# ArturKKK/graphcast-lite

Hardware: AMD Instinct MI355X
Metric: training samples/sec (6h windows) + achieved HBM GB/s on mesh GCNConv (higher is better)
Workload: dtype f32

## Files before the change

graphcast-lite_amd/csrc/aggregate.hip:

```cpp
#include <algorithm>

#include "common.h"
#include "halo.h"

namespace {

template <int LPR, bool VL, bool VS, int EW, int ITER>
__global__ __launch_bounds__(256) void agg_kernel(const int32_t* __restrict__ rowptr, const int32_t* __restrict__ col,
                                                  const float* __restrict__ w, const int32_t* __restrict__ ecol,
                                                  const float* __restrict__ ew, const float* __restrict__ H,
                                                  int64_t ldh, int64_t bsh, const float* __restrict__ bias,
                                                  float* __restrict__ Y, int64_t ldy, int64_t bsy, int32_t n,
                                                  int32_t B, int32_t F, int32_t nRB, int32_t xcd_map,
                                                  int32_t nt_store, const int32_t* __restrict__ order16) {
  constexpr int RPW = 64 / LPR;
  constexpr int EL = LPR < gcl::kEll ? LPR : gcl::kEll;
  static_assert(EW <= EL, "ELL width exceeds the lanes of a row group");
  const int bid = blockIdx.x;
  int b, rb;
  if (xcd_map) {
    const int xcd = bid & (gcl::kNumXCD - 1);
    const int slot = bid >> 3;
    b = xcd + gcl::kNumXCD * (slot / nRB);
    rb = slot % nRB;
  } else {
    b = bid / nRB;
    rb = bid % nRB;
  }
  if (b >= B) return;
  if (order16) {
    constexpr int RPB = RPW * 4 * ITER, K = 16 / RPB;
    rb = order16[rb / (K > 0 ? K : 1)] * (K > 0 ? K : 1) + rb % (K > 0 ? K : 1);
  }
  const int lane = threadIdx.x & 63;
  const int wave = threadIdx.x >> 6;
  const int sub = lane / LPR;
  const int l = lane % LPR;
  const int gbase = sub * LPR;
  const int c0 = l * 4;
  const bool cactive = c0 < F;
  const int cc = cactive ? c0 : 0;
  const float* __restrict__ Hb = H + (int64_t)b * bsh;
  float* __restrict__ Yb = Y + (int64_t)b * bsy;

  float bz0 = 0.f, bz1 = 0.f, bz2 = 0.f, bz3 = 0.f;
  if (bias && cactive) {
    bz0 = bias[c0];
    if (VS || c0 + 1 < F) bz1 = bias[c0 + 1];
    if (VS || c0 + 2 < F) bz2 = bias[c0 + 2];
    if (VS || c0 + 3 < F) bz3 = bias[c0 + 3];
  }

  auto ld4 = [&](int j, float& x0, float& x1, float& x2, float& x3) {
    const float* p = Hb + (int64_t)j * ldh + cc;
    if (VL) {
      const float4 v = *reinterpret_cast<const float4*>(p);
      x0 = v.x; x1 = v.y; x2 = v.z; x3 = v.w;
    } else {
      x0 = p[0];
      x1 = (cc + 1 < F) ? p[1] : 0.f;
      x2 = (cc + 2 < F) ? p[2] : 0.f;
      x3 = (cc + 3 < F) ? p[3] : 0.f;
    }
  };

  const int row_first = (rb * 4 + wave) * (RPW * ITER) + sub;
  auto meta = [&](int row, int& start, int& end, int& cj, float& wj) {
    const int rc = row < n ? row : n - 1;
    start = rowptr[rc];
    end = rowptr[rc + 1];
    cj = ecol[(int64_t)rc * gcl::kEll + (l & (EL - 1))];
    wj = ew[(int64_t)rc * gcl::kEll + (l & (EL - 1))];
  };
  int start, end, cj;
  float wj;
  meta(row_first, start, end, cj, wj);

#pragma unroll 1
  for (int it = 0; it < ITER; ++it) {
    const int row = row_first + it * RPW;
    int nstart = 0, nend = 0, ncj = 0;
    float nwj = 0.f;
    if (it + 1 < ITER) meta(row + RPW, nstart, nend, ncj, nwj);

    const int deg_all = end - start;
    const bool heavy = deg_all > gcl::kHeavy;
    const int deg = heavy ? 0 : deg_all;
    if (heavy) end = start;
    float a0 = 0.f, a1 = 0.f, a2 = 0.f, a3 = 0.f;
    {
      int jj[EW];
      float ww[EW], v0[EW], v1[EW], v2[EW], v3[EW];
#pragma unroll
      for (int k = 0; k < EW; ++k) {
        jj[k] = __shfl(cj, gbase + k, 64);
        ww[k] = __shfl(wj, gbase + k, 64);
      }
#pragma unroll
      for (int k = 0; k < EW; ++k) ld4(jj[k], v0[k], v1[k], v2[k], v3[k]);
#pragma unroll
      for (int k = 0; k < EW; ++k) {
        const bool in = k < deg;
        a0 += in ? ww[k] * v0[k] : 0.f;
        a1 += in ? ww[k] * v1[k] : 0.f;
        a2 += in ? ww[k] * v2[k] : 0.f;
        a3 += in ? ww[k] * v3[k] : 0.f;
      }
    }
    if (__any(deg > EW)) {
      for (int base = start + EW; base < end; base += LPR) {
        const int mine = base + l;
        int oj = 0;
        float ow = 0.f;
        if (mine < end) {
          oj = col[mine];
          ow = w[mine];
        }
        const int cnt = min(LPR, end - base);
        for (int k = 0; k < cnt; k += 4) {
          const int j0 = __shfl(oj, gbase + k, 64);
          const int j1 = __shfl(oj, gbase + ((k + 1) & (LPR - 1)), 64);
          const int j2 = __shfl(oj, gbase + ((k + 2) & (LPR - 1)), 64);
          const int j3 = __shfl(oj, gbase + ((k + 3) & (LPR - 1)), 64);
          const float w0 = __shfl(ow, gbase + k, 64);
          const float w1 = __shfl(ow, gbase + ((k + 1) & (LPR - 1)), 64);
          const float w2 = __shfl(ow, gbase + ((k + 2) & (LPR - 1)), 64);
          const float w3 = __shfl(ow, gbase + ((k + 3) & (LPR - 1)), 64);
          float p0 = 0, p1 = 0, p2 = 0, p3 = 0, q0 = 0, q1 = 0, q2 = 0, q3 = 0;
          float r0 = 0, r1 = 0, r2 = 0, r3 = 0, s0 = 0, s1 = 0, s2 = 0, s3 = 0;
          ld4(j0, p0, p1, p2, p3);
          if (k + 1 < cnt) ld4(j1, q0, q1, q2, q3);
          if (k + 2 < cnt) ld4(j2, r0, r1, r2, r3);
          if (k + 3 < cnt) ld4(j3, s0, s1, s2, s3);
          a0 += w0 * p0; a1 += w0 * p1; a2 += w0 * p2; a3 += w0 * p3;
          if (k + 1 < cnt) { a0 += w1 * q0; a1 += w1 * q1; a2 += w1 * q2; a3 += w1 * q3; }
          if (k + 2 < cnt) { a0 += w2 * r0; a1 += w2 * r1; a2 += w2 * r2; a3 += w2 * r3; }
          if (k + 3 < cnt) { a0 += w3 * s0; a1 += w3 * s1; a2 += w3 * s2; a3 += w3 * s3; }
        }
      }
    }
    if (row < n && cactive && !heavy) {
      a0 += bz0; a1 += bz1; a2 += bz2; a3 += bz3;
      float* __restrict__ yp = Yb + (int64_t)row * ldy + c0;
      if (VS) {
        if (nt_store) {
          typedef float v4f __attribute__((ext_vector_type(4)));
          v4f v = {a0, a1, a2, a3};
          __builtin_nontemporal_store(v, reinterpret_cast<v4f*>(yp));
        } else {
          *reinterpret_cast<float4*>(yp) = make_float4(a0, a1, a2, a3);
        }
      } else {
        yp[0] = a0;
        if (c0 + 1 < F) yp[1] = a1;
        if (c0 + 2 < F) yp[2] = a2;
        if (c0 + 3 < F) yp[3] = a3;
      }
    }
    start = nstart; end = nend; cj = ncj; wj = nwj;
  }
}

template <int LPR, bool VL, bool VS>
__global__ __launch_bounds__(256) void agg_heavy_kernel(const int32_t* __restrict__ rows_heavy,
                                                        const int32_t* __restrict__ rowptr,
                                                        const int32_t* __restrict__ col, const float* __restrict__ w,
                                                        const float* __restrict__ H, int64_t ldh, int64_t bsh,
                                                        const float* __restrict__ bias, float* __restrict__ Y,
                                                        int64_t ldy, int64_t bsy, int32_t F) {
  constexpr int NG = 256 / LPR;
  __shared__ float red[NG][LPR * 4 + 1];
  const int row = rows_heavy[blockIdx.x];
  const int b = blockIdx.y;
  const int g = threadIdx.x / LPR, l = threadIdx.x % LPR;
  const int c0 = l * 4;
  const bool cactive = c0 < F;
  const int cc = cactive ? c0 : 0;
  const float* __restrict__ Hb = H + (int64_t)b * bsh;
  const int start = rowptr[row], end = rowptr[row + 1];
  float a0 = 0.f, a1 = 0.f, a2 = 0.f, a3 = 0.f;
  auto ld4 = [&](int j, float& x0, float& x1, float& x2, float& x3) {
    const float* p = Hb + (int64_t)j * ldh + cc;
    if (VL) {
      const float4 v = *reinterpret_cast<const float4*>(p);
      x0 = v.x; x1 = v.y; x2 = v.z; x3 = v.w;
    } else {
      x0 = p[0];
      x1 = (cc + 1 < F) ? p[1] : 0.f;
      x2 = (cc + 2 < F) ? p[2] : 0.f;
      x3 = (cc + 3 < F) ? p[3] : 0.f;
    }
  };
  for (int e = start + g; e < end; e += 4 * NG) {
    const int e1 = e + NG, e2 = e + 2 * NG, e3 = e + 3 * NG;
    const int j0 = col[e], j1 = col[e1 < end ? e1 : e], j2 = col[e2 < end ? e2 : e], j3 = col[e3 < end ? e3 : e];
    const float w0 = w[e], w1 = e1 < end ? w[e1] : 0.f, w2 = e2 < end ? w[e2] : 0.f, w3 = e3 < end ? w[e3] : 0.f;
    float p0, p1, p2, p3, q0, q1, q2, q3, r0, r1, r2, r3, s0, s1, s2, s3;
    ld4(j0, p0, p1, p2, p3);
    ld4(j1, q0, q1, q2, q3);
    ld4(j2, r0, r1, r2, r3);
    ld4(j3, s0, s1, s2, s3);
    a0 += w0 * p0; a1 += w0 * p1; a2 += w0 * p2; a3 += w0 * p3;
    if (e1 < end) { a0 += w1 * q0; a1 += w1 * q1; a2 += w1 * q2; a3 += w1 * q3; }
    if (e2 < end) { a0 += w2 * r0; a1 += w2 * r1; a2 += w2 * r2; a3 += w2 * r3; }
    if (e3 < end) { a0 += w3 * s0; a1 += w3 * s1; a2 += w3 * s2; a3 += w3 * s3; }
  }
  red[g][c0] = a0; red[g][c0 + 1] = a1; red[g][c0 + 2] = a2; red[g][c0 + 3] = a3;
  __syncthreads();
  if (g == 0 && cactive) {
    float t0 = 0.f, t1 = 0.f, t2 = 0.f, t3 = 0.f;
#pragma unroll
    for (int q = 0; q < NG; ++q) { t0 += red[q][c0]; t1 += red[q][c0 + 1]; t2 += red[q][c0 + 2]; t3 += red[q][c0 + 3]; }
    if (bias) {
      t0 += bias[c0];
      if (c0 + 1 < F) t1 += bias[c0 + 1];
      if (c0 + 2 < F) t2 += bias[c0 + 2];
      if (c0 + 3 < F) t3 += bias[c0 + 3];
    }
    float* yp = Y + (int64_t)b * bsy + (int64_t)row * ldy + c0;
    if (VS) {
      *reinterpret_cast<float4*>(yp) = make_float4(t0, t1, t2, t3);
    } else {
      yp[0] = t0;
      if (c0 + 1 < F) yp[1] = t1;
      if (c0 + 2 < F) yp[2] = t2;
      if (c0 + 3 < F) yp[3] = t3;
    }
  }
}

using gcl::halo::mul_then_add;
using gcl::halo::row_bcast;
typedef gcl::halo::gptr_t gcl_gptr_t;
typedef gcl::halo::lptr_t gcl_lptr_t;

#ifdef GCL_STAMPS
__device__ unsigned long long agg_stamps[8 * 4096];
#define GCL_AGG_STAMP(i)                                   \
  {                                                        \
    const unsigned long long t_ = __builtin_amdgcn_s_memtime(); \
    st_acc[i] += t_ - st_last;                             \
    st_last = t_;                                          \
  }
#else
#define GCL_AGG_STAMP(i)
#endif

template <int LPR, int T, int MAXPW>
__global__ __launch_bounds__(256) void agg_halo_loop_kernel(const int32_t* __restrict__ list, const int32_t* __restrict__ cnt,
                                                            const int2* __restrict__ rec, const int32_t* __restrict__ rowptr,
                                                            const int32_t* __restrict__ opos, const float* __restrict__ w,
                                                            int32_t smax, const float* __restrict__ H, int64_t ldh,
                                                            int64_t bsh, const float* __restrict__ bias,
                                                            float* __restrict__ Y, int64_t ldy, int64_t bsy, int32_t n,
                                                            int32_t B, int32_t F, int32_t ntiles, int32_t nt_store) {
  extern __shared__ float4 img[];
  constexpr int RPW = 64 / LPR;
  constexpr int NW = 4;
  constexpr int NIT = T / NW / RPW;
  constexpr int SH = LPR == 16 ? 8 : LPR == 32 ? 9 : 10;
  typedef float v4f __attribute__((ext_vector_type(4)));
  typedef __attribute__((address_space(3))) const v4f* lds4_t;
  const int xcd = blockIdx.x & (gcl::kNumXCD - 1);
  const int J = gridDim.x >> 3, j = blockIdx.x >> 3;
  const int nsamp = (B - xcd + gcl::kNumXCD - 1) / gcl::kNumXCD;
  const int items = nsamp * ntiles;
  const int base = items / J, extra = items - base * J;
  int m = j * base + min(j, extra);
  const int mend = m + base + (j < extra ? 1 : 0);
  if (m >= mend) return;
  const int lane = threadIdx.x & 63;
  const int wave = __builtin_amdgcn_readfirstlane(threadIdx.x >> 6);
  const int sub = lane / LPR;
  const int l = lane % LPR;
  const int c0 = l * 4;
  const bool cactive = c0 < F;
  const unsigned cb = (unsigned)(cactive ? c0 : 0) * 4u;
  const unsigned ldb = (unsigned)ldh * 4u;
  const int hstride = smax - T;
  const unsigned lb = (unsigned)(size_t)((gcl_lptr_t)img) + (unsigned)l * 16u;
  const int zrow = smax << SH;

  if (threadIdx.x < LPR) img[smax * LPR + threadIdx.x] = make_float4(0.f, 0.f, 0.f, 0.f);
  float bz0 = 0.f, bz1 = 0.f, bz2 = 0.f, bz3 = 0.f;
  if (bias && cactive) {
    const float4 bv = *reinterpret_cast<const float4*>(bias + c0);
    bz0 = bv.x; bz1 = bv.y; bz2 = bv.z; bz3 = bv.w;
  }

  auto fetch_list = [&](int tile, int (&jj)[MAXPW], int& nhalo) {
    nhalo = cnt[tile] / RPW;
    const int32_t* __restrict__ tl = list + (int64_t)tile * hstride;
#pragma unroll
    for (int q = 0; q < MAXPW; ++q) {
      const int e0 = min((wave + NW * q) * RPW, hstride - RPW);
      int j = tl[e0];
#pragma unroll
      for (int r = 1; r < RPW; ++r) {
        const int jr = tl[e0 + r];
        j = sub == r ? jr : j;
      }
      jj[q] = j;
    }
  };
  int jj[MAXPW], nhalo = 0, tile = -1;
  int2 rc[NIT];
#ifdef GCL_STAMPS
  unsigned long long st_acc[8] = {0, 0, 0, 0, 0, 0, 0, 0}, st_last = __builtin_amdgcn_s_memtime();
#endif

  while (true) {
    const int tnew = m / nsamp;
    const int s = m - tnew * nsamp;
    const int b = xcd + gcl::kNumXCD * s;
    const bool newtile = tnew != tile;
    if (newtile) {
      tile = tnew;
      fetch_list(tile, jj, nhalo);
    }
    GCL_AGG_STAMP(0)
    const char* Hc = reinterpret_cast<const char*>(H + (int64_t)b * bsh);
    float* __restrict__ Yb = Y + (int64_t)b * bsy;
    const int row0 = tile * T + wave * (T / NW) + sub;
#pragma unroll
    for (int it = 0; it < NIT; ++it) {
      const int row = row0 + it * RPW;
      const char* src = Hc + (__umul24(row < n ? row : n - 1, ldb) + cb);
      __builtin_amdgcn_global_load_lds((gcl_gptr_t)src, (gcl_lptr_t)(img + (wave * (T / NW) + it * RPW) * LPR), 16, 0, 0);
    }
#pragma unroll
    for (int q = 0; q < MAXPW; ++q) {
      const int p = wave + NW * q;
      if (p < nhalo) {
        const char* src = Hc + (__umul24(jj[q], ldb) + cb);
        __builtin_amdgcn_global_load_lds((gcl_gptr_t)src, (gcl_lptr_t)(img + (T + p * RPW) * LPR), 16, 0, 0);
      }
    }
    if (newtile) {
#pragma unroll
      for (int it = 0; it < NIT; ++it) {
        const int row = row0 + it * RPW;
        rc[it] = rec[(int64_t)(row < n ? row : n - 1) * gcl::kHaloRec + (l & (gcl::kHaloRec - 1))];
      }
    }
    GCL_AGG_STAMP(1)
    __syncthreads();
    GCL_AGG_STAMP(2)

#pragma unroll
    for (int it = 0; it < NIT; ++it) {
      const int row = row0 + it * RPW;
      const int rx = rc[it].x, rw = rc[it].y;
      const int rxb = (rx & gcl::kHaloPosMask) << SH;
      float a0 = 0.f, a1 = 0.f, a2 = 0.f, a3 = 0.f;
#define GCL_HALO_MULADD(K)                                          \
  {                                                                 \
    const unsigned ad = (unsigned)row_bcast<K>(rxb) + lb;           \
    const float wk = __int_as_float(row_bcast<K>(rw));              \
    const v4f v = *(lds4_t)ad;                                      \
    a0 = mul_then_add(wk, v.x, a0);                                 \
    a1 = mul_then_add(wk, v.y, a1);                                 \
    a2 = mul_then_add(wk, v.z, a2);                                 \
    a3 = mul_then_add(wk, v.w, a3);                                 \
  }
#define GCL_HALO_FMA(K)                                             \
  {                                                                 \
    const unsigned ad = (unsigned)row_bcast<K>(rxb) + lb;           \
    const float wk = __int_as_float(row_bcast<K>(rw));              \
    const v4f v = *(lds4_t)ad;                                      \
    a0 = __fmaf_rn(wk, v.x, a0);                                    \
    a1 = __fmaf_rn(wk, v.y, a1);                                    \
    a2 = __fmaf_rn(wk, v.z, a2);                                    \
    a3 = __fmaf_rn(wk, v.w, a3);                                    \
  }
      GCL_HALO_MULADD(0) GCL_HALO_MULADD(1) GCL_HALO_MULADD(2) GCL_HALO_MULADD(3)
      GCL_HALO_MULADD(4) GCL_HALO_MULADD(5) GCL_HALO_MULADD(6) GCL_HALO_MULADD(7)
      const int last = row_bcast<15>(rx);
      if (__any(row_bcast<8>(rxb) != zrow)) {
        GCL_HALO_FMA(8) GCL_HALO_FMA(9) GCL_HALO_FMA(10) GCL_HALO_FMA(11)
        GCL_HALO_FMA(12) GCL_HALO_FMA(13) GCL_HALO_FMA(14) GCL_HALO_FMA(15)
        if (__any((last & gcl::kHaloMore) != 0)) {
          const int rcl = row < n ? row : n - 1;
          const int end = (last & gcl::kHaloMore) ? rowptr[rcl + 1] : 0;
          for (int e = rowptr[rcl] + gcl::kHaloRec; e < end; ++e) {
            const float wk = w[e];
            const v4f v = *(lds4_t)(((unsigned)opos[e] << SH) + lb);
            a0 = __fmaf_rn(wk, v.x, a0);
            a1 = __fmaf_rn(wk, v.y, a1);
            a2 = __fmaf_rn(wk, v.z, a2);
            a3 = __fmaf_rn(wk, v.w, a3);
          }
        }
      }
#undef GCL_HALO_MULADD
#undef GCL_HALO_FMA
      if (row < n && cactive && !(last & gcl::kHaloSkip)) {
        a0 += bz0; a1 += bz1; a2 += bz2; a3 += bz3;
        float* __restrict__ yp = Yb + (int64_t)row * ldy + c0;
        v4f v = {a0, a1, a2, a3};
        if (nt_store) __builtin_nontemporal_store(v, reinterpret_cast<v4f*>(yp));
        else *reinterpret_cast<v4f*>(yp) = v;
      }
    }
    GCL_AGG_STAMP(3)
#ifdef GCL_STAMPS
    st_acc[5] += 1;
#endif
    if (++m >= mend) break;
    __syncthreads();
    GCL_AGG_STAMP(4)
  }
#ifdef GCL_STAMPS
  if (lane == 0 && (blockIdx.x * NW + wave) < 4096)
    for (int i = 0; i < 8; ++i) agg_stamps[(blockIdx.x * NW + wave) * 8 + i] = st_acc[i];
#endif
}

#ifdef GCL_STAMPS
extern "C" int gcl_debug_read_agg_stamps(unsigned long long* host_out, int count) {
  GCL_CHECK_HIP(hipDeviceSynchronize());
  GCL_CHECK_HIP(hipMemcpyFromSymbol(host_out, HIP_SYMBOL(agg_stamps), sizeof(unsigned long long) * count));
  return GCL_OK;
}
#endif

struct AggArgs {
  const int32_t *rowptr, *col, *ecol, *heavy;
  const float *w, *ew;
  int ell_width, n_heavy;
  const gcl_halo* halo;
  const int32_t* order16 = nullptr;
  int32_t n_order16 = 0;
};

template <int LPR>
int launch_agg_halo(const AggArgs& ga, const float* h, int64_t ldh, int64_t bsh, const float* bias, float* y,
                    int64_t ldy, int64_t bsy, int32_t n, int32_t B, int32_t F, hipStream_t st) {
  const int enabled = gcl::env_int("GCL_AGG_HALO", 1);
  static const int force_t = gcl::env_int("GCL_AGG_HALO_T", 0);
  static const int bpc_env = gcl::env_int("GCL_AGG_HALO_BPC", 0);
  static const int nt = gcl::env_int("GCL_AGG_NT", 1);
  if (!enabled || ga.ell_width != 8) return -1;
  if ((int64_t)n * ldh * 4 >= (int64_t)1 << 31 || ldh * 4 >= (int64_t)1 << 24 || n >= 1 << 24) return -1;
  constexpr int RPW = 64 / LPR;
  const gcl_halo* hl = nullptr;
  for (int t = 0; t < 2; ++t) {
    const gcl_halo& c = ga.halo[t];
    if (c.T == 0 || (force_t && c.T != force_t)) continue;
    const int64_t bytes = (int64_t)(c.smax + 1) * LPR * 16;
    if (bytes > 80 * 1024 || gcl::cdiv((c.smax - c.T) / RPW, 4) > 32) continue;
    hl = &c;
    break;
  }
  if (!hl) return -1;
  const int64_t lds = (int64_t)(hl->smax + 1) * LPR * 16;
  const int per_cu = (int)std::min<int64_t>(8, gcl::kLdsBytes / lds);
  const int J = 32 * (bpc_env > 0 ? bpc_env : per_cu);
  const int mpw = (int)gcl::cdiv((hl->smax - hl->T) / RPW, 4);
  dim3 grid((unsigned)(gcl::kNumXCD * J)), block(256);
  auto go = [&](auto kern) -> int {
    GCL_ENSURE_DYN_LDS(kern, (size_t)lds);
    hipLaunchKernelGGL(kern, grid, block, (size_t)lds, st, hl->list, hl->cnt, reinterpret_cast<const int2*>(hl->rec),
                       ga.rowptr, hl->opos, ga.w, hl->smax, h, ldh, bsh, bias, y, ldy, bsy, n, B, F, hl->ntiles, nt);
    return GCL_OK;
  };
  int rc;
  if (hl->T == 64)
    rc = mpw <= 4 ? go(&agg_halo_loop_kernel<LPR, 64, 4>) : mpw <= 8 ? go(&agg_halo_loop_kernel<LPR, 64, 8>)
       : mpw <= 16 ? go(&agg_halo_loop_kernel<LPR, 64, 16>) : go(&agg_halo_loop_kernel<LPR, 64, 32>);
  else
    rc = mpw <= 4 ? go(&agg_halo_loop_kernel<LPR, 32, 4>) : mpw <= 8 ? go(&agg_halo_loop_kernel<LPR, 32, 8>)
       : mpw <= 16 ? go(&agg_halo_loop_kernel<LPR, 32, 16>) : go(&agg_halo_loop_kernel<LPR, 32, 32>);
  if (rc) return rc;
  GCL_CHECK_LAUNCH();
  return GCL_OK;
}

template <int LPR>
int launch_agg_heavy(const AggArgs& ga, const float* h, int64_t ldh, int64_t bsh, const float* bias, float* y,
                     int64_t ldy, int64_t bsy, int32_t B, int32_t F, bool vl, bool vs, hipStream_t st) {
  dim3 hgrid((unsigned)ga.n_heavy, (unsigned)B), block(256);
#define GCL_AGGH(VL_, VS_)                                                                                       \
  hipLaunchKernelGGL((agg_heavy_kernel<LPR, VL_, VS_>), hgrid, block, 0, st, ga.heavy, ga.rowptr, ga.col, ga.w, h, \
                     ldh, bsh, bias, y, ldy, bsy, F)
  if (vl && vs) GCL_AGGH(true, true);
  else if (vl) GCL_AGGH(true, false);
  else if (vs) GCL_AGGH(false, true);
  else GCL_AGGH(false, false);
#undef GCL_AGGH
  GCL_CHECK_LAUNCH();
  return GCL_OK;
}

template <int LPR>
int launch_agg(const AggArgs& ga, const float* h, int64_t ldh, int64_t bsh, const float* bias, float* y, int64_t ldy,
               int64_t bsy, int32_t n, int32_t B, int32_t F, hipStream_t st) {
  constexpr int RPW = 64 / LPR;
  constexpr int EL = LPR < gcl::kEll ? LPR : gcl::kEll;
  const bool vl = (ldh % 4 == 0) && (bsh % 4 == 0) && gcl::aligned16(h) && ldh >= ((F + 3) / 4) * 4;
  const bool vs = (ldy % 4 == 0) && (bsy % 4 == 0) && gcl::aligned16(y) && (F % 4 == 0);
  if constexpr (LPR >= 16) {
    if (vl && vs && (!bias || gcl::aligned16(bias))) {
      const int hr = launch_agg_halo<LPR>(ga, h, ldh, bsh, bias, y, ldy, bsy, n, B, F, st);
      if (hr >= 0) {
        if (hr != GCL_OK || ga.n_heavy == 0) return hr;
        return launch_agg_heavy<LPR>(ga, h, ldh, bsh, bias, y, ldy, bsy, B, F, true, true, st);
      }
    }
  }
  static const int iter_env = gcl::env_int("GCL_AGG_ITER", 0);
  static const int ew_env = gcl::env_int("GCL_AGG_EW", 0);
  static const int nt = gcl::env_int("GCL_AGG_NT", 1);
  int ewidth = ew_env > 0 ? ew_env : ga.ell_width;
  if (ewidth > EL) ewidth = EL;
  ewidth = ewidth >= 8 ? 8 : ewidth >= 4 ? 4 : ewidth >= 2 ? 2 : 1;
  const int iter = (iter_env == 1 || iter_env == 2 || iter_env == 4 || iter_env == 8) ? iter_env
                                                                                       : (ewidth >= 4 ? 1 : 2);
  int32_t nRB = (int32_t)gcl::cdiv(n, RPW * 4 * iter);
  if (ga.order16 && RPW * 4 * iter <= 16) nRB = ga.n_order16 * (16 / (RPW * 4 * iter));
  const int xcd_map = B >= gcl::kNumXCD ? 1 : 0;
  const int64_t nb = xcd_map ? (int64_t)gcl::kNumXCD * gcl::cdiv(B, gcl::kNumXCD) * nRB : (int64_t)B * nRB;
  GCL_CHECK_ARG(nb < (int64_t)INT32_MAX, "aggregate: grid too large");
  dim3 grid((unsigned)nb), block(256);
  const int32_t* order16 = (RPW * 4 * iter <= 16) ? ga.order16 : nullptr;
#define GCL_AGG4(VL_, VS_, EW_, IT_)                                                                             \
  hipLaunchKernelGGL((agg_kernel<LPR, VL_, VS_, EW_, IT_>), grid, block, 0, st, ga.rowptr, ga.col, ga.w, ga.ecol, \
                     ga.ew, h, ldh, bsh, bias, y, ldy, bsy, n, B, F, nRB, xcd_map, nt, order16)
#define GCL_AGG3(VL_, VS_, EW_)              \
  do {                                       \
    if (iter == 8) GCL_AGG4(VL_, VS_, EW_, 8); \
    else if (iter == 4) GCL_AGG4(VL_, VS_, EW_, 4); \
    else if (iter == 2) GCL_AGG4(VL_, VS_, EW_, 2); \
    else GCL_AGG4(VL_, VS_, EW_, 1);         \
  } while (0)
#define GCL_AGG2(VL_, VS_)                                        \
  do {                                                            \
    if constexpr (EL >= 8) { if (ewidth == 8) { GCL_AGG3(VL_, VS_, 8); break; } } \
    if (ewidth >= 4) GCL_AGG3(VL_, VS_, 4);                       \
    else if (ewidth == 2) GCL_AGG3(VL_, VS_, 2);                  \
    else GCL_AGG3(VL_, VS_, 1);                                   \
  } while (0)
  if (vl && vs) GCL_AGG2(true, true);
  else if (vl) GCL_AGG2(true, false);
  else if (vs) GCL_AGG2(false, true);
  else GCL_AGG2(false, false);
#undef GCL_AGG2
#undef GCL_AGG3
#undef GCL_AGG4
  GCL_CHECK_LAUNCH();
  if (ga.n_heavy > 0) return launch_agg_heavy<LPR>(ga, h, ldh, bsh, bias, y, ldy, bsy, B, F, vl, vs, st);
  return GCL_OK;
}

}

extern "C" int gcl_aggregate(const gcl_graph_t* g, int32_t transpose, const float* h, int64_t ldh, int64_t bsh,
                             const float* bias, float* y, int64_t ldy, int64_t bsy, int32_t B, int32_t F,
                             gcl_stream_t stream) {
  GCL_CHECK_ARG(g && h && y, "aggregate: null argument");
  GCL_CHECK_ARG(B > 0 && F > 0 && F <= 256, "aggregate: unsupported B=%d F=%d (F must be in 1..256)", B, F);
  GCL_CHECK_ARG(ldh >= F && ldy >= F, "aggregate: leading dimension smaller than F");
  GCL_CHECK_ARG(g->kind != GCL_GRAPH_GAT, "aggregate: GAT graphs carry no edge weights; use gcl_gat_fwd");
  GCL_CHECK_ARG(h != y, "aggregate: in-place aggregation is not supported");
  AggArgs ga;
  ga.rowptr = transpose ? g->trowptr : g->rowptr;
  ga.col = transpose ? g->tcol : g->col;
  ga.w = transpose ? g->tw : g->w;
  ga.ecol = transpose ? g->tecol : g->ecol;
  ga.ew = transpose ? g->tew : g->ew;
  ga.ell_width = transpose ? g->tell_width : g->ell_width;
  ga.order16 = g->order16[transpose ? 1 : 0];
  ga.n_order16 = g->n_order16;
  ga.heavy = transpose ? g->theavy : g->heavy;
  ga.n_heavy = transpose ? g->n_theavy : g->n_heavy;
  ga.halo = g->halo[transpose ? 1 : 0];
  GCL_CHECK_ARG(B <= 65535 || ga.n_heavy == 0, "aggregate: batch too large for the heavy-row launch");
  hipStream_t st = (hipStream_t)stream;
  const int lanes = (F + 3) / 4;
  if (lanes <= 4) return launch_agg<4>(ga, h, ldh, bsh, bias, y, ldy, bsy, g->n, B, F, st);
  if (lanes <= 8) return launch_agg<8>(ga, h, ldh, bsh, bias, y, ldy, bsy, g->n, B, F, st);
  if (lanes <= 16) return launch_agg<16>(ga, h, ldh, bsh, bias, y, ldy, bsy, g->n, B, F, st);
  if (lanes <= 32) return launch_agg<32>(ga, h, ldh, bsh, bias, y, ldy, bsy, g->n, B, F, st);
  return launch_agg<64>(ga, h, ldh, bsh, bias, y, ldy, bsy, g->n, B, F, st);
}
```

graphcast-lite_amd/csrc/gcn_layer.hip:

```cpp
#include "common.h"
#include "halo.h"
#include "mfma_io.h"
#include "x3.h"

namespace {

using namespace gcl::mfma_io;
using gcl::x3::bf16x8;
using gcl::x3::Pk3;
using gcl::x3::split2;
constexpr int kWRowB = 144;

template <int ACT>
__device__ __forceinline__ float act_t(float x, float a) {
  if (ACT == gcl::kActPrelu) return x > 0.f ? x : a * x;
  if (ACT == gcl::kActSilu) return gcl::silu_f(x);
  return x;
}

struct Sched {
  int xcd_map, nRT, s, rt, ds, drt, xg;
  int64_t left;
  __device__ __forceinline__ void init(int B_, int nRT_, int nwaves) {
    nRT = nRT_;
// ... 487 lines not shown
    for (int u = 0; u < 8; ++u) {
      const int k = s * 16 + h * 8 + u;
      v[u] = (j < N && k < K) ? W[(int64_t)j * K + k] : 0.f;
    }
    const Pk3 p0 = split2(v[0], v[1]), p1 = split2(v[2], v[3]), p2 = split2(v[4], v[5]), p3 = split2(v[6], v[7]);
    typedef unsigned u32x4_t __attribute__((ext_vector_type(4)));
    wf.f[s][0] = __builtin_bit_cast(bf16x8, u32x4_t{p0.h, p1.h, p2.h, p3.h});
    wf.f[s][1] = __builtin_bit_cast(bf16x8, u32x4_t{p0.m, p1.m, p2.m, p3.m});
    wf.f[s][2] = __builtin_bit_cast(bf16x8, u32x4_t{p0.l, p1.l, p2.l, p3.l});
  }
  return wf;
}

struct NoBetween {
  __device__ __forceinline__ void operator()(int) const {}
};
template <class F = NoBetween>
__device__ __forceinline__ void mfma_half_x3(f32x16& acc, const float* __restrict__ At, int KP, const WFrag& wf, int nks,
                                             F between = F()) {
  const int lane = threadIdx.x & 63, r = lane & 31, h = lane >> 5;
  const float* ap = At + r * KP + 8 * h;
  bf16x8 ah[4], am[4], al[4];
#pragma unroll
  for (int s = 0; s < 4; ++s) {
    if (s < nks) {
      const float2 f0 = *reinterpret_cast<const float2*>(ap + 16 * s), f1 = *reinterpret_cast<const float2*>(ap + 16 * s + 2);
      const float2 f2 = *reinterpret_cast<const float2*>(ap + 16 * s + 4), f3 = *reinterpret_cast<const float2*>(ap + 16 * s + 6);
      const Pk3 p0 = split2(f0.x, f0.y), p1 = split2(f1.x, f1.y), p2 = split2(f2.x, f2.y), p3 = split2(f3.x, f3.y);
      typedef unsigned u32x4_t __attribute__((ext_vector_type(4)));
      ah[s] = __builtin_bit_cast(bf16x8, u32x4_t{p0.h, p1.h, p2.h, p3.h});
      am[s] = __builtin_bit_cast(bf16x8, u32x4_t{p0.m, p1.m, p2.m, p3.m});
      al[s] = __builtin_bit_cast(bf16x8, u32x4_t{p0.l, p1.l, p2.l, p3.l});
    }
    between(s);
  }
#pragma unroll
  for (int s = 0; s < 4; ++s)
    if (s < nks) {
      acc = __builtin_amdgcn_mfma_f32_32x32x16_bf16(al[s], wf.f[s][0], acc, 0, 0, 0);
      acc = __builtin_amdgcn_mfma_f32_32x32x16_bf16(ah[s], wf.f[s][2], acc, 0, 0, 0);
      acc = __builtin_amdgcn_mfma_f32_32x32x16_bf16(am[s], wf.f[s][1], acc, 0, 0, 0);
    }
#pragma unroll
  for (int s = 0; s < 4; ++s)
    if (s < nks) {
      acc = __builtin_amdgcn_mfma_f32_32x32x16_bf16(am[s], wf.f[s][0], acc, 0, 0, 0);
      acc = __builtin_amdgcn_mfma_f32_32x32x16_bf16(ah[s], wf.f[s][1], acc, 0, 0, 0);
    }
#pragma unroll
  for (int s = 0; s < 4; ++s)
    if (s < nks) acc = __builtin_amdgcn_mfma_f32_32x32x16_bf16(ah[s], wf.f[s][0], acc, 0, 0, 0);
}

template <int ACT, int MAXPW, int STAUX = 0, bool DIRECT = false, bool INTER = false, bool TAB = false>
__global__ __launch_bounds__(256, 3) void gcn_halo_fwd_kernel(
    const int32_t* __restrict__ list, const int32_t* __restrict__ cnt, const int2* __restrict__ rec,
    const int32_t* __restrict__ rowptr, const int32_t* __restrict__ opos, const float* __restrict__ w, int32_t smax,
    const float* __restrict__ X, int64_t ldx, int64_t bsx, const float* __restrict__ slope_p, const float* __restrict__ W,
    const float* __restrict__ bias, float* __restrict__ Y, int64_t ldy, int64_t bsy, int32_t n, int32_t B, int32_t K,
    int32_t N, int32_t Nst, int32_t ntiles, const int32_t* __restrict__ tab = nullptr) {
  using gcl::halo::glds16;
  using gcl::halo::row_bcast;
  extern __shared__ __align__(16) float smem[];
  constexpr int T = 64, LPR = 16, RPW = 4, NIT = 4, SH = 8;
  typedef float v4f __attribute__((ext_vector_type(4)));
  typedef __attribute__((address_space(3))) const v4f* lds4_t;
  const int KP = K + 2;
  const int AtF = 32 * KP > 2048 ? 32 * KP : 2048;
  float* At = smem;
  float* imgf = At + 2 * AtF;
  float4* img = reinterpret_cast<float4*>(imgf);
  const int lane = threadIdx.x & 63;
  const int wave = __builtin_amdgcn_readfirstlane(threadIdx.x >> 6);
  const int sub = lane >> 4, l = lane & 15, c0 = l * 4;
  const bool cactive = c0 < K;
  const unsigned cb = (unsigned)(cactive ? c0 : 0) * 4u, ldb = (unsigned)ldx * 4u;
  const int hstride = smax - T;
  const unsigned lds_img = (unsigned)(size_t)((gcl::halo::lptr_t)img);
  const unsigned lb = lds_img + (unsigned)l * 16u;
  const int zrow = smax << SH;
  const int pair = wave >> 1, half = wave & 1;
  const WFrag wf = load_wfrag(W, half * 32, N, K);
  if (threadIdx.x < LPR) img[smax * LPR + threadIdx.x] = make_float4(0.f, 0.f, 0.f, 0.f);
  const float slope = (ACT == gcl::kActPrelu) ? *slope_p : 1.f;
  float4 bq = make_float4(0.f, 0.f, 0.f, 0.f);
  if (bias) {
    const int oc = half * 32 + (lane & 7) * 4;
    bq.x = oc < N ? bias[oc] : 0.f; bq.y = oc + 1 < N ? bias[oc + 1] : 0.f;
    bq.z = oc + 2 < N ? bias[oc + 2] : 0.f; bq.w = oc + 3 < N ? bias[oc + 3] : 0.f;
  }
  float bcol = 0.f;
  if (bias && half * 32 + (lane & 31) < N) bcol = bias[half * 32 + (lane & 31)];
  asm volatile("" : "+v"(bq.x), "+v"(bq.y), "+v"(bq.z), "+v"(bq.w), "+v"(bcol));
  __syncthreads();

  const int xcd = blockIdx.x & (gcl::kNumXCD - 1);
  const int J = gridDim.x >> 3, j = blockIdx.x >> 3;
  const int nsamp = (B - xcd + gcl::kNumXCD - 1) / gcl::kNumXCD;
  const int items = nsamp * ntiles;
  const int base = items / J, extra = items - base * J;
  int m = j * base + min(j, extra);
  const int mend = m + base + (j < extra ? 1 : 0);
  if (m >= mend) return;

  int jj[MAXPW], nhalo = 0, tile = -1;
  int own[TAB ? NIT : 1];
  int2 rc[NIT];
  auto new_tile = [&](int t) {
    tile = t;
    nhalo = cnt[t] / RPW;
    const int32_t* __restrict__ tl = list + (int64_t)t * hstride;
#pragma unroll
    for (int q = 0; q < MAXPW; ++q) {
      const int e0 = min((wave + 4 * q) * RPW, hstride - RPW);
      int jv = tl[e0];
#pragma unroll
      for (int r = 1; r < RPW; ++r) {
        const int jr = tl[e0 + r];
        jv = sub == r ? jr : jv;
      }
      jj[q] = TAB ? tab[jv] : jv;
    }
#pragma unroll
    for (int it = 0; it < NIT; ++it) {
      const int row = t * T + wave * 16 + sub + it * RPW;
      rc[it] = rec[(int64_t)(row < n ? row : n - 1) * gcl::kHaloRec + l];
      if (TAB) own[it] = tab[row < n ? row : n - 1];
    }
  };
  auto src_off = [&](int src, unsigned sboff) -> unsigned {
    if (!TAB) return __umul24(src, ldb) + cb;
    return (src >= 0 ? sboff + __umul24(src, ldb) : __umul24(~src, ldb)) + cb;
  };
  auto stage = [&](int mm) {
    const int s = mm - tile * nsamp;
    const char* Xc = reinterpret_cast<const char*>(X + (TAB ? 0 : (int64_t)(xcd + gcl::kNumXCD * s) * bsx));
    const unsigned sboff = TAB ? (unsigned)(xcd + gcl::kNumXCD * s) * (unsigned)bsx * 4u : 0u;
#pragma unroll
    for (int it = 0; it < NIT; ++it) {
      const int row = tile * T + wave * 16 + sub + it * RPW;
      glds16(Xc, src_off(TAB ? own[TAB ? it : 0] : (row < n ? row : n - 1), sboff), lds_img + (unsigned)((wave * 16 + it * RPW) << SH));
    }
#pragma unroll
    for (int q = 0; q < MAXPW; ++q) {
      const int p = wave + 4 * q;
      if (p < nhalo) glds16(Xc, src_off(jj[q], sboff), lds_img + (unsigned)((T + p * RPW) << SH));
    }
  };
  const char* Xn = nullptr;
  unsigned sbn = 0;
  auto stage_pair = [&](int s2) {
#pragma unroll
    for (int u = 0; u < 2; ++u) {
      const int pc = s2 * 2 + u;
      if (pc < NIT) {
        const int row = tile * T + wave * 16 + sub + pc * RPW;
        glds16(Xn, src_off(TAB ? own[TAB ? pc : 0] : (row < n ? row : n - 1), sbn), lds_img + (unsigned)((wave * 16 + pc * RPW) << SH));
      } else if (pc - NIT < MAXPW) {
        const int q = pc - NIT, p = wave + 4 * q;
        if (p < nhalo) glds16(Xn, src_off(jj[q < MAXPW ? q : 0], sbn), lds_img + (unsigned)((T + p * RPW) << SH));
      }
    }
  };
  new_tile(m / nsamp);
#pragma unroll
  for (int it = 0; it < NIT; ++it) asm volatile("" : "+v"(rc[it].x), "+v"(rc[it].y));
  if (TAB) {
#pragma unroll
    for (int it = 0; it < NIT; ++it) asm volatile("" : "+v"(own[TAB ? it : 0]));
  }
  stage(m);
#ifdef GCL_STAMPS
  unsigned long long stamp_acc[8] = {0, 0, 0, 0, 0, 0, 0, 0}, stamp_last = __builtin_amdgcn_s_memtime();
#endif

  while (true) {
    const int s = m - tile * nsamp;
    const int b = xcd + gcl::kNumXCD * s;
    const int trow = tile * T;
    asm volatile("s_waitcnt vmcnt(0)" ::: "memory");
    if (ACT != gcl::kActNone) {
      typedef __attribute__((address_space(3))) v4f* lds4w_t;
      auto act_piece = [&](unsigned ad) {
        v4f v = *(lds4_t)ad;
        if (ACT == gcl::kActPrelu) {
          v.x = v.x > 0.f ? v.x : slope * v.x; v.y = v.y > 0.f ? v.y : slope * v.y;
          v.z = v.z > 0.f ? v.z : slope * v.z; v.w = v.w > 0.f ? v.w : slope * v.w;
        } else {
          v.x = gcl::silu_f(v.x); v.y = gcl::silu_f(v.y); v.z = gcl::silu_f(v.z); v.w = gcl::silu_f(v.w);
        }
        *(lds4w_t)ad = v;
      };
      const unsigned la = lds_img + (unsigned)lane * 16u;
#pragma unroll
      for (int it = 0; it < NIT; ++it) act_piece(la + (unsigned)((wave * 16 + it * RPW) << SH));
#pragma unroll
      for (int q = 0; q < MAXPW; ++q) {
        const int p = wave + 4 * q;
        if (p < nhalo) act_piece(la + (unsigned)((T + p * RPW) << SH));
      }
      asm volatile("s_waitcnt lgkmcnt(0)" ::: "memory");
    }
    __builtin_amdgcn_s_barrier();
    GCL_STAMP(0);
    float* Ap = At + pair * AtF;
#pragma unroll
    for (int it = 0; it < NIT; ++it) {
      const int row = trow + wave * 16 + it * RPW + sub;
      const int rx = rc[it].x, rw = rc[it].y;
      const int rxb = (rx & gcl::kHaloPosMask) << SH;
      f32x2 a01 = {0.f, 0.f}, a23 = {0.f, 0.f};
#define GCL_FUSED_SLOT(Kk)                                              \
  {                                                                     \
    const unsigned ad = (unsigned)row_bcast<Kk>(rxb) + lb;              \
    const float wk = __int_as_float(row_bcast<Kk>(rw));                 \
    const v4f v = *(lds4_t)ad;                                          \
    row_fma<gcl::kActNone>(a01, a23, make_float4(v.x, v.y, v.z, v.w), wk, 1.f); \
  }
      GCL_FUSED_SLOT(0) GCL_FUSED_SLOT(1) GCL_FUSED_SLOT(2) GCL_FUSED_SLOT(3)
      GCL_FUSED_SLOT(4) GCL_FUSED_SLOT(5) GCL_FUSED_SLOT(6) GCL_FUSED_SLOT(7)
      const int last = row_bcast<15>(rx);
      if (__any(row_bcast<8>(rxb) != zrow)) {
        GCL_FUSED_SLOT(8) GCL_FUSED_SLOT(9) GCL_FUSED_SLOT(10) GCL_FUSED_SLOT(11)
        GCL_FUSED_SLOT(12) GCL_FUSED_SLOT(13) GCL_FUSED_SLOT(14) GCL_FUSED_SLOT(15)
        if (__any((last & gcl::kHaloMore) != 0)) {
          const int rcl = row < n ? row : n - 1;
          const int end = (last & gcl::kHaloMore) ? rowptr[rcl + 1] : 0;
          for (int e = rowptr[rcl] + gcl::kHaloRec; e < end; ++e) {
            const v4f v = *(lds4_t)(((unsigned)opos[e] << SH) + lb);
            row_fma<gcl::kActNone>(a01, a23, make_float4(v.x, v.y, v.z, v.w), w[e], 1.f);
          }
        }
      }
#undef GCL_FUSED_SLOT
      if (cactive) {
        float2* d = reinterpret_cast<float2*>(Ap + (half * 16 + it * RPW + sub) * KP + c0);
        d[0] = make_float2(a01.x, a01.y);
        d[1] = make_float2(a23.x, a23.y);
      }
    }
    GCL_STAMP(1);
    asm volatile("s_waitcnt lgkmcnt(0)" ::: "memory");
    __builtin_amdgcn_s_barrier();
    GCL_STAMP(2);
    const bool more = m + 1 < mend;
    if (more) {
      const int tn = (m + 1) / nsamp;
      if (tn != tile) new_tile(tn);
      if (!INTER) stage(m + 1);
      else if (TAB) Xn = reinterpret_cast<const char*>(X), sbn = (unsigned)(xcd + gcl::kNumXCD * (m + 1 - tile * nsamp)) * (unsigned)bsx * 4u;
      else Xn = reinterpret_cast<const char*>(X + (int64_t)(xcd + gcl::kNumXCD * (m + 1 - tile * nsamp)) * bsx);
    }
    GCL_STAMP(3);
    f32x16 acc;
#pragma unroll
    for (int r = 0; r < 16; ++r) acc[r] = 0.f;
    if (INTER) {
      static_assert(!INTER || NIT + MAXPW <= 8, "the interleaved issue places two pieces behind each of four k-steps");
      mfma_half_x3(acc, Ap, KP, wf, K >> 4, [&](int s2) {
        if (more) stage_pair(s2);
      });
    } else
    mfma_half_x3(acc, Ap, KP, wf, K >> 4);
#ifdef GCL_STAMPS
    asm volatile("" ::"v"(acc[0]));
#endif
    GCL_STAMP(4);
    if (DIRECT) {
      const int r0 = trow + pair * 32;
      const int nr = n - r0 < 32 ? n - r0 : 32;
      const int col = half * 32 + (lane & 31);
      float* Yb = Y + (int64_t)b * bsy + (int64_t)r0 * ldy;
      const __amdgpu_buffer_rsrc_t ry = make_rsrc(Yb, nr > 0 ? ((int64_t)(nr - 1) * ldy + Nst) * 4 : 0);
      const unsigned cofs = col < Nst ? (unsigned)col * 4u : kOOB;
      const unsigned ldyb = (unsigned)ldy * 4u;
#pragma unroll
      for (int r = 0; r < 16; ++r) {
        const unsigned off = (unsigned)d_row(r, lane) * ldyb + cofs;
        __builtin_amdgcn_raw_buffer_store_b32(__builtin_bit_cast(unsigned, acc[r] + bcol), ry, off, 0, STAUX);
      }
      GCL_STAMP(6);
    } else {
    asm volatile("s_waitcnt lgkmcnt(0)" ::: "memory");
    __builtin_amdgcn_s_barrier();
    GCL_STAMP(5);
    {
      f32x16 accv[1] = {acc};
      const int r0 = trow + pair * 32;
      const int nr = n - r0 < 32 ? n - r0 : 32;
      int nst = Nst - half * 32;
      nst = nst < 0 ? 0 : (nst > 32 ? 32 : nst);
      store_tile<1, STAUX>(accv, Ap + half * (32 * 32), Y + (int64_t)b * bsy + (int64_t)r0 * ldy + half * 32, ldy, nr, nst, bq);
    }
    GCL_STAMP(6);
    }
#ifdef GCL_STAMPS
    stamp_acc[7] += 1;
#endif
    if (!more) break;
    ++m;
  }
#ifdef GCL_STAMPS
  if (lane == 0 && blockIdx.x < 4096 / 4)
    for (int i = 0; i < 8; ++i) gl_stamps[(blockIdx.x * 4 + wave) * 8 + i] = stamp_acc[i];
#endif
}

}

#ifdef GCL_STAMPS
extern "C" int gcl_debug_read_stamps(unsigned long long* host_out, int count) {
  GCL_CHECK_HIP(hipDeviceSynchronize());
  GCL_CHECK_HIP(hipMemcpyFromSymbol(host_out, HIP_SYMBOL(gl_stamps), sizeof(unsigned long long) * count));
  return GCL_OK;
}
#endif

static int halo_layer_launch(const gcl_graph_t* g, const float* x, int64_t ldx, int64_t bsx, const int32_t* tab,
                             int64_t x_rows, int32_t act, const float* slope, const float* W, const float* bias, float* y,
                             int64_t ldy, int64_t bsy, int32_t B, int32_t Fin, int32_t Fout, int32_t Fout_store,
                             int32_t rows_out, hipStream_t st, bool* launched) {
  *launched = false;
  const int32_t n = g->n;
  const int halo_on = gcl::env_int("GCL_GCN_HALO", 1);
  const int x3_on = gcl::env_int("GCL_X3", 1) && gcl::env_int("GCL_X3_GCN", 1);
  const gcl_halo& hl = g->halo[0][0];
  const int hp4 = hl.T == 64 ? (int)gcl::cdiv((hl.smax - 64) / 4, 4) : 99;
  const int KPh = Fin + 2;
  const size_t ldsh = (size_t)2 * (32 * KPh > 2048 ? 32 * KPh : 2048) * 4 + (size_t)(hl.smax + 1) * 256;
  const bool offs_ok = tab ? (x_rows * ldx * 4 < ((int64_t)1 << 32) && (int64_t)B * bsx * 4 < ((int64_t)1 << 32) && x_rows < (1 << 24))
                           : ((int64_t)n * ldx * 4 < ((int64_t)1 << 31));
  if (!(halo_on && x3_on && g->kind == GCL_GRAPH_GCN && g->n_heavy == 0 && hl.T == 64 && hp4 <= 8 && Fin % 16 == 0 && Fin > 32 && rows_out == n &&
        g->e >= 6 * (int64_t)n && ldsh <= 80 * 1024 && offs_ok && n < (1 << 24) && ldx * 4 < (1 << 24) &&
        (int64_t)n * ldy * 4 < ((int64_t)1 << 31)))
    return GCL_OK;
  if (tab && hp4 > 4) return GCL_OK;
  static const int bpc_env = gcl::env_int("GCL_GCN_HALO_BPC", 0);
  const int per_cu = (int)(gcl::kLdsBytes / ldsh);
  const int Jx = 32 * (bpc_env > 0 ? bpc_env : per_cu);
  dim3 grid((unsigned)(gcl::kNumXCD * Jx));
  auto go = [&](auto kern) -> int {
    GCL_ENSURE_DYN_LDS(kern, ldsh);
    hipLaunchKernelGGL(kern, grid, dim3(256), ldsh, st, hl.list, hl.cnt, reinterpret_cast<const int2*>(hl.rec), g->rowptr,
                       hl.opos, g->w, hl.smax, x, ldx, bsx, slope, W, bias, y, ldy, bsy, n, B, Fin, Fout, Fout_store,
                       hl.ntiles, tab);
    return GCL_OK;
  };
  int rc;
  const int form_env = gcl::env_int("GCL_GCN_HALO_FORM", 1);
  if (tab)
    rc = act == GCL_ACT_PRELU  ? go(&gcn_halo_fwd_kernel<gcl::kActPrelu, 4, 2, true, true, true>)
         : act == GCL_ACT_SILU ? go(&gcn_halo_fwd_kernel<gcl::kActSilu, 4, 2, true, true, true>)
                               : go(&gcn_halo_fwd_kernel<gcl::kActNone, 4, 2, true, true, true>);
  else if (hp4 <= 4 && form_env)
    rc = act == GCL_ACT_PRELU  ? go(&gcn_halo_fwd_kernel<gcl::kActPrelu, 4, 2, true, true>)
         : act == GCL_ACT_SILU ? go(&gcn_halo_fwd_kernel<gcl::kActSilu, 4, 2, true, true>)
                               : go(&gcn_halo_fwd_kernel<gcl::kActNone, 4, 2, true, true>);
  else if (hp4 <= 4)
    rc = act == GCL_ACT_PRELU  ? go(&gcn_halo_fwd_kernel<gcl::kActPrelu, 4>)
         : act == GCL_ACT_SILU ? go(&gcn_halo_fwd_kernel<gcl::kActSilu, 4>)
                               : go(&gcn_halo_fwd_kernel<gcl::kActNone, 4>);
  else
    rc = act == GCL_ACT_PRELU  ? go(&gcn_halo_fwd_kernel<gcl::kActPrelu, 8, 2, true>)
         : act == GCL_ACT_SILU ? go(&gcn_halo_fwd_kernel<gcl::kActSilu, 8, 2, true>)
                               : go(&gcn_halo_fwd_kernel<gcl::kActNone, 8, 2, true>);
  if (rc) return rc;
  GCL_CHECK_LAUNCH();
  *launched = true;
  return GCL_OK;
}

extern "C" int gcl_gcn_layer_fwd(const gcl_graph_t* g, const float* x, int64_t ldx, int64_t bsx, int32_t act,
                                 const float* slope, const float* W, const float* bias, float* y, int64_t ldy,
                                 int64_t bsy, int32_t B, int32_t Fin, int32_t Fout, int32_t Fout_store,
                                 gcl_stream_t stream) {
  return gcl_gcn_layer_fwd_rows(g, x, ldx, bsx, act, slope, W, bias, y, ldy, bsy, B, Fin, Fout, Fout_store,
                                g ? g->n : 0, stream);
}

extern "C" int gcl_gcn_layer_fwd_rows(const gcl_graph_t* g, const float* x, int64_t ldx, int64_t bsx, int32_t act,
                                      const float* slope, const float* W, const float* bias, float* y, int64_t ldy,
                                      int64_t bsy, int32_t B, int32_t Fin, int32_t Fout, int32_t Fout_store,
                                      int32_t rows_out, gcl_stream_t stream) {
  GCL_CHECK_ARG(g && x && W && y, "gcn_layer_fwd: null argument");
  GCL_CHECK_ARG(g->kind == GCL_GRAPH_GCN || g->kind == GCL_GRAPH_MEAN, "gcn_layer_fwd: graph carries no edge weights");
  GCL_CHECK_ARG(B > 0 && Fin >= 4 && Fin <= 64 && Fin % 4 == 0 && Fout >= 1 && Fout <= 64,
                "gcn_layer_fwd: unsupported Fin=%d Fout=%d (Fin %% 4 == 0, both <= 64)", Fin, Fout);
  GCL_CHECK_ARG(Fout_store >= Fout && Fout_store % 4 == 0 && Fout_store <= 64 && ldy >= Fout_store,
                "gcn_layer_fwd: Fout_store=%d must be a multiple of 4 in [Fout, min(64, ldy)]", Fout_store);
  GCL_CHECK_ARG(ldx >= Fin && ldx % 4 == 0 && bsx % 4 == 0 && gcl::aligned16(x), "gcn_layer_fwd: x rows must be 16-B aligned");
  GCL_CHECK_ARG(ldy % 4 == 0 && bsy % 4 == 0 && gcl::aligned16(y), "gcn_layer_fwd: y rows must be 16-B aligned");
  GCL_CHECK_ARG(g->n_heavy == 0, "gcn_layer_fwd: the graph has rows with more than %d in-edges", gcl::kHeavy);
  GCL_CHECK_ARG(act == GCL_ACT_NONE || act == GCL_ACT_SILU || (act == GCL_ACT_PRELU && slope),
                "gcn_layer_fwd: bad activation %d", act);
  GCL_CHECK_ARG(x != y, "gcn_layer_fwd: in-place is not supported");
  const int32_t n = g->n;
  GCL_CHECK_ARG(rows_out >= 1 && rows_out <= n, "gcn_layer_fwd: rows_out=%d outside [1, n=%d]", rows_out, n);
  hipStream_t st = (hipStream_t)stream;
  {
    bool launched = false;
    const int rc = halo_layer_launch(g, x, ldx, bsx, nullptr, 0, act, slope, W, bias, y, ldy, bsy, B, Fin, Fout, Fout_store,
                                     rows_out, st, &launched);
    if (rc || launched) return rc;
  }
  const int32_t nRT = (int32_t)gcl::cdiv(rows_out, 32);
  const int NS = Fout_store > 32 ? 2 : 1;
  constexpr int NW12 = 12, NW8 = 8;
  const int KP = Fin + 2;
  const int x3_env = gcl::env_int("GCL_X3", 1) && gcl::env_int("GCL_X3_GCN", 1);
  const size_t wave1_b = (size_t)wave_region_f(32 * (KP > NS * 32 ? KP : NS * 32)) * sizeof(float);
  const bool x3 = x3_env != 0 && (Fin % 16 == 0);
  const int NWr = x3 ? NW8 : NW12;
  const size_t lds = (x3 ? (size_t)3 * NS * 32 * kWRowB : (size_t)NS * 32 * KP * sizeof(float)) + NWr * wave1_b;
  GCL_CHECK_ARG((int64_t)n * ldx * 4 < (int64_t)1 << 31 && n < (1 << 24) && ldx * 4 < (1 << 24),
                "gcn_layer_fwd: one sample of x must stay below 2 GiB (n, row bytes < 2^24)");
  const int64_t tiles = (int64_t)B * nRT;
  int64_t grid = gcl::kNumCU;
  if (tiles < grid * NWr) grid = gcl::cdiv(tiles, NWr);
  if (B >= gcl::kNumXCD) grid = gcl::cdiv(grid, gcl::kNumXCD) * gcl::kNumXCD;
  const int ewidth = g->ell_cover;
#define GCL_GF4(NS_, ACT_, EW_)                \
  do {                                         \
    if (x3) GCL_GF5(NS_, ACT_, EW_, true);     \
    else GCL_GF5(NS_, ACT_, EW_, false);       \
  } while (0)
#define GCL_GF5(NS_, ACT_, EW_, X3_)                                                                                 \
  do {                                                                                                              \
    constexpr int NW = X3_ ? NW8 : NW12;                                                                            \
    auto kern = gcn_fwd_kernel<NS_, ACT_, EW_, NW, false, X3_>;                                                              \
    GCL_ENSURE_DYN_LDS(kern, gcl::kLdsBytes);                                                                       \
    hipLaunchKernelGGL(kern, dim3((unsigned)grid), dim3(NW * 64), lds, st, g->rowptr, g->col, g->w, g->ecol, g->ew, x, \
                       ldx, bsx, slope, W, bias, y, ldy, bsy, n, B, Fin, Fout, Fout_store, nRT, rows_out);                     \
  } while (0)
#define GCL_GF3(NS_, ACT_)                  \
  do {                                      \
    switch (ewidth) {                       \
      case 8: GCL_GF4(NS_, ACT_, 8); break; \
      case 4: GCL_GF4(NS_, ACT_, 4); break; \
      default: GCL_GF4(NS_, ACT_, 2); break; \
    }                                       \
  } while (0)
#define GCL_GF2(NS_)                                         \
  do {                                                       \
    if (act == GCL_ACT_PRELU) GCL_GF3(NS_, gcl::kActPrelu);  \
    else if (act == GCL_ACT_SILU) GCL_GF3(NS_, gcl::kActSilu); \
    else GCL_GF3(NS_, gcl::kActNone);                        \
  } while (0)
  if (g->kind == GCL_GRAPH_MEAN) {
    GCL_CHECK_ARG(act == GCL_ACT_NONE, "gcn_layer_fwd: mean-aggregation graphs take no activation");
    constexpr int NW = NW12;
    const size_t lds = (size_t)NS * 32 * KP * sizeof(float) + NW * wave1_b;
    int64_t grid = gcl::kNumCU;
    if (tiles < grid * NW) grid = gcl::cdiv(tiles, NW);
    if (B >= gcl::kNumXCD) grid = gcl::cdiv(grid, gcl::kNumXCD) * gcl::kNumXCD;
    if (NS == 2) {
      auto kern = gcn_fwd_kernel<2, gcl::kActNone, 8, NW, true, false>;
      GCL_ENSURE_DYN_LDS(kern, gcl::kLdsBytes);
      hipLaunchKernelGGL(kern, dim3((unsigned)grid), dim3(NW * 64), lds, st, g->rowptr, g->col, g->w, g->ecol, g->ew, x, ldx,
                         bsx, slope, W, bias, y, ldy, bsy, n, B, Fin, Fout, Fout_store, nRT, rows_out);
    } else {
      auto kern = gcn_fwd_kernel<1, gcl::kActNone, 8, NW, true, false>;
      GCL_ENSURE_DYN_LDS(kern, gcl::kLdsBytes);
      hipLaunchKernelGGL(kern, dim3((unsigned)grid), dim3(NW * 64), lds, st, g->rowptr, g->col, g->w, g->ecol, g->ew, x, ldx,
                         bsx, slope, W, bias, y, ldy, bsy, n, B, Fin, Fout, Fout_store, nRT, rows_out);
    }
  } else if (NS == 2) GCL_GF2(2);
  else GCL_GF2(1);
#undef GCL_GF2
#undef GCL_GF3
#undef GCL_GF4
#undef GCL_GF5
  GCL_CHECK_LAUNCH();
  return GCL_OK;
}

extern "C" int gcl_gcn_layer_fwd_tab(const gcl_graph_t* g, const float* x, int64_t ldx, int64_t bsx, int64_t x_rows,
                                     const int32_t* tab, int32_t act, const float* slope, const float* W,
                                     const float* bias, float* y, int64_t ldy, int64_t bsy, int32_t B, int32_t Fin,
                                     int32_t Fout, int32_t Fout_store, gcl_stream_t stream) {
  GCL_CHECK_ARG(g && x && W && y && tab, "gcn_layer_fwd_tab: null argument");
  GCL_CHECK_ARG(g->kind == GCL_GRAPH_GCN, "gcn_layer_fwd_tab: graph carries no GCN edge weights");
  GCL_CHECK_ARG(B > 0 && Fin >= 4 && Fin <= 64 && Fin % 4 == 0 && Fout >= 1 && Fout <= 64,
                "gcn_layer_fwd_tab: unsupported Fin=%d Fout=%d (Fin %% 4 == 0, both <= 64)", Fin, Fout);
  GCL_CHECK_ARG(Fout_store >= Fout && Fout_store % 4 == 0 && Fout_store <= 64 && ldy >= Fout_store,
                "gcn_layer_fwd_tab: Fout_store=%d must be a multiple of 4 in [Fout, min(64, ldy)]", Fout_store);
  GCL_CHECK_ARG(ldx >= Fin && ldx % 4 == 0 && bsx % 4 == 0 && gcl::aligned16(x) && x_rows >= 1,
                "gcn_layer_fwd_tab: x rows must be 16-B aligned");
  GCL_CHECK_ARG(ldy % 4 == 0 && bsy % 4 == 0 && gcl::aligned16(y), "gcn_layer_fwd_tab: y rows must be 16-B aligned");
  GCL_CHECK_ARG(act == GCL_ACT_NONE || act == GCL_ACT_SILU || (act == GCL_ACT_PRELU && slope),
                "gcn_layer_fwd_tab: bad activation %d", act);
  bool launched = false;
  const int rc = halo_layer_launch(g, x, ldx, bsx, tab, x_rows, act, slope, W, bias, y, ldy, bsy, B, Fin, Fout, Fout_store,
                                   g->n, (hipStream_t)stream, &launched);
  if (rc) return rc;
  if (!launched && g->n_heavy) {
    gcl::set_error("gcn_layer_fwd_tab: the graph has %d heavy rows (more than %d in-edges), which the source-tile form "
                   "does not compute", g->n_heavy, gcl::kHeavy);
    return GCL_EUNSUPPORTED;
  }
  if (!launched) {
    gcl::set_error("gcn_layer_fwd_tab: this graph / shape has no source-tile form (Fin=%d Fout=%d)", Fin, Fout);
    return GCL_EUNSUPPORTED;
  }
  return GCL_OK;
}

extern "C" int gcl_gcn_layer_fwd_tab_ok(const gcl_graph_t* g, int64_t ldx, int64_t bsx, int64_t x_rows, int32_t B,
                                        int32_t Fin, int32_t Fout) {
  if (!g || g->kind != GCL_GRAPH_GCN || g->n_heavy) return 0;
  const int x3_on = gcl::env_int("GCL_X3", 1) && gcl::env_int("GCL_X3_GCN", 1);
  const gcl_halo& hl = g->halo[0][0];
  if (!gcl::env_int("GCL_GCN_HALO", 1) || !x3_on || hl.T != 64) return 0;
  const int hp4 = (int)gcl::cdiv((hl.smax - 64) / 4, 4);
  const size_t ldsh = (size_t)2 * (32 * (Fin + 2) > 2048 ? 32 * (Fin + 2) : 2048) * 4 + (size_t)(hl.smax + 1) * 256;
  return hp4 <= 4 && Fin % 16 == 0 && Fin > 32 && Fin <= 64 && Fout >= 1 && Fout <= 64 && g->e >= 6 * (int64_t)g->n &&
                 ldsh <= 80 * 1024 && x_rows * ldx * 4 < ((int64_t)1 << 32) && (int64_t)B * bsx * 4 < ((int64_t)1 << 32) &&
                 x_rows < (1 << 24) && g->n < (1 << 24) && ldx * 4 < (1 << 24)
             ? 1
             : 0;
}
```

graphcast-lite_amd/csrc/norm.hip:

```cpp
#include "common.h"

namespace {

template <int LPR>
__device__ __forceinline__ float group_sum(float v) {
#pragma unroll
  for (int off = LPR / 2; off > 0; off >>= 1) v += __shfl_xor(v, off, 64);
  return v;
}

__device__ __forceinline__ void load4(const float* p, int c0, int F, bool vec, float& a, float& b, float& c, float& d) {
  if (vec) {
#ifndef GCL_NORM_LD_PLAIN
    typedef float lv4f __attribute__((ext_vector_type(4)));
    const lv4f v = __builtin_nontemporal_load(reinterpret_cast<const lv4f*>(p));
#else
    const float4 v = *reinterpret_cast<const float4*>(p);
#endif
    a = v.x; b = v.y; c = v.z; d = v.w;
  } else {
    a = (c0 < F) ? p[0] : 0.f;
    b = (c0 + 1 < F) ? p[1] : 0.f;
    c = (c0 + 2 < F) ? p[2] : 0.f;
    d = (c0 + 3 < F) ? p[3] : 0.f;
  }
}
template <bool V>
__device__ __forceinline__ void load4_row(const float* p, int c0, int F, bool vec, float& a, float& b, float& c, float& d) {
  load4(p, c0, F, vec, a, b, c, d);
  if (!V && vec) {
    b = (c0 + 1 < F) ? b : 0.f;
    c = (c0 + 2 < F) ? c : 0.f;
    d = (c0 + 3 < F) ? d : 0.f;
  }
}
__device__ __forceinline__ void store4(float* p, int c0, int F, bool vec, float a, float b, float c, float d) {
  if (vec) {
    *reinterpret_cast<float4*>(p) = make_float4(a, b, c, d);
  } else {
    if (c0 < F) p[0] = a;
    if (c0 + 1 < F) p[1] = b;
    if (c0 + 2 < F) p[2] = c;
    if (c0 + 3 < F) p[3] = d;
  }
}

template <int LPR, bool V, bool MAP = false>
__global__ __launch_bounds__(256) void ln_fwd_kernel(const float* __restrict__ X, int64_t ldx,
                                                     const float* __restrict__ gamma, const float* __restrict__ beta,
                                                     float eps, float* __restrict__ Y, int64_t ldy,
                                                     float* __restrict__ stats, int64_t rows, int32_t F, int32_t vx,
                                                     int32_t vy, const int32_t* __restrict__ pos = nullptr,
                                                     int64_t bsy = 0, int32_t n_per = 1) {
  if (V) vx = vy = 1;
  constexpr int RPB = (64 / LPR) * 4;
  const int lane = threadIdx.x & 63, wave = threadIdx.x >> 6;
  const int sub = lane / LPR, l = lane % LPR, c0 = l * 4;
  const float invF = 1.f / (float)F;
  float g0 = 0, g1 = 0, g2 = 0, g3 = 0, b0 = 0, b1 = 0, b2 = 0, b3 = 0;
  if (c0 < F) {
    load4(gamma + c0, c0, F, false, g0, g1, g2, g3);
    load4(beta + c0, c0, F, false, b0, b1, b2, b3);
  }
  for (int64_t row = (int64_t)blockIdx.x * RPB + wave * (64 / LPR) + sub; row < rows; row += (int64_t)gridDim.x * RPB) {
    float x0 = 0, x1 = 0, x2 = 0, x3 = 0;
    if (c0 < F) load4_row<V>(X + row * ldx + c0, c0, F, vx, x0, x1, x2, x3);
    const float mean = group_sum<LPR>(x0 + x1 + x2 + x3) * invF;
    const float d0 = (c0 < F) ? x0 - mean : 0.f, d1 = (c0 + 1 < F) ? x1 - mean : 0.f;
    const float d2 = (c0 + 2 < F) ? x2 - mean : 0.f, d3 = (c0 + 3 < F) ? x3 - mean : 0.f;
    float sq;
    {
#pragma clang fp contract(off)
      const float q0 = d0 * d0, q1 = d1 * d1, q2 = d2 * d2, q3 = d3 * d3;
      sq = (q0 + q1) + (q2 + q3);
    }
    const float var = group_sum<LPR>(sq) * invF;
    const float rstd = 1.0f / sqrtf(var + eps);
    if (MAP) {
      const int64_t bq = row / n_per;
      const int pj = pos[(int)(row - bq * n_per)];
      if (c0 < F && pj >= 0)
        store4(Y + bq * bsy + (int64_t)pj * ldy + c0, c0, F, vy, d0 * rstd * g0 + b0, d1 * rstd * g1 + b1,
               d2 * rstd * g2 + b2, d3 * rstd * g3 + b3);
    } else if (c0 < F)
      store4(Y + row * ldy + c0, c0, F, vy, d0 * rstd * g0 + b0, d1 * rstd * g1 + b1, d2 * rstd * g2 + b2,
             d3 * rstd * g3 + b3);
    if (l == 0 && stats) {
      stats[2 * row] = mean;
      stats[2 * row + 1] = rstd;
    }
  }
}

template <int LPR, bool V, bool CS, bool MAP>
__global__ __launch_bounds__(256) void ln_bwd_kernel(const float* __restrict__ dY, int64_t lddy,
                                                     const float* __restrict__ X, int64_t ldx,
                                                     const float* __restrict__ gamma, const float* __restrict__ stats,
                                                     float* __restrict__ dX, int64_t lddx, float* __restrict__ part,
                                                     int64_t rows, int32_t F, int32_t FP, int32_t vdy, int32_t vx,
                                                     int32_t vdx, const int32_t* __restrict__ pos, int64_t bsdy,
                                                     int32_t n_per) {
  if (V) vdy = vx = vdx = 1;
  constexpr int RPW = 64 / LPR;
  constexpr int RPB = RPW * 4;
  constexpr int NV = CS ? 3 : 2;
  __shared__ float red[RPB][LPR * 4 * NV + 1];
  const int lane = threadIdx.x & 63, wave = threadIdx.x >> 6;
  const int sub = lane / LPR, l = lane % LPR, c0 = l * 4;
  const float invF = 1.f / (float)F;
  float g0 = 0, g1 = 0, g2 = 0, g3 = 0;
  if (c0 < F) load4(gamma + c0, c0, F, false, g0, g1, g2, g3);
  float dg0 = 0, dg1 = 0, dg2 = 0, dg3 = 0, db0 = 0, db1 = 0, db2 = 0, db3 = 0;
  float cs0 = 0, cs1 = 0, cs2 = 0, cs3 = 0;
  const int64_t row_first = (int64_t)blockIdx.x * RPB + wave * RPW + sub, row_step = (int64_t)gridDim.x * RPB;
  int64_t mb = 0, msb = 0;
  int mi = 0, msi = 0;
  if (MAP) {
    mb = row_first / n_per;
    mi = (int)(row_first - mb * n_per);
    msb = row_step / n_per;
    msi = (int)(row_step - msb * n_per);
  }
  for (int64_t row = row_first; row < rows; row += row_step) {
    float x0 = 0, x1 = 0, x2 = 0, x3 = 0, y0 = 0, y1 = 0, y2 = 0, y3 = 0;
    if (c0 < F) {
      load4_row<V>(X + row * ldx + c0, c0, F, vx, x0, x1, x2, x3);
      if (MAP) {
        const int pj = pos[mi];
        if (pj >= 0) load4_row<V>(dY + mb * bsdy + (int64_t)pj * lddy + c0, c0, F, vdy, y0, y1, y2, y3);
      } else {
        load4_row<V>(dY + row * lddy + c0, c0, F, vdy, y0, y1, y2, y3);
      }
    }
    if (MAP) {
      mi += msi;
      mb += msb;
      if (mi >= n_per) { mi -= n_per; ++mb; }
    }
    const float mean = stats[2 * row], rstd = stats[2 * row + 1];
    const float h0 = (c0 < F) ? (x0 - mean) * rstd : 0.f, h1 = (c0 + 1 < F) ? (x1 - mean) * rstd : 0.f;
    const float h2 = (c0 + 2 < F) ? (x2 - mean) * rstd : 0.f, h3 = (c0 + 3 < F) ? (x3 - mean) * rstd : 0.f;
    const float q0 = y0 * g0, q1 = y1 * g1, q2 = y2 * g2, q3 = y3 * g3;
    const float m1 = group_sum<LPR>(q0 + q1 + q2 + q3) * invF;
    const float m2 = group_sum<LPR>(q0 * h0 + q1 * h1 + q2 * h2 + q3 * h3) * invF;
    const float o0 = rstd * (q0 - m1 - h0 * m2), o1 = rstd * (q1 - m1 - h1 * m2), o2 = rstd * (q2 - m1 - h2 * m2),
                o3 = rstd * (q3 - m1 - h3 * m2);
    if (c0 < F) store4(dX + row * lddx + c0, c0, F, vdx, o0, o1, o2, o3);
    if (CS) {
      cs0 += (c0 < F) ? o0 : 0.f; cs1 += (c0 + 1 < F) ? o1 : 0.f; cs2 += (c0 + 2 < F) ? o2 : 0.f; cs3 += (c0 + 3 < F) ? o3 : 0.f;
    }
    dg0 += y0 * h0; dg1 += y1 * h1; dg2 += y2 * h2; dg3 += y3 * h3;
    db0 += y0; db1 += y1; db2 += y2; db3 += y3;
  }
  const int g = wave * RPW + sub;
  float* r = red[g];
  r[c0] = dg0; r[c0 + 1] = dg1; r[c0 + 2] = dg2; r[c0 + 3] = dg3;
  r[LPR * 4 + c0] = db0; r[LPR * 4 + c0 + 1] = db1; r[LPR * 4 + c0 + 2] = db2; r[LPR * 4 + c0 + 3] = db3;
  if (CS) {
    r[2 * LPR * 4 + c0] = cs0; r[2 * LPR * 4 + c0 + 1] = cs1; r[2 * LPR * 4 + c0 + 2] = cs2; r[2 * LPR * 4 + c0 + 3] = cs3;
  }
  __syncthreads();
  for (int idx = threadIdx.x; idx < NV * LPR * 4; idx += 256) {
    float s = 0.f;
#pragma unroll
    for (int q = 0; q < RPB; ++q) s += red[q][idx];
    const int which = idx / (LPR * 4), c = idx % (LPR * 4);
    if (c < F) part[(size_t)blockIdx.x * NV * FP + which * FP + c] = s;
  }
}

template <int LPR, bool V>
__global__ __launch_bounds__(256) void colsum_kernel(const float* __restrict__ X, int64_t ldx,
                                                     float* __restrict__ part, int64_t rows, int32_t F, int32_t FP,
                                                     int32_t vx) {
  if (V) vx = 1;
  constexpr int RPW = 64 / LPR;
  constexpr int RPB = RPW * 4;
  __shared__ float red[RPB][LPR * 4 + 1];
  const int lane = threadIdx.x & 63, wave = threadIdx.x >> 6;
  const int sub = lane / LPR, l = lane % LPR, c0 = l * 4;
  float s0 = 0, s1 = 0, s2 = 0, s3 = 0;
  if (c0 < F) {
    const int64_t step = (int64_t)gridDim.x * RPB;
    int64_t row = (int64_t)blockIdx.x * RPB + wave * RPW + sub;
    for (; row + 3 * step < rows; row += 4 * step) {
      float a0, a1, a2, a3, b0, b1, b2, b3, c1_, c2_, c3_, c4_, d0, d1, d2, d3;
      load4(X + row * ldx + c0, c0, F, vx, a0, a1, a2, a3);
// ... 40 lines not shown
    case 16: CALL(16); break;       \
    case 32: CALL(32); break;       \
    default: CALL(64); break;       \
  }

extern "C" int gcl_layernorm_fwd(const float* x, int64_t ldx, const float* gamma, const float* beta, float eps,
                                 float* y, int64_t ldy, float* stats, int64_t rows, int32_t F, gcl_stream_t stream) {
  GCL_CHECK_ARG(x && gamma && beta && y, "layernorm_fwd: null argument");
  GCL_CHECK_ARG(F >= 1 && F <= 256 && ldx >= F && ldy >= F, "layernorm_fwd: bad shape F=%d", F);
  if (rows == 0) return GCL_OK;
  const int lpr = lpr_for(F);
  const int rpb = (64 / lpr) * 4;
  int64_t nb = gcl::cdiv(rows, rpb);
  if (nb > 8192) nb = 8192;
  const int vx = vec_ok(x, ldx, F), vy = vec_store_ok(y, ldy, F);
#define CALL(L)                                                                                                  \
  if (vx && vy)                                                                                                  \
    hipLaunchKernelGGL((ln_fwd_kernel<L, true>), dim3((unsigned)nb), dim3(256), 0, (hipStream_t)stream, x, ldx,  \
                       gamma, beta, eps, y, ldy, stats, rows, F, vx, vy, (const int32_t*)nullptr, (int64_t)0, 1); \
  else                                                                                                           \
    hipLaunchKernelGGL((ln_fwd_kernel<L, false>), dim3((unsigned)nb), dim3(256), 0, (hipStream_t)stream, x, ldx, \
                       gamma, beta, eps, y, ldy, stats, rows, F, vx, vy, (const int32_t*)nullptr, (int64_t)0, 1)
  GCL_DISPATCH_LPR(lpr, CALL)
#undef CALL
  GCL_CHECK_LAUNCH();
  return GCL_OK;
}

extern "C" int gcl_layernorm_fwd_map(const float* x, int64_t ldx, const float* gamma, const float* beta, float eps,
                                     float* y, int64_t ldy, int64_t bsy, const int32_t* pos, int32_t n_per, float* stats,
                                     int64_t rows, int32_t F, gcl_stream_t stream) {
  GCL_CHECK_ARG(x && gamma && beta && y && pos && stats, "layernorm_fwd_map: null argument");
  GCL_CHECK_ARG(F >= 1 && F <= 256 && ldx >= F && ldy >= F, "layernorm_fwd_map: bad shape F=%d", F);
  GCL_CHECK_ARG(n_per > 0 && rows % n_per == 0, "layernorm_fwd_map: rows must be B * n_per");
  if (rows == 0) return GCL_OK;
  const int lpr = lpr_for(F);
  const int rpb = (64 / lpr) * 4;
  int64_t nb = gcl::cdiv(rows, rpb);
  if (nb > 8192) nb = 8192;
  const int vx = vec_ok(x, ldx, F), vy = vec_store_ok(y, ldy, F) && (bsy % 4 == 0);
#define CALL(L)                                                                                                        \
  if (vx && vy)                                                                                                        \
    hipLaunchKernelGGL((ln_fwd_kernel<L, true, true>), dim3((unsigned)nb), dim3(256), 0, (hipStream_t)stream, x, ldx,  \
                       gamma, beta, eps, y, ldy, stats, rows, F, vx, vy, pos, bsy, n_per);                             \
  else                                                                                                                 \
    hipLaunchKernelGGL((ln_fwd_kernel<L, false, true>), dim3((unsigned)nb), dim3(256), 0, (hipStream_t)stream, x, ldx, \
                       gamma, beta, eps, y, ldy, stats, rows, F, vx, vy, pos, bsy, n_per)
  GCL_DISPATCH_LPR(lpr, CALL)
#undef CALL
  GCL_CHECK_LAUNCH();
  return GCL_OK;
}

extern "C" size_t gcl_layernorm_bwd_ws_bytes(int64_t rows, int32_t F) {
  (void)rows;
  const size_t FP = (size_t)((F + 3) / 4) * 4;
  return (size_t)kNormBlocks * 3 * FP * sizeof(float);
}

extern "C" int gcl_layernorm_bwd_cs(const float* dy, int64_t lddy, const float* x, int64_t ldx, const float* gamma,
                                    const float* stats, float* dx, int64_t lddx, float* dgamma, float* dbeta,
                                    float* colsum_dx, int32_t accumulate, int64_t rows, int32_t F, void* ws,
                                    size_t ws_bytes, gcl_stream_t stream) {
  return gcl_layernorm_bwd_map(dy, lddy, 0, nullptr, 0, x, ldx, gamma, stats, dx, lddx, dgamma, dbeta, colsum_dx, accumulate,
                               rows, F, ws, ws_bytes, stream);
}

extern "C" int gcl_layernorm_bwd_map(const float* dy, int64_t lddy, int64_t bsdy, const int32_t* pos, int32_t n_per,
                                     const float* x, int64_t ldx, const float* gamma, const float* stats, float* dx,
                                     int64_t lddx, float* dgamma, float* dbeta, float* colsum_dx, int32_t accumulate,
                                     int64_t rows, int32_t F, void* ws, size_t ws_bytes, gcl_stream_t stream) {
  GCL_CHECK_ARG(dy && x && gamma && stats && dx && dgamma && dbeta, "layernorm_bwd: null argument");
  GCL_CHECK_ARG(!pos || (n_per > 0 && rows % n_per == 0), "layernorm_bwd: mapped dy needs rows = B * n_per");
  GCL_CHECK_ARG(F >= 1 && F <= 256 && ldx >= F && lddy >= F && lddx >= F, "layernorm_bwd: bad shape F=%d", F);
  GCL_CHECK_ARG(ws && ws_bytes >= gcl_layernorm_bwd_ws_bytes(rows, F), "layernorm_bwd: workspace too small");
  if (rows == 0) return GCL_OK;
  hipStream_t st = (hipStream_t)stream;
  const int lpr = lpr_for(F);
  const int rpb = (64 / lpr) * 4;
  const int FP = ((F + 3) / 4) * 4;
  int64_t nb = gcl::cdiv(rows, rpb);
  if (nb > kNormBlocks) nb = kNormBlocks;
  float* part = (float*)ws;
  const int vdy = vec_ok(dy, lddy, F) && (bsdy % 4 == 0), vx = vec_ok(x, ldx, F), vdx = vec_store_ok(dx, lddx, F);
  const int acc_p = (accumulate & GCL_ACC_DW) ? 1 : 0, acc_cs = (accumulate & GCL_ACC_COLSUM) ? 1 : 0;
#define CALL4(L, V_, CS_, MAP_)                                                                                       \
  hipLaunchKernelGGL((ln_bwd_kernel<L, V_, CS_, MAP_>), dim3((unsigned)nb), dim3(256), 0, st, dy, lddy, x, ldx, gamma, \
                     stats, dx, lddx, part, rows, F, FP, vdy, vx, vdx, pos, bsdy, n_per)
#define CALL3(L, V_, CS_)            \
  do {                               \
    if (pos) CALL4(L, V_, CS_, true); \
    else CALL4(L, V_, CS_, false);   \
  } while (0)
#define CALL(L)                                     \
  if (vdy && vx && vdx) {                           \
    if (colsum_dx) CALL3(L, true, true);            \
    else CALL3(L, true, false);                     \
  } else {                                          \
    if (colsum_dx) CALL3(L, false, true);           \
    else CALL3(L, false, false);                    \
  }
  GCL_DISPATCH_LPR(lpr, CALL)
#undef CALL
#undef CALL3
#undef CALL4
  GCL_CHECK_LAUNCH();
  if (!colsum_dx) return gcl::launch_reduce_parts2(part, (int)nb, 2 * FP, FP, FP, dgamma, dbeta, F, acc_p, st);
  return gcl::launch_reduce_parts3(part, (int)nb, 3 * FP, FP, dgamma, acc_p, dbeta, acc_p, colsum_dx, acc_cs, F, st);
}

extern "C" int gcl_layernorm_bwd(const float* dy, int64_t lddy, const float* x, int64_t ldx, const float* gamma,
                                 const float* stats, float* dx, int64_t lddx, float* dgamma, float* dbeta,
                                 int32_t accumulate, int64_t rows, int32_t F, void* ws, size_t ws_bytes,
                                 gcl_stream_t stream) {
  return gcl_layernorm_bwd_cs(dy, lddy, x, ldx, gamma, stats, dx, lddx, dgamma, dbeta, nullptr,
                              accumulate ? GCL_ACC_DW : 0, rows, F, ws, ws_bytes, stream);
}

extern "C" size_t gcl_colsum_ws_bytes(int64_t rows, int32_t F) {
  (void)rows;
  return (size_t)kNormBlocks * (size_t)(((F + 3) / 4) * 4) * sizeof(float);
}

extern "C" int gcl_colsum(const float* x, int64_t ldx, int64_t rows, int32_t F, float* out, int32_t accumulate,
                          void* ws, size_t ws_bytes, gcl_stream_t stream) {
  GCL_CHECK_ARG(x && out, "colsum: null argument");
  GCL_CHECK_ARG(F >= 1 && F <= 256 && ldx >= F, "colsum: bad shape F=%d", F);
  GCL_CHECK_ARG(ws && ws_bytes >= gcl_colsum_ws_bytes(rows, F), "colsum: workspace too small");
  hipStream_t st = (hipStream_t)stream;
  const int lpr = lpr_for(F);
  const int rpb = (64 / lpr) * 4;
  const int FP = ((F + 3) / 4) * 4;
  int64_t nb = gcl::cdiv(rows > 0 ? rows : 1, rpb);
  if (nb > kNormBlocks) nb = kNormBlocks;
  float* part = (float*)ws;
  const int vx = vec_ok(x, ldx, F);
#define CALL(L)                                                                                                     \
  if (vx) hipLaunchKernelGGL((colsum_kernel<L, true>), dim3((unsigned)nb), dim3(256), 0, st, x, ldx, part, rows, F, FP, vx); \
  else hipLaunchKernelGGL((colsum_kernel<L, false>), dim3((unsigned)nb), dim3(256), 0, st, x, ldx, part, rows, F, FP, vx)
  GCL_DISPATCH_LPR(lpr, CALL)
#undef CALL
  GCL_CHECK_LAUNCH();
  return gcl::launch_reduce_parts(part, (int)nb, FP, FP, out, F, 1, F, accumulate, st);
}
```

graphcast-lite_amd/functional.py:

```python
from typing import List, Optional

import os

import torch

from . import hip


def _grad_slot(p: Optional[torch.Tensor], needs: bool):
    if p is None or not needs:
        return None, False, True
    if p.grad is not None:
        return p.grad, True, True
    return torch.zeros_like(p), False, False


class _Grads:

    def __init__(self, params: List[Optional[torch.Tensor]], needs: List[bool]):
        self.dst, self.acc, self.ret_none = [], [], []
        for p, nd in zip(params, needs):
            d, a, r = _grad_slot(p, nd)
            self.dst.append(d)
            self.acc.append(a)
# ... 23 lines not shown
            W, b = params[3 * k], params[3 * k + 1]
            z = hip.linear_fwd(cur, W.detach(), b.detach(), slope)
            zs.append(z)
            cur = z
            slope = params[3 * k + 2].detach() if k < L - 1 else None
        stats = None
        out = cur
        if has_ln:
            out, stats = hip.layernorm_fwd(cur, params[-2].detach(), params[-1].detach(), eps)
        ctx.owner, ctx.has_ln, ctx.L = owner, has_ln, L
        ctx.x2, ctx.zs, ctx.stats = x2, zs, stats
        ctx.params = params
        return out.view(shape[:-1] + (out.shape[-1],))

    @staticmethod
    def backward(ctx, dy):
        params, L = ctx.params, ctx.L
        needs = list(ctx.needs_input_grad[4:])
        G = _Grads(list(params), needs)
        dy2 = hip.rows2d(dy)
        zs = ctx.zs
        if ctx.has_ln:
            gi, bi = len(params) - 2, len(params) - 1
            dgam = G.dst[gi] if G.dst[gi] is not None else torch.zeros_like(params[gi])
            dbet = G.dst[bi] if G.dst[bi] is not None else torch.zeros_like(params[bi])
            dz = hip.layernorm_bwd(dy2, zs[-1], params[gi].detach(), ctx.stats, dgam, dbet, G.acc[gi] and G.acc[bi])
        else:
            dz = dy2
        dx = None
        for k in range(L - 1, -1, -1):
            W = params[3 * k].detach()
            inp = ctx.x2 if k == 0 else zs[k - 1]
            slope = None if k == 0 else params[3 * k - 1].detach()
            wi, bi = 3 * k, 3 * k + 1
            dW = G.dst[wi] if G.dst[wi] is not None else torch.zeros_like(params[wi])
            db = G.dst[bi]
            if k > 0:
                dz = hip.linear_bwd_all(dz, W, inp, slope, G.dst[3 * k - 1], dW, db, None, G.acc[wi], acc_db=G.acc[bi])
            elif ctx.needs_input_grad[0]:
                dx = hip.linear_bwd_all(dz, W, inp, None, None, dW, db, None, G.acc[wi], acc_db=G.acc[bi],
                                        act=hip.ACT_NONE)
            elif db is not None and G.acc[bi] != G.acc[wi]:
                hip.linear_bwd_dw(dz, inp, None, dW, None, G.acc[wi])
                hip.colsum(dz, db, G.acc[bi])
            else:
                hip.linear_bwd_dw(dz, inp, None, dW, db, G.acc[wi])
        if dx is not None:
            dx = dx.view(dy.shape[:-1] + (dx.shape[-1],))
        return (dx, None, None, None) + G.out()


_LN_COLSUM = os.environ.get("GCL_NO_LN_COLSUM", "0") in ("0", "")
_ROWS_OUT = os.environ.get("GCL_NO_ROWS_OUT", "0") in ("0", "")


def _lat_first_layer_bwd(lat, enc3, dz3, W, dW, acc_dw: bool, want_dx: bool, Pc=None, enc_shape=None):
    _, _, inv_a, inv_fold = lat.maps
    B, ne, D = enc_shape if enc3 is None else enc3.shape
    G, Md, r = lat.G, lat.Md, lat.r
    nc = Md + r
    Fo = dz3.shape[-1]
    dz3 = dz3 if dz3.is_contiguous() else dz3.contiguous()
    dzc = torch.empty(B, nc, Fo, dtype=torch.float32, device=dz3.device)
    if Md > 0:
        hip.gather2_rows(dz3, inv_a[G: G + Md], None, None, Md, B, out=dzc[:, :Md])
    if r > 1:
        hip.gather2_rows(dz3, inv_fold, None, None, B * r, B, sum_batch=True, out=dzc[:, Md:], deal=r)
    elif r == 1:
        tmp = hip.gather2_rows(dz3, inv_fold, None, None, B * r, B, sum_batch=True)
        hip.copy_rows(tmp.view(B, r, Fo), dzc[:, Md:])
    if Pc is None:
        Pc = hip.copy_rows(enc3[:, G:, :], torch.empty(B, nc, D, dtype=torch.float32, device=dz3.device))
    land = lat.landing
    shared = land is not None and land.buf is not None
    if not want_dx:
        hip.linear_bwd_dw(dzc.view(B * nc, Fo), Pc.view(B * nc, D), None, dW, None, acc_dw)
        dxc = None
    else:
        dxc = hip.linear_bwd_all(dzc.view(B * nc, Fo), W, Pc.view(B * nc, D), None, None, dW, None, None, acc_dw,
                                 act=hip.ACT_NONE).view(B, nc, D)
    if shared:
        if dxc is not None:
            hip.copy_rows(dxc, land.buf[:, G:])
        land.buf, land.mesh_pending, land.handed_over = None, False, False
        return None
    if dxc is None:
        return None
    out = torch.zeros(B, ne, D, dtype=torch.float32, device=dz3.device)
    hip.copy_rows(dxc, out[:, G:])
    return out


class LatSource:

    def __init__(self, tab, maps, M: int, G: int, Md: int, r: int, landing=None):
        self.tab, self.maps, self.M, self.G, self.Md, self.r, self.landing = tab, maps, M, G, Md, r, landing
        self._compact = {}

    def compact_tab(self, ne: int):
        t = self._compact.get(ne)
        if t is None:
            tab = self.tab.to(torch.int64)
            f = -tab - 1
            bq = torch.div(f, ne, rounding_mode="floor")
            flat_c = bq * (self.Md + self.r) + (f - bq * ne - self.G)
            t = torch.where(tab >= 0, tab - self.G, -flat_c - 1).to(torch.int32).contiguous()
            self._compact[ne] = t
        return t


class GCNStackFn(torch.autograd.Function):
    @staticmethod
    def forward(ctx, x, owner, graph, L: int, has_ln: bool, eps: float, out_rows: int, *params):
        squeeze = x.dim() == 2
        x3 = _flat3(x.detach())
        B, n, _ = x3.shape
        lat = getattr(owner, "_lat_src", None)
        if lat is not None:
            owner._lat_src = None
            n = lat.M
            if not x3.is_contiguous():
                x3 = x3.contiguous()
            if lat.landing is not None:
                lat.landing.mesh_pending = True
        ctx.lat = lat
        slope_p = params[2 * L]
        akind = getattr(owner, "act_kind", hip.ACT_PRELU)
        slope_t = slope_p.detach() if slope_p is not None else getattr(owner, "const_slope", None)
        ps = []
        cur = x3
        pad_last = None
        for k in range(L):
            W, b = params[2 * k].detach(), params[2 * k + 1].detach()
            Fout = W.shape[0]
            ldh = (Fout + 3) // 4 * 4
            act_k, slope_k = (akind, slope_t) if k > 0 else (hip.ACT_NONE, None)
            if k == 0 and lat is not None:
                p = hip.gcn_layer_fwd_tab(graph, x3, lat.tab, act_k, slope_k, W, b)
                if ldh != Fout:
                    p = p.contiguous()
                ps.append(p)
                cur = p
                continue
            if hip.gcn_layer_fusable(graph, cur, W.shape[1], Fout):
                last_rows = int(out_rows) if (k == L - 1 and out_rows and out_rows < n and not has_ln and _ROWS_OUT) else None
                p = hip.gcn_layer_fwd(graph, cur, act_k, slope_k, W, b, rows_out=last_rows)
                if k == L - 1 and ldh != Fout and not has_ln:
                    pad_last = (ldh, Fout, None)
                elif ldh != Fout:
                    p = p.contiguous()
                ps.append(p)
                cur = p
                continue
            if k == L - 1 and ldh != Fout and not has_ln:
                Wp = torch.nn.functional.pad(W, (0, 0, 0, ldh - Fout))
                bp = torch.nn.functional.pad(b, (0, ldh - Fout))
                h = hip.linear_fwd(cur.reshape(B * n, -1), Wp, None, slope_k, act=act_k)
                p = hip.aggregate(graph, h.view(B, n, ldh), bp)
                ps.append(p)
                cur = p[..., :Fout]
                pad_last = (ldh, Fout, Wp)
                continue
            h = hip.linear_fwd(cur.reshape(B * n, -1) if not cur.is_contiguous() else cur.view(B * n, -1), W, None, slope_k,
                               ld_out=ldh, act=act_k)
            h3 = torch.as_strided(h, (B, n, Fout), (n * ldh, ldh, 1))
            p = hip.aggregate(graph, h3, b)
            ps.append(p)
            cur = p
        ctx.akind, ctx.slope_t, ctx.pad_last = akind, slope_t, pad_last
        out, stats = cur, None
        ctx.land = getattr(owner, "_grad_src", None)
        if ctx.land is not None:
            owner._grad_src = None
            if has_ln and not (out_rows and out_rows < n) and not squeeze:
                ctx.land.proc_ready = True
            else:
                ctx.land = None
        if has_ln:
            land = ctx.land
            if land is not None and land.dec_buf is not None and cur.is_contiguous() and land.dec_buf.shape[2] == cur.shape[2]:
                stats = hip.layernorm_fwd_map(cur.view(B * n, -1), params[-2].detach(), params[-1].detach(), eps,
                                              land.dec_buf, land.dec_map)
                land.dec_filled = True
                out = cur.new_zeros(()).expand(B, n, cur.shape[2])
            else:
                o2, stats = hip.layernorm_fwd(cur.view(B * n, -1), params[-2].detach(), params[-1].detach(), eps)
                out = o2.view(B, n, -1)
        ctx.owner, ctx.graph, ctx.L, ctx.has_ln = owner, graph, L, has_ln
        ctx.x3, ctx.ps, ctx.stats, ctx.params, ctx.squeeze = x3, ps, stats, params, squeeze
        ctx.n_rows, ctx.out_rows = n, (int(out_rows) if out_rows and out_rows < n else 0)
        if ctx.out_rows:
            out = out[:, :ctx.out_rows, :]
        return out[0] if squeeze else out

    @staticmethod
    def backward(ctx, dy):
        params, L, graph = ctx.params, ctx.L, ctx.graph
        needs = list(ctx.needs_input_grad[7:])
        G = _Grads(list(params), needs)
        land = ctx.land
        dy_map = None
        if land is not None and land.proc_src is not None:
            if all(st == 0 for st in dy.stride()):
                dy_map = (land.proc_src, land.proc_map)
                dy3 = dy
            else:
                src, pmap = land.proc_src, land.proc_map
                dy3 = _flat3(dy) + hip.gather2_rows(src, pmap, None, None, dy.shape[-2], src.shape[0])
            land.proc_src = land.proc_map = None
            land.proc_ready = False
        else:
            dy3 = _flat3(dy)
        B, n = dy3.shape[0], ctx.n_rows
        ps = ctx.ps
        pad = ctx.pad_last
        dy_rows = dy3
        if ctx.out_rows and (ctx.has_ln or pad is None):
            dy3 = hip.pad_rows(dy3, n, dy3.shape[2])
        bi_last = 2 * L - 1
        cs_done = False
        if ctx.has_ln:
            gi, bi = len(params) - 2, len(params) - 1
            dgam = G.dst[gi] if G.dst[gi] is not None else torch.zeros_like(params[gi])
            dbet = G.dst[bi] if G.dst[bi] is not None else torch.zeros_like(params[bi])
            cs = G.dst[bi_last] if (pad is None and _LN_COLSUM) else None
            dp = hip.layernorm_bwd(None if dy_map is not None else dy3.view(B * n, -1), ps[-1].view(B * n, -1),
                                   params[gi].detach(), ctx.stats, dgam, dbet, G.acc[gi] and G.acc[bi], colsum_dx=cs,
                                   acc_colsum=bool(cs is not None and G.acc[bi_last]), dy_map=dy_map).view(B, n, -1)
            cs_done = cs is not None
        else:
            dp = dy3
        si = 2 * L
        dsl = G.dst[si] if params[si] is not None else None
        slope_t, akind = ctx.slope_t, ctx.akind
        dx = None
        Fo = params[2 * (L - 1)].shape[0]
        Fp = Fo
        if pad is not None:
            Fp = pad[0]
            dp = hip.pad_rows(dy_rows if not ctx.has_ln else dp, n, Fp)
        if G.dst[bi_last] is not None and not cs_done:
            src = dy_rows if not ctx.has_ln else dp[..., :Fo]
            hip.colsum(src.reshape(-1, Fo), G.dst[bi_last], G.acc[bi_last])
        for k in range(L - 1, -1, -1):
            W = params[2 * k].detach()
            wi = 2 * k
            inp = (ctx.x3 if k == 0 else ps[k - 1]).view(-1, (ctx.x3 if k == 0 else ps[k - 1]).shape[-1])
            dh2 = hip.aggregate(graph, dp, None, transpose=True).view(B * n, -1)
            if k == L - 1 and Fp != Fo:
                dh2 = dh2[:, :Fo]
            dW = G.dst[wi] if G.dst[wi] is not None else torch.zeros_like(params[wi])
            if k > 0:
                dp = hip.linear_bwd_all(dh2, W, inp, slope_t, dsl, dW, None, G.dst[2 * k - 1], G.acc[wi],
                                        acc_colsum=G.acc[2 * k - 1], act=akind).view(B, n, -1)
            elif ctx.lat is not None:
                dx = _lat_first_layer_bwd(ctx.lat, ctx.x3, dh2.reshape(B, n, -1), W, dW, G.acc[wi], ctx.needs_input_grad[0])
            elif ctx.needs_input_grad[0]:
                dx = hip.linear_bwd_all(dh2, W, inp, None, None, dW, None, None, G.acc[wi],
                                        act=hip.ACT_NONE).view(B, n, -1)
            else:
                hip.linear_bwd_dw(dh2, inp, None, dW, None, G.acc[wi])
        if dx is not None and ctx.squeeze:
            dx = dx[0]
        return (dx, None, None, None, None, None, None) + G.out()


class GATLayerFn(torch.autograd.Function):

    @staticmethod
    def forward(ctx, x, owner, graph, H: int, want_alpha: bool, slope, W, att_src, att_dst, bias):
        squeeze = x.dim() == 2
        x3 = _flat3(x.detach())
        B, n, _ = x3.shape
        Cc = W.shape[0] // H
        sl = slope.detach() if slope is not None else None
        act = getattr(owner, "_in_act", None)
        lat = getattr(owner, "_lat_src", None)
        ctx.lat = ctx.tab = None
        if lat is not None:
            owner._lat_src = None
            assert sl is None, "a LatSource feeds the first layer of a stack (no input activation)"
            if not x3.is_contiguous():
                x3 = x3.contiguous()
            ne, D = x3.shape[1], x3.shape[2]
            nc = lat.Md + lat.r
            Pc = hip.copy_rows(x3[:, lat.G:, :], torch.empty(B, nc, D, dtype=torch.float32, device=x3.device))
            h = hip.linear_fwd(Pc.view(B * nc, D), W.detach(), None, None, act=act).view(B, nc, H * Cc)
            ctx.lat, ctx.tab, ctx.enc_shape = lat, lat.compact_tab(ne), x3.shape
            x3 = Pc
            if lat.landing is not None:
                lat.landing.mesh_pending = True
        else:
            h = hip.linear_fwd(x3.view(B * n, -1), W.detach(), None, sl, act=act).view(B, n, H * Cc)
        ctx.act = act
        y, a_s, a_d, alpha = hip.gat_fwd(graph, h, att_src.detach().reshape(-1), att_dst.detach().reshape(-1),
                                         bias.detach(), H, Cc, tab=ctx.tab)
        alpha_edges = hip.gat_alpha_edge_order(graph, alpha[0], H) if want_alpha else torch.empty(0, device=x3.device)
        ctx.owner, ctx.graph, ctx.H, ctx.Cc, ctx.squeeze = owner, graph, H, Cc, squeeze
        ctx.x3, ctx.h, ctx.a_s, ctx.a_d, ctx.alpha = x3, h, a_s, a_d, alpha
        ctx.params = (slope, W, att_src, att_dst, bias)
        ctx.mark_non_differentiable(alpha_edges)
# ... 189 lines not shown
    @staticmethod
    def forward(ctx, a, b, maps, nd: int, B: int, landing=None):
        map_a, map_b, inv_a, inv_b = maps
        a3 = a.detach()
        if not a3.is_contiguous():
            a3 = a3.contiguous()
        ctx.maps, ctx.B, ctx.landing = maps, B, landing
        ctx.sa, ctx.sb = a3.shape, (b.shape if b is not None else None)
        if landing is not None and landing.dec_filled:
            landing.dec_filled = False
            buf, landing.dec_buf = landing.dec_buf, None
            hip.copy_rows(a3[:, : landing.head, :], buf[:, : landing.head, :])
            return buf
        if landing is not None:
            landing.dec_buf = None
        b3 = b.detach() if b is not None else None
        if b3 is not None and not b3.is_contiguous():
            b3 = b3.contiguous()
        return hip.gather2_rows(a3, map_a, b3, map_b, nd, B)

    @staticmethod
    def backward(ctx, g):
        map_a, map_b, inv_a, inv_b = ctx.maps
        g = g.contiguous()
        da = db = None
        if ctx.needs_input_grad[0]:
            bc = ctx.sa[0] == 1 and ctx.B > 1
            land = ctx.landing
            if land is not None and land.mesh_pending and not bc:
                land.buf = torch.empty(ctx.sa, dtype=torch.float32, device=g.device)
                hip.gather2_rows(g, inv_a, None, None, land.head, ctx.B, out=land.buf[:, : land.head])
                da = land.buf
                land.handed_over = True
            else:
                da = hip.gather2_rows(g, inv_a, None, None, ctx.sa[1], ctx.B, sum_batch=bc)
        if ctx.sb is not None and ctx.needs_input_grad[1]:
            bc = ctx.sb[0] == 1 and ctx.B > 1
            land = ctx.landing
            if land is not None and land.proc_ready and not bc:
                land.proc_src, land.proc_map = g, inv_b
                db = g.new_zeros(()).expand(ctx.sb)
            else:
                db = hip.gather2_rows(g, inv_b, None, None, ctx.sb[1], ctx.B, sum_batch=bc)
        return da, db, None, None, None, None


class GradLanding:

    def __init__(self, head: int):
        self.head, self.buf, self.mesh_pending = head, None, False
        self.handed_over = False
        self.proc_ready, self.proc_src, self.proc_map = False, None, None
        self.dec_buf, self.dec_map, self.dec_filled = None, None, False


class MeshLatFn(torch.autograd.Function):

    @staticmethod
    def forward(ctx, enc, maps, M: int, gmd: int, r: int, landing=None):
        map_a, map_b, inv_a, inv_fold = maps
        e3 = enc.detach()
        if not e3.is_contiguous():
            e3 = e3.contiguous()
        B, ne, D = e3.shape
        ctx.maps, ctx.shape, ctx.gmd, ctx.r, ctx.landing = maps, (B, ne, D), gmd, r, landing
        if landing is not None:
            landing.mesh_pending = True
        return hip.gather2_rows(e3, map_a, e3.view(1, B * ne, D), map_b, M, B)

    @staticmethod
    def backward(ctx, g):
        _, _, inv_a, inv_fold = ctx.maps
        B, ne, D = ctx.shape
        g = g.contiguous()
        land = ctx.landing
        shared = land is not None and land.buf is not None
        out = land.buf if shared else torch.empty(B, ne, D, dtype=torch.float32, device=g.device)
        h = land.head if shared else 0
        hip.gather2_rows(g, inv_a[h:], None, None, ctx.gmd - h, B, out=out[:, h: ctx.gmd])
        if ctx.r > 1:
            hip.gather2_rows(g, inv_fold, None, None, B * ctx.r, B, sum_batch=True, out=out[:, ctx.gmd:], deal=ctx.r)
        elif ctx.r == 1:
            tmp = hip.gather2_rows(g, inv_fold, None, None, B * ctx.r, B, sum_batch=True)
            hip.copy_rows(tmp.view(B, ctx.r, D), out[:, ctx.gmd:])
        if shared:
            land.buf, land.mesh_pending, land.handed_over = None, False, False
            return None, None, None, None, None, None
        return out, None, None, None, None, None


class EdgeLayout:

    def __init__(self, edge_index: torch.Tensor, n: int, device):
        ei = edge_index.detach().to("cpu", torch.int64)
        snd, rcv = ei[0], ei[1]
        if ei.numel() and (int(ei.min()) < 0 or int(ei.max()) >= n):
            raise ValueError("edge_index refers to nodes outside [0, n)")
        order = torch.sort(rcv, stable=True).indices
        self.order = order.to(device)
        snd_s, rcv_s = snd[order], rcv[order]
        cnt = torch.bincount(rcv_s, minlength=n)
        rowptr = torch.zeros(n + 1, dtype=torch.int64)
        rowptr[1:] = torch.cumsum(cnt, 0)
        torder = torch.sort(snd_s, stable=True).indices
        tcnt = torch.bincount(snd_s, minlength=n)
        trowptr = torch.zeros(n + 1, dtype=torch.int64)
# ... 123 lines not shown
```

graphcast-lite_amd/hip.py:

```python
import ctypes as C
import os
from typing import Optional

import torch

_HERE = os.path.dirname(os.path.abspath(__file__))
LIB_PATH = os.environ.get("GCL_LIB") or os.path.join(_HERE, "libgcl_hip.so")

GRAPH_GCN, GRAPH_GAT, GRAPH_MEAN = 0, 1, 2

_lib = None

_i32, _i64, _f32, _vp, _sz = C.c_int32, C.c_int64, C.c_float, C.c_void_p, C.c_size_t

_SIGNATURES = {
    "gcl_version": (C.c_int, []),
    "gcl_last_error": (C.c_char_p, []),
    "gcl_graph_count_edges": (C.c_int, [_vp, _i64, _i32, _i32, C.POINTER(_i64)]),
    "gcl_graph_build_host": (C.c_int, [_vp, _i64, _i32, _i32] + [_vp] * 8),
    "gcl_graph_create": (C.c_int, [_vp, _i64, _i32, _i32, C.POINTER(_vp)]),
    "gcl_graph_destroy": (None, [_vp]),
    "gcl_graph_num_nodes": (_i32, [_vp]),
    "gcl_graph_num_edges": (_i64, [_vp]),
    "gcl_graph_max_in_degree": (_i32, [_vp]),
    "gcl_graph_export_edges": (C.c_int, [_vp, _vp]),
    "gcl_graph_eperm_device": (_vp, [_vp]),
    "gcl_graph_halo_info": (C.c_int, [_vp, _i32, _i32, _vp]),
    "gcl_linear_fwd": (C.c_int, [_vp, _i64, _vp, _vp, _vp, _vp, _i64, _i64, _i32, _i32, _vp]),
    "gcl_linear_bwd_dx": (C.c_int, [_vp, _i64, _vp, _vp, _i64, _vp, _vp, _vp, _i64, _i64, _i32, _i32, _vp, _sz, _vp]),
    "gcl_linear_bwd_dw": (C.c_int, [_vp, _i64, _vp, _i64, _vp, _vp, _vp, _i64, _i32, _i32, _i32, _vp, _sz, _vp]),
    "gcl_linear_bwd_ws_bytes": (_sz, [_i64, _i32, _i32]),
    "gcl_linear_bwd_all": (C.c_int, [_vp, _i64, _vp, _vp, _i64, _vp, _vp, _vp, _i64, _vp, _vp, _vp, _i64, _i32, _i32,
                                     _i32, _vp, _sz, _vp]),
    "gcl_linear_bwd_all_deferred": (C.c_int, [_vp, _i64, _vp, _vp, _i64, _vp, _vp, _vp, _i64, _vp, _vp, _vp, _i64, _i32,
                                              _i32, _i32, _vp, _sz, _vp, _vp]),
    "gcl_reduce_jobs": (C.c_int, [_vp, _i32, _vp]),
    "gcl_linear_bwd_all_ws_bytes": (_sz, [_i64, _i32, _i32]),
    "gcl_aggregate": (C.c_int, [_vp, _i32, _vp, _i64, _i64, _vp, _vp, _i64, _i64, _i32, _i32, _vp]),
    "gcl_gat_fwd": (C.c_int, [_vp, _vp, _i64, _i64, _vp, _vp, _vp, _vp, _vp, _vp, _vp, _i64, _i64, _i32, _i32, _i32, _vp]),
    "gcl_gat_bwd": (C.c_int, [_vp, _vp, _i64, _i64, _vp, _i64, _i64, _vp, _vp, _vp, _vp, _vp, _vp, _i64, _i64,
                              _vp, _vp, _vp, _i32, _i32, _i32, _i32, _vp, _sz, _vp]),
    "gcl_gat_bwd_ws_bytes": (_sz, [_i64, _i32, _i32, _i32, _i32]),
    "gcl_gat_fwd_tab": (C.c_int, [_vp, _vp, _i64, _i64, _vp, _vp, _vp, _vp, _vp, _vp, _vp, _vp, _i64, _i64, _i32, _i32, _i32, _vp]),
    "gcl_gat_bwd_tab": (C.c_int, [_vp, _vp, _i64, _i64, _vp, _i64, _i64, _vp, _vp, _vp, _vp, _vp, _vp, _vp, _i64, _i64,
                                  _vp, _vp, _vp, _i32, _i32, _i32, _i32, _vp, _sz, _vp]),
    "gcl_gat_tab_ok": (C.c_int, [_vp, _i64, _i32, _i32]),
    "gcl_gat_alpha_to_edge_order": (C.c_int, [_vp, _vp, _vp, _i32, _vp]),
    "gcl_gat_prune": (C.c_int, [_vp, _vp, _f32, _vp, C.POINTER(_i64), _vp, _sz, _vp]),
    "gcl_gat_prune_ws_bytes": (_sz, [_i64]),
    "gcl_layernorm_fwd": (C.c_int, [_vp, _i64, _vp, _vp, _f32, _vp, _i64, _vp, _i64, _i32, _vp]),
    "gcl_layernorm_bwd": (C.c_int, [_vp, _i64, _vp, _i64, _vp, _vp, _vp, _i64, _vp, _vp, _i32, _i64, _i32, _vp, _sz, _vp]),
    "gcl_layernorm_bwd_cs": (C.c_int, [_vp, _i64, _vp, _i64, _vp, _vp, _vp, _i64, _vp, _vp, _vp, _i32, _i64, _i32, _vp, _sz, _vp]),
    "gcl_layernorm_bwd_map": (C.c_int, [_vp, _i64, _i64, _vp, _i32, _vp, _i64, _vp, _vp, _vp, _i64, _vp, _vp, _vp, _i32, _i64,
                                        _i32, _vp, _sz, _vp]),
    "gcl_layernorm_bwd_ws_bytes": (_sz, [_i64, _i32]),
    "gcl_graphnorm_fwd": (C.c_int, [_vp, _i64, _i64, _vp, _vp, _f32, _vp, _i64, _i64, _vp, _i32, _i32, _i32, _vp, _sz, _vp]),
    "gcl_graphnorm_bwd": (C.c_int, [_vp, _i64, _i64, _vp, _i64, _i64, _vp, _vp, _f32, _vp, _i64, _i64, _vp, _vp,
                                    _i32, _i32, _i32, _i32, _vp, _sz, _vp]),
    "gcl_graphnorm_ws_bytes": (_sz, [_i32, _i32, _i32]),
    "gcl_colsum": (C.c_int, [_vp, _i64, _i64, _i32, _vp, _i32, _vp, _sz, _vp]),
    "gcl_colsum_ws_bytes": (_sz, [_i64, _i32]),
    "gcl_assemble_input": (C.c_int, [_vp, _vp, _vp, _vp, _i64, _i32, _i32, _i32, _i32, _i32, _vp]),
    "gcl_assemble_input_tail": (C.c_int, [_vp, _vp, _vp, _vp, _i32, _vp, _i64, _i32, _i32, _i32, _i32, _i32, _vp]),
    "gcl_wmse_fwd_bwd": (C.c_int, [_vp, _i64, _i64, _vp, _i64, _i64, _vp, _i64, _i64, _vp, _vp, _f32, _f32, _vp,
                                   _vp, _vp, _vp, _i32, _i32, _i32, _vp, _sz, _vp]),
    "gcl_ar_step_bwd": (C.c_int, [_vp, _vp, _vp, _vp, _i32, _i32, _vp, _vp, _i32, _i32, _i32, _i32, _vp]),
    "gcl_pad_rows": (C.c_int, [_vp, _i64, _i64, _i32, _i32, _vp, _i64, _i64, _i32, _i32, _i32, _vp]),
    "gcl_zero": (C.c_int, [_vp, _sz, _vp]),
    "gcl_wmse_ws_bytes": (_sz, [_i32, _i32, _i32]),
    "gcl_adam_step": (C.c_int, [_vp, _vp, _vp, _vp, _i64, _f32, _f32, _f32, _f32, _f32, _i32, _f32, _vp]),
    "gcl_adam_step_dev": (C.c_int, [_vp, _vp, _vp, _vp, _i64, _f32, _f32, _f32, _f32, _f32, _vp, _vp, _f32, _vp]),
    "gcl_adam_step_groups": (C.c_int, [_vp, _vp, _vp, _vp, _i64, _vp, _i32, _vp, _vp, _vp, _vp, _f32, _f32, _f32, _f32,
                                       _f32, _vp]),
    "gcl_copy_rows": (C.c_int, [_vp, _i64, _i64, _vp, _i64, _i64, _i32, _i32, _i32, _vp]),
    "gcl_dense_fwd": (C.c_int, [_vp, _i64, _i32, _vp, _vp, _i64, _vp, _vp, _i64, _vp, _i64, _i64, _i32, _i32, _vp]),
    "gcl_dense_bwd_dx": (C.c_int, [_vp, _i64, _vp, _i64, _vp, _i64, _i32, _vp, _vp, _vp, _i64, _vp, _i64, _i64, _i32, _i32,
                                   _vp, C.c_size_t, _vp]),
    "gcl_dense_bwd_dw": (C.c_int, [_vp, _i64, _vp, _i64, _i32, _vp, _vp, _i64, _vp, _i64, _i32, _i32, _i32, _vp,
                                   C.c_size_t, _vp]),
    "gcl_gcn_layer_fwd": (C.c_int, [_vp, _vp, _i64, _i64, _i32, _vp, _vp, _vp, _vp, _i64, _i64, _i32, _i32, _i32, _i32, _vp]),
    "gcl_gcn_layer_fwd_rows": (C.c_int, [_vp, _vp, _i64, _i64, _i32, _vp, _vp, _vp, _vp, _i64, _i64, _i32, _i32, _i32, _i32, _i32, _vp]),
    "gcl_layernorm_fwd_map": (C.c_int, [_vp, _i64, _vp, _vp, _f32, _vp, _i64, _i64, _vp, _i32, _vp, _i64, _i32, _vp]),
    "gcl_gcn_layer_fwd_tab": (C.c_int, [_vp, _vp, _i64, _i64, _i64, _vp, _i32, _vp, _vp, _vp, _vp, _i64, _i64, _i32, _i32, _i32, _i32, _vp]),
    "gcl_gcn_layer_fwd_tab_ok": (C.c_int, [_vp, _i64, _i64, _i64, _i32, _i32, _i32]),
    "gcl_segment_reduce": (C.c_int, [_vp, _i64, _i64, _vp, _vp, _i32, _vp, _i64, _i64, _i32, _i32, _i32, _vp]),
    "gcl_edge_combine": (C.c_int, [_vp, _vp, _vp, _i64, _i64, _vp, _vp, _vp, _i64, _i64, _vp, _vp, _i32, _i64, _i32, _vp]),
    "gcl_act_fwd": (C.c_int, [_vp, _vp, _i64, _i32, _vp, _vp]),
    "gcl_act_bwd": (C.c_int, [_vp, _vp, _vp, _i64, _i32, _vp, _vp, _vp, C.c_size_t, _vp]),
    "gcl_act_bwd_ws_bytes": (C.c_size_t, []),
    "gcl_window_pack": (C.c_int, [_vp, _i64, _i32, _i32, _i32, _vp, _vp, _vp, _i32, _i32, _i32, _vp, _vp, _i32, _vp]),
    "gcl_ar_advance": (C.c_int, [_vp, _vp, _i64, _i64, _vp, _i64, _i64, _vp, _vp, _vp, _i64, _i64, _i32, _i32, _i32, _i32,
                                 _i32, _i32, _vp]),
    "gcl_gather2_rows": (C.c_int, [_vp, _i64, _i64, _vp, _vp, _i64, _i64, _vp, _vp, _i64, _i64, _i32, _i32, _i32, _i32, _vp]),
    "gcl_roi_gather_rows": (C.c_int, [_vp, _i32, _i32] + [_vp, _i64, _i64, _i32] * 3 + [_vp, _i64, _i64, _i32, _i32, _vp]),
    "gcl_roi_compose": (C.c_int, [_vp, _i64, _i64, _vp, _i64, _i64, _vp, _vp, _i64, _i64, _i32, _i32, _i32, _vp]),
    "gcl_segment_wsum": (C.c_int, [_vp, _i64, _i64, _i32, _i32, _vp, _vp, _vp, _vp, _i64, _i64, _vp, _i64, _i64, _i32,
                                   _i32, _i32, _i32, _vp]),
    "gcl_cross_update_fwd": (C.c_int, [_vp, _i64, _i64, _vp, _i64, _i64, _vp, _vp, _vp, _f32, _vp, _vp, _vp, _i32, _i32,
                                       _i32, _vp]),
    "gcl_nudge": (C.c_int, [_vp, _i64, _i64, _vp, _i64, _i64, _vp, _f32, _f32, _i32, _vp, _i64, _i64, _i32, _i32, _i32,
                            _vp]),
    "gcl_oi_max_stations": (C.c_int, []),
    "gcl_oi_station_cov": (C.c_int, [_vp, _vp, _i32, C.c_double, C.c_double, C.c_double, _vp, _vp]),
    "gcl_oi_factor": (C.c_int, [_vp, _i32, _vp]),
    "gcl_oi_solve": (C.c_int, [_vp, _i32, _vp, _vp, _vp, _i32, _vp]),
    "gcl_oi_innovation": (C.c_int, [_vp, _i64, _i64, _vp, _i64, _i64, _vp, _vp, _vp, _i32, _i32, _i32, _vp, _vp]),
    "gcl_oi_analysis": (C.c_int, [_vp, _i64, _i64, _vp, _i64, _i64, _vp, _i32, _vp, _vp, _vp, _vp, _i32, _vp, _vp, _vp,
                                  _vp, _i32, _f32, _f32, _f32, _f32, _i32, _vp]),
    "gcl_verify_colstats_ws_bytes": (_sz, [_i32, _i32, _i32, _i32]),
    "gcl_verify_colstats": (C.c_int, [_vp, _i64, _i64, _i32, _i32] + [_vp, _i64, _i64, _vp] * 4
                            + [_vp, _i32, _i32, _vp, _vp, _sz, _vp]),
    "gcl_verify_accumulate": (C.c_int, [_vp, _vp, _i32, _vp, _vp, _vp]),
    "gcl_regrid_blend": (C.c_int, [_vp, _i32, _i64, _i64, _i32, _vp, _vp, _i32, _i32, _vp, _i64, _i64, _vp, _vp, _i64,
                                   _i64, _vp, _i64, _i64, _i32, _vp]),
    "gcl_taper_blend": (C.c_int, [_vp, _vp, _i64, _i64, _vp, _i64, _i64, _vp, _i64, _i64, _i32, _i32, _i32, _vp]),
    "gcl_mos_forest_eval": (C.c_int, [_vp, _vp, _i32, C.c_double, _vp, _i32, _vp, _vp]),
    "gcl_mos_forest_predict": (C.c_int, [_vp, _vp, _i32, C.c_double, _vp, _i32, _i64, _i64, _i64, _i32] + [_i32] * 5
                               + [_vp, _vp, _i32, _i32, _vp, _vp, _vp, _vp, _i32, _vp]),
    "gcl_mos_idw_apply": (C.c_int, [_vp, _i32, _i64, _i64, _i64, _vp, _i64, _i64, _i64, _i32, _i32, _i32, _i32, _vp,
                                    _vp, _vp, _i32, _vp, _i32, C.c_double, C.c_double, _vp, _i32, _vp]),
    "gcl_mos_table_apply": (C.c_int, [_vp, _i32, _i64, _i64, _i64, _vp, _i64, _i64, _i64, _i32, _i32, _i32, _i32, _vp,
                                      _i32, _i32, _vp]),
    "gcl_multires_window_pack": (C.c_int, [_vp, _i64, _i32, _i32, _i32, _vp, _i64, _i32, _i32, _i32, _vp, _i32, _i32, _vp,
                                           _vp, _vp, _i64, _i64, _vp, _vp, _i32, _i32, _i32, _i32, _i32, _vp, _vp, _i32,
                                           _vp]),
    "gcl_pipeline_roi_phys": (C.c_int, [_vp, _i64, _vp, _i64, _vp, _i32, _i32, _i32, _vp, _vp, _i32, _i32, C.c_double,
                                        _i32, _vp, _vp, _vp]),
    "gcl_pipeline_lapse": (C.c_int, [_vp, _vp, _i32, _i32, _i32, _i32, _i32, C.c_double, _i32, _vp]),
    "gcl_pipeline_station_obs": (C.c_int, [_vp, _i64, _vp, _i32, _i32, _i32, _vp, _vp]),
    "gcl_pipeline_sqerr": (C.c_int, [_vp, _i64, _i64, _i32, _vp, _i64, _vp, _i32, _i32, _i32, _i32, _i32, _vp, _vp, _vp]),
}


def exported_symbols():
# ... 283 lines not shown
    a = _act_of(act, in_slope)
    if a == ACT_SILU:
        if db is not None and bool(acc_db) != bool(acc_dW):
            dense_bwd_dw(dy, x, dW, None, acc_dW, a, None)
            colsum(dy, db, acc_db)
        else:
            dense_bwd_dw(dy, x, dW, db, acc_dW, a, None)
        dx = dense_bwd_dx(dy, W, x, a, None, None)
        if colsum_dx is not None:
            colsum(dx, colsum_dx, acc_colsum)
        return dx
    rows, Fout = dy.shape
    Fin = W.shape[1]
    dx = torch.empty(rows, Fin, dtype=torch.float32, device=dy.device)
    nb = lib().gcl_linear_bwd_all_ws_bytes(rows, Fin, Fout)
    acc = (ACC_DW if acc_dW else 0) | (ACC_DB if acc_db else 0) | (ACC_COLSUM if acc_colsum else 0)
    d = _deferred
    if d.active:
        dests = {t.data_ptr() for t in (dW, db, colsum_dx) if t is not None}
        if dests & d.dests:
            defer_flush(close=False)
        ws = d.ws(nb, dy.device)
        job = ReduceJob()
        _check(lib().gcl_linear_bwd_all_deferred(
            _p(dy), _ld(dy), _p(W), _p(x), _ld(x), _p(in_slope), _p(d_in_slope), _p(dx), Fin, _p(dW), _p(db),
            _p(colsum_dx), rows, Fin, Fout, acc, ws.data_ptr(), ws.numel(), _stream(), C.byref(job)))
        if job.nparts > 0:
            d.jobs.append(job)
            d.dests |= dests
            d.keep.append((dW, db, colsum_dx, d_in_slope, ws))
        else:
            d.used -= 1
        return dx
    ws = workspace(nb, dy.device)
    _check(lib().gcl_linear_bwd_all(
        _p(dy), _ld(dy), _p(W), _p(x), _ld(x), _p(in_slope), _p(d_in_slope), _p(dx), Fin, _p(dW), _p(db),
        _p(colsum_dx), rows, Fin, Fout, acc, ws.data_ptr(), ws.numel(), _stream()))
    return dx


def aggregate(graph: Graph, h3, bias, transpose=False, out=None):
    B, n, F = h3.shape
    assert n == graph.n, f"graph has {graph.n} nodes, features have {n} rows"
    assert h3.stride(2) == 1
    if out is None:
        out = torch.empty(B, n, F, dtype=torch.float32, device=h3.device)
    tok = _probe_begin("aggregate", graph=graph, transpose=bool(transpose), B=B, F=F)
    _check(lib().gcl_aggregate(graph.handle, 1 if transpose else 0, _p(h3), h3.stride(1), h3.stride(0), _p(bias),
                               _p(out), out.stride(1), out.stride(0), B, F, _stream()))
    _probe_end(tok)
    return out


def layernorm_fwd(x, gamma, beta, eps=1e-5):
    rows, F = x.shape
    y = torch.empty(rows, F, dtype=torch.float32, device=x.device)
    stats = torch.empty(rows, 2, dtype=torch.float32, device=x.device)
    _check(lib().gcl_layernorm_fwd(_p(x), _ld(x), _p(gamma), _p(beta), float(eps), _p(y), F, _p(stats), rows, F, _stream()))
    return y, stats


def layernorm_fwd_map(x, gamma, beta, eps, out3, pos):
    rows, F = x.shape
    n_per = pos.numel()
    assert out3.stride(2) == 1 and rows % n_per == 0 and out3.shape[0] == rows // n_per
    stats = torch.empty(rows, 2, dtype=torch.float32, device=x.device)
    _check(lib().gcl_layernorm_fwd_map(_p(x), _ld(x), _p(gamma), _p(beta), float(eps), _p(out3), out3.stride(1), out3.stride(0),
                                       _pi(pos), n_per, _p(stats), rows, F, _stream()))
    return stats


def layernorm_bwd(dy, x, gamma, stats, dgamma, dbeta, accumulate: bool, colsum_dx=None, acc_colsum: bool = False,
                  dy_map=None):
    rows, F = x.shape
    dx = torch.empty(rows, F, dtype=torch.float32, device=x.device)
    nb = lib().gcl_layernorm_bwd_ws_bytes(rows, F)
    ws = workspace(nb, x.device)
    acc = (ACC_DW if accumulate else 0) | (ACC_COLSUM if acc_colsum else 0)
    if dy_map is not None:
        src3, pos = dy_map
        assert src3.stride(2) == 1 and src3.shape[2] >= F and rows % pos.numel() == 0 and src3.shape[0] == rows // pos.numel()
        _check(lib().gcl_layernorm_bwd_map(_p(src3), src3.stride(1), src3.stride(0), _pi(pos), pos.numel(), _p(x), _ld(x),
                                           _p(gamma), _p(stats), _p(dx), F, _p(dgamma), _p(dbeta), _p(colsum_dx), acc, rows, F,
                                           ws.data_ptr(), ws.numel(), _stream()))
        return dx
    _check(lib().gcl_layernorm_bwd_cs(_p(dy), _ld(dy), _p(x), _ld(x), _p(gamma), _p(stats), _p(dx), F, _p(dgamma),
                                      _p(dbeta), _p(colsum_dx), acc, rows, F, ws.data_ptr(), ws.numel(), _stream()))
    return dx


def graphnorm_fwd(x3, gamma, beta, eps=1e-5):
    B, n, F = x3.shape
    y = torch.empty(B, n, F, dtype=torch.float32, device=x3.device)
    stats = torch.empty(B, 2, dtype=torch.float32, device=x3.device)
    nb = lib().gcl_graphnorm_ws_bytes(B, n, F)
    ws = workspace(nb, x3.device)
    _check(lib().gcl_graphnorm_fwd(_p(x3), x3.stride(1), x3.stride(0), _p(gamma), _p(beta), float(eps), _p(y), F, n * F,
                                   _p(stats), B, n, F, ws.data_ptr(), ws.numel(), _stream()))
    return y, stats


def graphnorm_bwd(dy3, x3, gamma, stats, dgamma, dbeta, accumulate: bool, eps=1e-5):
    B, n, F = x3.shape
    dx = torch.empty(B, n, F, dtype=torch.float32, device=x3.device)
    nb = lib().gcl_graphnorm_ws_bytes(B, n, F)
    ws = workspace(nb, x3.device)
    _check(lib().gcl_graphnorm_bwd(_p(dy3), dy3.stride(1), dy3.stride(0), _p(x3), x3.stride(1), x3.stride(0), _p(gamma),
                                   _p(stats), float(eps), _p(dx), F, n * F, _p(dgamma), _p(dbeta),
                                   1 if accumulate else 0, B, n, F, ws.data_ptr(), ws.numel(), _stream()))
    return dx


def colsum(x, out, accumulate: bool):
    rows, F = x.shape
    nb = lib().gcl_colsum_ws_bytes(rows, F)
    ws = workspace(nb, x.device)
    _check(lib().gcl_colsum(_p(x), _ld(x), rows, F, _p(out), 1 if accumulate else 0, ws.data_ptr(), ws.numel(), _stream()))
    return out


def gat_tab_ok(graph: Graph, H: int, Cc: int) -> bool:
    return bool(lib().gcl_gat_tab_ok(graph.handle, H * Cc, int(H), int(Cc)))


def gat_fwd(graph: Graph, h3, att_src, att_dst, bias, H, Cc, need_alpha=True, tab=None):
    B, n, HC = h3.shape
    if tab is not None:
        n = graph.n
        assert h3.is_contiguous()
    dev = h3.device
    a_s = torch.empty(B, n, H, dtype=torch.float32, device=dev)
    a_d = torch.empty(B, n, H, dtype=torch.float32, device=dev)
    alpha = torch.empty(B, graph.e, H, dtype=torch.float32, device=dev) if need_alpha else None
    y = torch.empty(B, n, Cc, dtype=torch.float32, device=dev)
    tok = _probe_begin("gat_fwd", graph=graph, B=B, H=H, C=Cc, alpha=need_alpha)
    if tab is not None:
        _check(lib().gcl_gat_fwd_tab(graph.handle, _p(h3), h3.stride(1), h3.stride(0), _pi(tab), _p(att_src), _p(att_dst),
                                     _p(bias), _p(a_s), _p(a_d), _p(alpha), _p(y), Cc, n * Cc, B, H, Cc, _stream()))
# ... 250 lines not shown
        out3 = torch.empty(B, E, D, dtype=torch.float32, device=(A3 if ref is None else ref).device)
    _check(lib().gcl_edge_combine(
        _p(base3), _p(extra3), _p(A3), A3.stride(1) if A3 is not None else 0, A3.stride(0) if A3 is not None else 0,
        _pi(ia), _p(sa), _p(C3), C3.stride(1) if C3 is not None else 0, C3.stride(0) if C3 is not None else 0, _pi(ic),
        _p(out3), B, E, D, _stream()))
    return out3


def act_fwd(x, act, slope=None):
    y = torch.empty_like(x)
    assert x.is_contiguous()
    _check(lib().gcl_act_fwd(_p(x), _p(y), x.numel(), int(act), _p(slope), _stream()))
    return y


def act_bwd(x, dy, act, slope=None, d_slope=None):
    assert x.is_contiguous() and dy.is_contiguous()
    dx = torch.empty_like(x)
    ws = workspace(lib().gcl_act_bwd_ws_bytes(), x.device)
    _check(lib().gcl_act_bwd(_p(x), _p(dy), _p(dx), x.numel(), int(act), _p(slope), _p(d_slope), ws.data_ptr(), ws.numel(),
                             _stream()))
    return dx


def window_pack(series, t0, mean, std, C: int, obs: int, pred: int, out=None):
    assert series.is_cuda and series.dtype == torch.float16 and series.is_contiguous()
    assert t0.is_cuda and t0.dtype == torch.int64 and t0.is_contiguous()
    if series.dim() == 3:
        T, n_lon, Ct = series.shape
        n_lat = 1
    else:
        T, n_lon, n_lat, Ct = series.shape
    B, G = t0.numel(), n_lon * n_lat
    if out is not None:
        X, Y = out
        assert X.is_contiguous() and X.shape == (B, G, obs * C) and X.dtype == torch.float32 and X.device == series.device
        assert pred == 0 or (Y.is_contiguous() and Y.shape == (B, G, pred * C) and Y.dtype == torch.float32)
    else:
        X = torch.empty(B, G, obs * C, dtype=torch.float32, device=series.device)
        Y = torch.empty(B, G, pred * C, dtype=torch.float32, device=series.device) if pred > 0 else None
    _check(lib().gcl_window_pack(series.data_ptr(), T, n_lon, n_lat, Ct, t0.data_ptr(), _p(mean), _p(std), C, obs, pred,
                                 _p(X), _p(Y), B, _stream()))
    return X, Y


def gcn_layer_fusable(graph: Graph, x3, Fin: int, Fout: int) -> bool:
    import os
    if os.environ.get("GCL_FUSED_GCN", "1") in ("0",):
        return False
    return (Fin % 4 == 0 and 4 <= Fin <= 64 and 1 <= Fout <= 64 and graph.max_in_degree <= 64 and graph.kind in (GRAPH_GCN, GRAPH_MEAN)
            and x3.stride(2) == 1 and x3.stride(1) % 4 == 0 and x3.stride(0) % 4 == 0 and x3.data_ptr() % 16 == 0)


def gcn_layer_fwd(graph: Graph, x3, act, slope, W, bias, out=None, rows_out=None):
    B, n, Fin = x3.shape
    assert n == graph.n
    Fout = W.shape[0]
    Fst = (Fout + 3) // 4 * 4
    if out is None:
        out = torch.empty(B, n, Fst, dtype=torch.float32, device=x3.device)
    assert out.shape[2] >= Fst or out.stride(1) >= Fst
    tok = _probe_begin("gcn_layer_fwd", graph=graph, B=B, Fin=Fin, Fout=Fout)
    _check(lib().gcl_gcn_layer_fwd_rows(graph.handle, _p(x3), x3.stride(1), x3.stride(0), int(act), _p(slope),
                                        _p(W.contiguous()), _p(bias), _p(out), out.stride(1), out.stride(0), B, Fin, Fout,
                                        Fst, int(rows_out) if rows_out else n, _stream()))
    _probe_end(tok)
    return out[..., :Fout]


def gcn_layer_tab_ok(graph: Graph, x3, Fout: int) -> bool:
    B, nx, Fin = x3.shape
    return bool(lib().gcl_gcn_layer_fwd_tab_ok(graph.handle, x3.stride(1), x3.stride(0), B * nx, B, Fin, int(Fout)))


def gcn_layer_fwd_tab(graph: Graph, x3, tab, act, slope, W, bias):
    B, nx, Fin = x3.shape
    assert x3.is_contiguous() and tab.dtype == torch.int32 and tab.numel() == graph.n
    Fout = W.shape[0]
    Fst = (Fout + 3) // 4 * 4
    out = torch.empty(B, graph.n, Fst, dtype=torch.float32, device=x3.device)
    tok = _probe_begin("gcn_layer_fwd", graph=graph, B=B, Fin=Fin, Fout=Fout)
    _check(lib().gcl_gcn_layer_fwd_tab(graph.handle, _p(x3), x3.stride(1), x3.stride(0), B * nx, _pi(tab), int(act), _p(slope),
                                       _p(W.contiguous()), _p(bias), _p(out), out.stride(1), out.stride(0), B, Fin, Fout, Fst,
                                       _stream()))
    _probe_end(tok)
    return out[..., :Fout]


def _pd(t: torch.Tensor):
    assert t.is_cuda and t.dtype == torch.float64 and t.is_contiguous()
    return t.data_ptr()


def nudge(f3, o3, out3, c0: float, c1: float, form: int, chan_mask=None):
    B, G, Cc = f3.shape
    assert o3.shape == f3.shape and out3.shape == f3.shape
    assert f3.stride(2) == 1 and o3.stride(2) == 1 and out3.stride(2) == 1
    if chan_mask is not None:
        assert chan_mask.is_cuda and chan_mask.dtype == torch.uint8 and chan_mask.numel() == Cc
    _check(lib().gcl_nudge(_p(f3), f3.stride(1), f3.stride(0), _p(o3), o3.stride(1), o3.stride(0),
                           chan_mask.data_ptr() if chan_mask is not None else None, float(c0), float(c1), int(form),
                           _p(out3), out3.stride(1), out3.stride(0), B, G, Cc, _stream()))
    return out3


def oi_max_stations() -> int:
    return int(lib().gcl_oi_max_stations())


def oi_factor(lat, lon, sb2: float, rl2: float, diag: float):
    m = lat.numel()
    M = torch.empty(m, m, dtype=torch.float64, device=lat.device)
    _check(lib().gcl_oi_station_cov(_pd(lat), _pd(lon), m, float(sb2), float(rl2), float(diag), M.data_ptr(), _stream()))
    _check(lib().gcl_oi_factor(M.data_ptr(), m, _stream()))
# ... 163 lines not shown
```

graphcast-lite_amd/models.py:

```python
import contextlib
import math
import os
import sys
from collections import OrderedDict
from typing import Optional, Tuple

import numpy as np
import torch
import torch.nn as nn

from . import hip
from .config import (
    DataConfig,
    GraphBlock,
    GraphBuildingConfig,
    GraphLayerType,
    MLPBlock,
    ModelConfig,
    PipelineConfig,
)
from .create_graphs import (create_decoding_graph, create_encoding_graph, create_processing_graph,
                            create_product_graph)
from .functional import (AssembleFn, EdgeLayout, GATLayerFn, Gather2Fn, GCNStackFn, GradLanding, GraphNormFn, InteractionNetFn,
                         LatSource, LayerNormFn, MeanAggFn, MeshLatFn, MLPFn)
# ... 650 lines not shown

    def _forward_compact(self, X: torch.Tensor, attention_threshold=0.0, **kwargs):
        G, M = self._num_grid_nodes, self._num_mesh_nodes
        squeeze = X.dim() == 2 or (X.dim() == 3 and X.shape[0] == 1)
        X3 = X if X.dim() == 3 else X.unsqueeze(0)
        B = X3.shape[0]
        if self.use_product_graph:
            X3 = self._product_stage(X3)
        c = getattr(self, "_compact", None) or self._compact_setup(X3.device)
        if self._fold_invariant_rows:
            f = c.fold.get(B) or self._fold_setup(c, B, X3.device)
            if self._mlp_on_folded_rows and self.encoder.mlp is not None and f.rd > 0:
                x_m = AssembleFn.apply(X3, self.init_grid_features, f.mstat2, f.x_tail2)
                h_m = self.encoder.mlp(X=x_m)
                x_g = MeshLatFn.apply(h_m, f.maps_e, f.ne, G + f.r, f.rd, None)
                enc_c = self.encoder.graph_layer(X=x_g, edge_index=c.enc_graph)
            else:
                x_c = AssembleFn.apply(X3, self.init_grid_features, f.mstat, f.x_fold if f.r > 0 else None)
                enc_c = self.encoder.forward(X=x_c, edge_index=c.enc_graph)
            land = GradLanding(G) if kwargs.pop("_landing", False) and self._grad_landing else None
            lat_src = self._lat_source(c, f, enc_c, land)
            if lat_src is None:
                mesh_lat = MeshLatFn.apply(enc_c, f.maps, M, G + c.Md, f.r, land)
            maps_dec = f.maps_dec
        else:
            kwargs.pop("_landing", None)
            land = None
            lat_src = None
            maps_dec = c.maps_dec
            x_c = AssembleFn.apply(X3, self.init_grid_features, c.mstat_dep)
            enc_c = self.encoder.forward(X=x_c, edge_index=c.enc_graph)
            inv = self.encoder.forward(X=c.x_inv, edge_index=c.empty_graph) if c.Mi > 0 else None
            mesh_lat = Gather2Fn.apply(enc_c, inv, c.maps_mesh, M, B)
        if self.using_sparse_gat:
            pg = self._processing_graph_tiled() if c.perm is not None else self.processing_graph
            if land is not None and self._ln_into_decoder_input and self._latents_discarded and not squeeze:
                land.dec_buf = torch.empty(B, G + c.U, enc_c.shape[-1], dtype=torch.float32, device=enc_c.device)
                land.dec_map = maps_dec[3]
            processed, new_edge_index = self.processor.forward(
                X=mesh_lat, edge_index=pg, attention_threshold=attention_threshold,
                **({"_grad_src": land} if land is not None else {}), **kwargs)
            self.processing_graph = self._processing_graph_from_tiled(new_edge_index) if c.perm is not None else new_edge_index
        elif self.using_interaction_net:
            processed = self.processor.forward(X=mesh_lat, edge_index=self.processing_graph,
                                               attention_threshold=attention_threshold,
                                               edge_attr=self._processing_edge_features)
        else:
            pg = self._processing_graph_tiled() if c.perm is not None else self.processing_graph
            if (land is not None and self._ln_into_decoder_input and self._latents_discarded
                    and self.processor.graph_layer.layer_type in (GraphLayerType.ConvGCN, GraphLayerType.GATConv)
                    and not squeeze):
                land.dec_buf = torch.empty(B, G + c.U, enc_c.shape[-1], dtype=torch.float32, device=enc_c.device)
                land.dec_map = maps_dec[3]
            if lat_src is not None:
                processed = self.processor.forward(X=enc_c, edge_index=pg, attention_threshold=attention_threshold,
                                                   _lat_src=lat_src, **({"_grad_src": land} if land is not None else {}))
            else:
                processed = self.processor.forward(X=mesh_lat, edge_index=pg, attention_threshold=attention_threshold,
                                                   **({"_grad_src": land} if land is not None else {}))
        dec_in = Gather2Fn.apply(enc_c, processed, maps_dec, G + c.U, B, land)
        gcn_dec = self.decoder.graph_layer.layer_type == GraphLayerType.ConvGCN
        decoded = self.decoder.forward(X=dec_in, edge_index=c.dec_graph, **({"_out_rows": G} if gcn_dec else {}))
        out, grid_lat = (decoded if gcn_dec else decoded[:, :G, :]), enc_c[:, :G, :]
        if c.perm is not None and not self._want_prediction_only:
            pos_dev = getattr(c, "perm_pos_dev", None)
            if pos_dev is None or pos_dev.device != processed.device:
                pos_dev = c.perm_pos_dev = c.perm[1].to(processed.device)
            processed = processed.index_select(1, pos_dev)
        if squeeze:
            return out[0], grid_lat[0], processed[0]
        return out, grid_lat, processed

    _lat_through_table = os.environ.get("GCL_NO_LAT_TABLE", "0") in ("0", "")
    _mlp_on_folded_rows = os.environ.get("GCL_NO_MLP_FOLD", "0") in ("0", "")
    _ln_into_decoder_input = os.environ.get("GCL_NO_LN_MAP", "0") in ("0", "")
    _latents_discarded = False

    def _lat_source(self, c, f, enc_c, land):
        if not self._lat_through_table or c.perm is None or self.processor.mlp is not None:
            return None
        gl = self.processor.graph_layer
        if gl.layer_type == GraphLayerType.GATConv:
            first = gl.layers[0]
            if not isinstance(first, GATConv) or first.heads != 1 or enc_c.dim() != 3 or first.lin.weight.shape[1] != enc_c.shape[-1]:
                return None
            g = _graphs.get(self._processing_graph_tiled(), self._num_mesh_nodes, hip.GRAPH_GAT)
            if not hip.gat_tab_ok(g, 1, first.lin.weight.shape[0]):
                return None
            return LatSource(f.tab, f.maps, self._num_mesh_nodes, self._num_grid_nodes, c.Md, f.r, land)
        if gl.layer_type != GraphLayerType.ConvGCN:
            return None
        convs = [m for m in gl.layers if isinstance(m, GCNConv)]
        if not convs or enc_c.dim() != 3 or convs[0].lin.weight.shape[1] != enc_c.shape[-1]:
            return None
        g = _graphs.get(self._processing_graph_tiled(), self._num_mesh_nodes, hip.GRAPH_GCN)
        if not hip.gcn_layer_tab_ok(g, enc_c, convs[0].lin.weight.shape[0]):
            return None
        return LatSource(f.tab, f.maps, self._num_mesh_nodes, self._num_grid_nodes, c.Md, f.r, land)

    _want_prediction_only = False

    def forward_with_latents(self, X: torch.Tensor, attention_threshold=0.0, **kwargs):
        landing = kwargs.pop("_landing", False)
        self._want_prediction_only = landing
        if self._compact_eligible():
            return self._forward_compact(X, attention_threshold, _landing=landing, **kwargs)
# ... 37 lines not shown
```

include/gcl.h:

```cpp
#ifndef GCL_H
#define GCL_H

#include <stddef.h>
#include <stdint.h>

#ifdef __cplusplus
extern "C" {
#endif

#define GCL_VERSION 100

#define GCL_OK 0
#define GCL_EINVAL (-1)
#define GCL_EHIP (-2)
#define GCL_ENOMEM (-3)
#define GCL_EUNSUPPORTED (-4)

typedef struct gcl_graph gcl_graph_t;
typedef void* gcl_stream_t;

int gcl_version(void);
const char* gcl_last_error(void);

#define GCL_GRAPH_GCN 0
// ... 23 lines not shown
                      const float* in_slope, float* d_in_slope, float* dx, int64_t lddx,
                      int64_t rows, int32_t Fin, int32_t Fout, void* ws, size_t ws_bytes,
                      gcl_stream_t stream);
int gcl_linear_bwd_dw(const float* dy, int64_t lddy, const float* x, int64_t ldx,
                      const float* in_slope, float* dW, float* db, int64_t rows, int32_t Fin,
                      int32_t Fout, int32_t accumulate, void* ws, size_t ws_bytes,
                      gcl_stream_t stream);
size_t gcl_linear_bwd_ws_bytes(int64_t rows, int32_t Fin, int32_t Fout);
#define GCL_ACC_DW 1
#define GCL_ACC_DB 2
#define GCL_ACC_COLSUM 4
int gcl_linear_bwd_all(const float* dy, int64_t lddy, const float* W, const float* x, int64_t ldx,
                       const float* in_slope, float* d_in_slope, float* dx, int64_t lddx, float* dW,
                       float* db, float* colsum_dx, int64_t rows, int32_t Fin, int32_t Fout,
                       int32_t accumulate, void* ws, size_t ws_bytes, gcl_stream_t stream);
size_t gcl_linear_bwd_all_ws_bytes(int64_t rows, int32_t Fin, int32_t Fout);

typedef struct gcl_reduce_job {
  const float* part;
  int64_t pstride;
  struct {
    float* out;
    int32_t poff, count, pld, cols, ldo, acc;
  } seg[3];
  const double* spart;
  float* sout;
  int32_t nparts, ns;
} gcl_reduce_job;
int gcl_linear_bwd_all_deferred(const float* dy, int64_t lddy, const float* W, const float* x, int64_t ldx,
                                const float* in_slope, float* d_in_slope, float* dx, int64_t lddx, float* dW,
                                float* db, float* colsum_dx, int64_t rows, int32_t Fin, int32_t Fout,
                                int32_t accumulate, void* ws, size_t ws_bytes, gcl_stream_t stream,
                                gcl_reduce_job* job);
int gcl_reduce_jobs(const gcl_reduce_job* jobs, int32_t n, gcl_stream_t stream);

#define GCL_ACT_NONE 0
#define GCL_ACT_PRELU 1
#define GCL_ACT_SILU 2
int gcl_dense_fwd(const float* x, int64_t ldx, int32_t act, const float* slope, const float* W,
                  int64_t ldw, const float* bias, const float* addend, int64_t ldadd, float* y,
                  int64_t ldy, int64_t rows, int32_t Fin, int32_t Fout, gcl_stream_t stream);
int gcl_dense_bwd_dx(const float* dy, int64_t lddy, const float* W, int64_t ldw, const float* z,
                     int64_t ldz, int32_t act, const float* slope, float* d_slope,
                     const float* addend, int64_t ldadd, float* dx, int64_t lddx, int64_t rows,
                     int32_t Fin, int32_t Fout, void* ws, size_t ws_bytes, gcl_stream_t stream);
int gcl_dense_bwd_dw(const float* dy, int64_t lddy, const float* x, int64_t ldx, int32_t act,
                     const float* slope, float* dW, int64_t lddw, float* db, int64_t rows,
                     int32_t Fin, int32_t Fout, int32_t accumulate, void* ws, size_t ws_bytes,
                     gcl_stream_t stream);

int gcl_aggregate(const gcl_graph_t* g, int32_t transpose, const float* h, int64_t ldh, int64_t bsh,
                  const float* bias, float* y, int64_t ldy, int64_t bsy, int32_t B, int32_t F,
                  gcl_stream_t stream);

int gcl_gat_fwd(const gcl_graph_t* g, const float* h, int64_t ldh, int64_t bsh,
                const float* att_src , const float* att_dst , const float* bias ,
                float* a_src , float* a_dst , float* alpha ,
                float* y, int64_t ldy, int64_t bsy, int32_t B, int32_t H, int32_t C,
                gcl_stream_t stream);
int gcl_gat_bwd(const gcl_graph_t* g, const float* dy, int64_t lddy, int64_t bsdy,
                const float* h, int64_t ldh, int64_t bsh, const float* att_src, const float* att_dst,
                const float* a_src, const float* a_dst, const float* alpha,
                float* dh, int64_t lddh, int64_t bsdh, float* d_att_src, float* d_att_dst,
                float* d_bias, int32_t accumulate, int32_t B, int32_t H, int32_t C,
                void* ws, size_t ws_bytes, gcl_stream_t stream);
size_t gcl_gat_bwd_ws_bytes(int64_t e_prime, int32_t n, int32_t B, int32_t H, int32_t C);
int gcl_gat_fwd_tab(const gcl_graph_t* g, const float* h, int64_t ldh, int64_t bsh, const int32_t* tab ,
                    const float* att_src, const float* att_dst, const float* bias, float* a_src, float* a_dst,
                    float* alpha, float* y, int64_t ldy, int64_t bsy, int32_t B, int32_t H, int32_t C,
                    gcl_stream_t stream);
int gcl_gat_bwd_tab(const gcl_graph_t* g, const float* dy, int64_t lddy, int64_t bsdy, const float* h, int64_t ldh,
                    int64_t bsh, const int32_t* tab , const float* att_src, const float* att_dst,
                    const float* a_src, const float* a_dst, const float* alpha, float* dh, int64_t lddh, int64_t bsdh,
                    float* d_att_src, float* d_att_dst, float* d_bias, int32_t accumulate, int32_t B, int32_t H,
                    int32_t C, void* ws, size_t ws_bytes, gcl_stream_t stream);
int gcl_gat_tab_ok(const gcl_graph_t* g, int64_t ldh, int32_t H, int32_t C);
int gcl_gat_alpha_to_edge_order(const gcl_graph_t* g, const float* alpha_slots, float* alpha_edges,
                                int32_t H, gcl_stream_t stream);
int gcl_gat_prune(const gcl_graph_t* g, const float* alpha_edges, float threshold,
                  int64_t* edge_index_out, int64_t* kept, void* ws, size_t ws_bytes,
                  gcl_stream_t stream);
size_t gcl_gat_prune_ws_bytes(int64_t e_prime);

int gcl_layernorm_fwd(const float* x, int64_t ldx, const float* gamma, const float* beta, float eps,
                      float* y, int64_t ldy, float* stats, int64_t rows, int32_t F,
                      gcl_stream_t stream);
int gcl_layernorm_fwd_map(const float* x, int64_t ldx, const float* gamma, const float* beta, float eps, float* y,
                          int64_t ldy, int64_t bsy, const int32_t* pos , int32_t n_per, float* stats,
                          int64_t rows, int32_t F, gcl_stream_t stream);
int gcl_layernorm_bwd(const float* dy, int64_t lddy, const float* x, int64_t ldx, const float* gamma,
                      const float* stats, float* dx, int64_t lddx, float* dgamma, float* dbeta,
                      int32_t accumulate, int64_t rows, int32_t F, void* ws, size_t ws_bytes,
                      gcl_stream_t stream);
int gcl_layernorm_bwd_cs(const float* dy, int64_t lddy, const float* x, int64_t ldx, const float* gamma,
                         const float* stats, float* dx, int64_t lddx, float* dgamma, float* dbeta,
                         float* colsum_dx, int32_t accumulate, int64_t rows, int32_t F, void* ws,
                         size_t ws_bytes, gcl_stream_t stream);
int gcl_layernorm_bwd_map(const float* dy, int64_t lddy, int64_t bsdy, const int32_t* pos, int32_t n_per,
                          const float* x, int64_t ldx, const float* gamma, const float* stats, float* dx,
                          int64_t lddx, float* dgamma, float* dbeta, float* colsum_dx, int32_t accumulate,
                          int64_t rows, int32_t F, void* ws, size_t ws_bytes, gcl_stream_t stream);
size_t gcl_layernorm_bwd_ws_bytes(int64_t rows, int32_t F);
int gcl_graphnorm_fwd(const float* x, int64_t ldx, int64_t bsx, const float* gamma, const float* beta,
                      float eps, float* y, int64_t ldy, int64_t bsy, float* stats, int32_t B,
                      int32_t n, int32_t F, void* ws, size_t ws_bytes, gcl_stream_t stream);
int gcl_graphnorm_bwd(const float* dy, int64_t lddy, int64_t bsdy, const float* x, int64_t ldx,
                      int64_t bsx, const float* gamma, const float* stats, float eps, float* dx,
                      int64_t lddx, int64_t bsdx, float* dgamma, float* dbeta, int32_t accumulate,
                      int32_t B, int32_t n, int32_t F, void* ws, size_t ws_bytes, gcl_stream_t stream);
size_t gcl_graphnorm_ws_bytes(int32_t B, int32_t n, int32_t F);

int gcl_colsum(const float* x, int64_t ldx, int64_t rows, int32_t F, float* out, int32_t accumulate,
               void* ws, size_t ws_bytes, gcl_stream_t stream);
size_t gcl_colsum_ws_bytes(int64_t rows, int32_t F);

int gcl_assemble_input(const float* x , const float* grid_static ,
                       const float* mesh_static , float* out, int64_t ldo, int32_t B,
                       int32_t G, int32_t M, int32_t Cdyn, int32_t Cs, gcl_stream_t stream);
int gcl_assemble_input_tail(const float* x, const float* grid_static, const float* mesh_static, const float* tail,
                            int32_t r, float* out, int64_t ldo, int32_t B, int32_t G, int32_t M, int32_t Cdyn,
                            int32_t Cs, gcl_stream_t stream);

int gcl_wmse_fwd_bwd(const float* delta, int64_t ldd, int64_t bsd, const float* x_last, int64_t ldx,
                     int64_t bsx, const float* y, int64_t ldy_, int64_t bsy, const float* node_w,
                     const float* chan_w, float inv_wsum, float grad_scale, float* d_delta,
                     float* out_state, const float* loss_prev, float* loss_out, int32_t B, int32_t G,
                     int32_t C, void* ws, size_t ws_bytes, gcl_stream_t stream);
size_t gcl_wmse_ws_bytes(int32_t B, int32_t G, int32_t C);

int gcl_adam_step(float* p, const float* g, float* m, float* v, int64_t count, float lr, float beta1,
                  float beta2, float eps, float weight_decay, int32_t step, float grad_scale,
                  gcl_stream_t stream);

int gcl_adam_step_dev(float* p, const float* g, float* m, float* v, int64_t count, float lr, float beta1,
                      float beta2, float eps, float weight_decay, int32_t* step_dev, float* bc_dev,
                      float grad_scale, gcl_stream_t stream);

int gcl_adam_step_groups(float* p, const float* g, float* m, float* v, int64_t count, const int32_t* chunk_param,
                         int32_t num_params, const int32_t* active, const float* lr, int32_t* step, float* bc,
                         float beta1, float beta2, float eps, float weight_decay, float grad_scale,
                         gcl_stream_t stream);

int gcl_copy_rows(const float* src, int64_t lds, int64_t bss, float* dst, int64_t ldd, int64_t bsd,
                  int32_t B, int32_t rows, int32_t F, gcl_stream_t stream);

int gcl_gcn_layer_fwd(const gcl_graph_t* g, const float* x, int64_t ldx, int64_t bsx, int32_t act,
                      const float* slope, const float* W , const float* bias, float* y,
                      int64_t ldy, int64_t bsy, int32_t B, int32_t Fin, int32_t Fout, int32_t Fout_store,
                      gcl_stream_t stream);
int gcl_gcn_layer_fwd_rows(const gcl_graph_t* g, const float* x, int64_t ldx, int64_t bsx, int32_t act,
                           const float* slope, const float* W , const float* bias, float* y,
                           int64_t ldy, int64_t bsy, int32_t B, int32_t Fin, int32_t Fout, int32_t Fout_store,
                           int32_t rows_out, gcl_stream_t stream);
int gcl_gcn_layer_fwd_tab(const gcl_graph_t* g, const float* x, int64_t ldx, int64_t bsx, int64_t x_rows,
                          const int32_t* tab , int32_t act, const float* slope, const float* W ,
                          const float* bias, float* y, int64_t ldy, int64_t bsy, int32_t B, int32_t Fin, int32_t Fout,
                          int32_t Fout_store, gcl_stream_t stream);
int gcl_gcn_layer_fwd_tab_ok(const gcl_graph_t* g, int64_t ldx, int64_t bsx, int64_t x_rows, int32_t B, int32_t Fin,
                             int32_t Fout);

int gcl_segment_reduce(const float* src, int64_t ld_src, int64_t bs_src, const int32_t* perm,
                       const int32_t* rowptr , int32_t mean, float* out, int64_t ld_out,
                       int64_t bs_out, int32_t B, int32_t n, int32_t D, gcl_stream_t stream);
int gcl_edge_combine(const float* base, const float* extra, const float* A, int64_t lda, int64_t bsa,
                     const int32_t* ia, const float* sa, const float* C, int64_t ldc, int64_t bsc,
                     const int32_t* ic, float* out, int32_t B, int64_t E, int32_t D,
                     gcl_stream_t stream);
int gcl_act_fwd(const float* x, float* y, int64_t count, int32_t act, const float* slope,
                gcl_stream_t stream);
int gcl_act_bwd(const float* x, const float* dy, float* dx, int64_t count, int32_t act,
                const float* slope, float* d_slope, void* ws, size_t ws_bytes, gcl_stream_t stream);
size_t gcl_act_bwd_ws_bytes(void);

int gcl_window_pack(const uint16_t* series , int64_t T, int32_t n_lon, int32_t n_lat,
                    int32_t Ct, const int64_t* t0, const float* mean, const float* stdv, int32_t C,
                    int32_t obs, int32_t pred, float* X , float* Y ,
                    int32_t B, gcl_stream_t stream);

int gcl_ar_advance(const float* state, const float* delta, int64_t ldd, int64_t bsd, const float* y_step,
                   int64_t ldy, int64_t bsy, const int32_t* chan_kind, float* new_state, float* out,
                   int64_t ldo, int64_t bso, int32_t out_off, int32_t B, int32_t G, int32_t obs, int32_t C,
                   int32_t residual, gcl_stream_t stream);
int gcl_ar_step_bwd(const float* dd, const float* g_loss, const float* g_new, const int32_t* chan_kind,
                    int32_t has_y, int32_t residual, float* d_delta, float* d_state, int32_t B, int32_t G,
                    int32_t obs, int32_t C, gcl_stream_t stream);

int gcl_pad_rows(const float* src, int64_t lds, int64_t bss, int32_t rows_src, int32_t F_src, float* dst,
                 int64_t ldd, int64_t bsd, int32_t rows_dst, int32_t F_dst, int32_t B, gcl_stream_t stream);
int gcl_zero(void* ptr, size_t nbytes, gcl_stream_t stream);

int gcl_gather2_rows(const float* a, int64_t lda, int64_t bsa, const int32_t* map_a, const float* b,
                     int64_t ldb, int64_t bsb, const int32_t* map_b, float* dst, int64_t ldd, int64_t bsd,
                     int32_t B, int32_t nd, int32_t F, int32_t sum_batch, gcl_stream_t stream);

int gcl_roi_gather_rows(const int32_t* rows, int32_t n, int32_t rows_src, const float* s0, int64_t ld0,
                        int64_t bs0, int32_t w0, const float* s1, int64_t ld1, int64_t bs1, int32_t w1,
                        const float* s2, int64_t ld2, int64_t bs2, int32_t w2, float* dst, int64_t ldd,
                        int64_t bsd, int32_t Fp, int32_t B, gcl_stream_t stream);
int gcl_roi_compose(const float* pred, int64_t ldp, int64_t bsp, const float* corr, int64_t ldc, int64_t bsc,
                    const int32_t* pos, float* out, int64_t ldo, int64_t bso, int32_t B, int32_t G, int32_t C,
                    gcl_stream_t stream);

int gcl_segment_wsum(const float* src, int64_t ld_src, int64_t bs_src, int32_t n_src, int32_t act,
                     const int32_t* idx, const float* w, const int32_t* rowptr, const float* addend,
                     int64_t ld_add, int64_t bs_add, float* out, int64_t ld_out, int64_t bs_out,
                     int32_t accumulate, int32_t B, int32_t n, int32_t D, gcl_stream_t stream);
// ... 82 lines not shown
```

Before: 24670.

## Add presence-masked aggregation and GCN layer paths to skip absent rows

Adds a presence table to the aggregate, heavy-row, halo and GCN layer kernels so that neighbours or rows marked absent are read from a shared zero page instead of the feature matrix. New map-skip layernorm forward and backward entry points and a decoder row list let the model avoid writing or normalising rows that are later overwritten. The intent is to cut the HBM traffic and work spent on rows whose values are not needed. In exchange every gather now does an extra present[] lookup, and presence launches pin the iteration count, ignoring the env override.

```diff
diff --git a/graphcast-lite_amd/csrc/aggregate.hip b/graphcast-lite_amd/csrc/aggregate.hip
--- a/graphcast-lite_amd/csrc/aggregate.hip
+++ b/graphcast-lite_amd/csrc/aggregate.hip
@@ -2,17 +2,19 @@
 
 #include "common.h"
 #include "halo.h"
+#include "mfma_io.h"
 
 namespace {
 
-template <int LPR, bool VL, bool VS, int EW, int ITER>
+template <int LPR, bool VL, bool VS, int EW, int ITER, bool PRES = false>
 __global__ __launch_bounds__(256) void agg_kernel(const int32_t* __restrict__ rowptr, const int32_t* __restrict__ col,
                                                   const float* __restrict__ w, const int32_t* __restrict__ ecol,
                                                   const float* __restrict__ ew, const float* __restrict__ H,
                                                   int64_t ldh, int64_t bsh, const float* __restrict__ bias,
                                                   float* __restrict__ Y, int64_t ldy, int64_t bsy, int32_t n,
                                                   int32_t B, int32_t F, int32_t nRB, int32_t xcd_map,
-                                                  int32_t nt_store, const int32_t* __restrict__ order16) {
+                                                  int32_t nt_store, const int32_t* __restrict__ order16,
+                                                  const int32_t* __restrict__ present = nullptr) {
   constexpr int RPW = 64 / LPR;
   constexpr int EL = LPR < gcl::kEll ? LPR : gcl::kEll;
   static_assert(EW <= EL, "ELL width exceeds the lanes of a row group");
@@ -53,6 +55,7 @@
 
   auto ld4 = [&](int j, float& x0, float& x1, float& x2, float& x3) {
     const float* p = Hb + (int64_t)j * ldh + cc;
+    if (PRES) p = j >= 0 ? p : reinterpret_cast<const float*>(gcl::mfma_io::zero4);
     if (VL) {
       const float4 v = *reinterpret_cast<const float4*>(p);
       x0 = v.x; x1 = v.y; x2 = v.z; x3 = v.w;
@@ -71,6 +74,7 @@
     end = rowptr[rc + 1];
     cj = ecol[(int64_t)rc * gcl::kEll + (l & (EL - 1))];
     wj = ew[(int64_t)rc * gcl::kEll + (l & (EL - 1))];
+    if (PRES) cj = present[cj] >= 0 ? cj : -1;
   };
   int start, end, cj;
   float wj;
@@ -115,6 +119,7 @@
         if (mine < end) {
           oj = col[mine];
           ow = w[mine];
+          if (PRES) oj = present[oj] >= 0 ? oj : -1;
         }
         const int cnt = min(LPR, end - base);
         for (int k = 0; k < cnt; k += 4) {
@@ -161,13 +166,14 @@
   }
 }
 
-template <int LPR, bool VL, bool VS>
+template <int LPR, bool VL, bool VS, bool PRES = false>
 __global__ __launch_bounds__(256) void agg_heavy_kernel(const int32_t* __restrict__ rows_heavy,
                                                         const int32_t* __restrict__ rowptr,
                                                         const int32_t* __restrict__ col, const float* __restrict__ w,
                                                         const float* __restrict__ H, int64_t ldh, int64_t bsh,
                                                         const float* __restrict__ bias, float* __restrict__ Y,
-                                                        int64_t ldy, int64_t bsy, int32_t F) {
+                                                        int64_t ldy, int64_t bsy, int32_t F,
+                                                        const int32_t* __restrict__ present = nullptr) {
   constexpr int NG = 256 / LPR;
   __shared__ float red[NG][LPR * 4 + 1];
   const int row = rows_heavy[blockIdx.x];
@@ -181,6 +187,7 @@
   float a0 = 0.f, a1 = 0.f, a2 = 0.f, a3 = 0.f;
   auto ld4 = [&](int j, float& x0, float& x1, float& x2, float& x3) {
     const float* p = Hb + (int64_t)j * ldh + cc;
+    if (PRES) p = present[j] >= 0 ? p : reinterpret_cast<const float*>(gcl::mfma_io::zero4);
     if (VL) {
       const float4 v = *reinterpret_cast<const float4*>(p);
       x0 = v.x; x1 = v.y; x2 = v.z; x3 = v.w;
@@ -246,14 +253,15 @@
 #define GCL_AGG_STAMP(i)
 #endif
 
-template <int LPR, int T, int MAXPW>
+template <int LPR, int T, int MAXPW, bool PRES = false>
 __global__ __launch_bounds__(256) void agg_halo_loop_kernel(const int32_t* __restrict__ list, const int32_t* __restrict__ cnt,
                                                             const int2* __restrict__ rec, const int32_t* __restrict__ rowptr,
                                                             const int32_t* __restrict__ opos, const float* __restrict__ w,
                                                             int32_t smax, const float* __restrict__ H, int64_t ldh,
                                                             int64_t bsh, const float* __restrict__ bias,
                                                             float* __restrict__ Y, int64_t ldy, int64_t bsy, int32_t n,
-                                                            int32_t B, int32_t F, int32_t ntiles, int32_t nt_store) {
+                                                            int32_t B, int32_t F, int32_t ntiles, int32_t nt_store,
+                                                            const int32_t* __restrict__ present = nullptr) {
   extern __shared__ float4 img[];
   constexpr int RPW = 64 / LPR;
   constexpr int NW = 4;
@@ -300,11 +308,13 @@
         const int jr = tl[e0 + r];
         j = sub == r ? jr : j;
       }
-      jj[q] = j;
+      jj[q] = (PRES && present[j] < 0) ? -1 : j;
     }
   };
   int jj[MAXPW], nhalo = 0, tile = -1;
   int2 rc[NIT];
+  bool own[PRES ? NIT : 1];
+  const char* const zpage = reinterpret_cast<const char*>(gcl::mfma_io::zero4);
 #ifdef GCL_STAMPS
   unsigned long long st_acc[8] = {0, 0, 0, 0, 0, 0, 0, 0}, st_last = __builtin_amdgcn_s_memtime();
 #endif
@@ -317,6 +327,13 @@
     if (newtile) {
       tile = tnew;
       fetch_list(tile, jj, nhalo);
+      if (PRES) {
+#pragma unroll
+        for (int it = 0; it < NIT; ++it) {
+          const int row = tile * T + wave * (T / NW) + sub + it * RPW;
+          own[it] = present[row < n ? row : n - 1] >= 0;
+        }
+      }
     }
     GCL_AGG_STAMP(0)
     const char* Hc = reinterpret_cast<const char*>(H + (int64_t)b * bsh);
@@ -326,6 +343,7 @@
     for (int it = 0; it < NIT; ++it) {
       const int row = row0 + it * RPW;
       const char* src = Hc + (__umul24(row < n ? row : n - 1, ldb) + cb);
+      if (PRES) src = own[PRES ? it : 0] ? src : zpage;
       __builtin_amdgcn_global_load_lds((gcl_gptr_t)src, (gcl_lptr_t)(img + (wave * (T / NW) + it * RPW) * LPR), 16, 0, 0);
     }
 #pragma unroll
@@ -333,6 +351,7 @@
       const int p = wave + NW * q;
       if (p < nhalo) {
         const char* src = Hc + (__umul24(jj[q], ldb) + cb);
+        if (PRES) src = jj[q] >= 0 ? src : zpage;
         __builtin_amdgcn_global_load_lds((gcl_gptr_t)src, (gcl_lptr_t)(img + (T + p * RPW) * LPR), 16, 0, 0);
       }
     }
@@ -435,7 +454,8 @@
 
 template <int LPR>
 int launch_agg_halo(const AggArgs& ga, const float* h, int64_t ldh, int64_t bsh, const float* bias, float* y,
-                    int64_t ldy, int64_t bsy, int32_t n, int32_t B, int32_t F, hipStream_t st) {
+                    int64_t ldy, int64_t bsy, int32_t n, int32_t B, int32_t F, hipStream_t st,
+                    const int32_t* present = nullptr) {
   const int enabled = gcl::env_int("GCL_AGG_HALO", 1);
   static const int force_t = gcl::env_int("GCL_AGG_HALO_T", 0);
   static const int bpc_env = gcl::env_int("GCL_AGG_HALO_BPC", 0);
@@ -461,11 +481,17 @@
   auto go = [&](auto kern) -> int {
     GCL_ENSURE_DYN_LDS(kern, (size_t)lds);
     hipLaunchKernelGGL(kern, grid, block, (size_t)lds, st, hl->list, hl->cnt, reinterpret_cast<const int2*>(hl->rec),
-                       ga.rowptr, hl->opos, ga.w, hl->smax, h, ldh, bsh, bias, y, ldy, bsy, n, B, F, hl->ntiles, nt);
+                       ga.rowptr, hl->opos, ga.w, hl->smax, h, ldh, bsh, bias, y, ldy, bsy, n, B, F, hl->ntiles, nt, present);
     return GCL_OK;
   };
   int rc;
-  if (hl->T == 64)
+  if (present && hl->T == 64)
+    rc = mpw <= 4 ? go(&agg_halo_loop_kernel<LPR, 64, 4, true>) : mpw <= 8 ? go(&agg_halo_loop_kernel<LPR, 64, 8, true>)
+       : mpw <= 16 ? go(&agg_halo_loop_kernel<LPR, 64, 16, true>) : go(&agg_halo_loop_kernel<LPR, 64, 32, true>);
+  else if (present)
+    rc = mpw <= 4 ? go(&agg_halo_loop_kernel<LPR, 32, 4, true>) : mpw <= 8 ? go(&agg_halo_loop_kernel<LPR, 32, 8, true>)
+       : mpw <= 16 ? go(&agg_halo_loop_kernel<LPR, 32, 16, true>) : go(&agg_halo_loop_kernel<LPR, 32, 32, true>);
+  else if (hl->T == 64)
     rc = mpw <= 4 ? go(&agg_halo_loop_kernel<LPR, 64, 4>) : mpw <= 8 ? go(&agg_halo_loop_kernel<LPR, 64, 8>)
        : mpw <= 16 ? go(&agg_halo_loop_kernel<LPR, 64, 16>) : go(&agg_halo_loop_kernel<LPR, 64, 32>);
   else
@@ -478,11 +504,24 @@
 
 template <int LPR>
 int launch_agg_heavy(const AggArgs& ga, const float* h, int64_t ldh, int64_t bsh, const float* bias, float* y,
-                     int64_t ldy, int64_t bsy, int32_t B, int32_t F, bool vl, bool vs, hipStream_t st) {
+                     int64_t ldy, int64_t bsy, int32_t B, int32_t F, bool vl, bool vs, hipStream_t st,
+                     const int32_t* present = nullptr) {
   dim3 hgrid((unsigned)ga.n_heavy, (unsigned)B), block(256);
+  if (present) {
+#define GCL_AGGH(VL_, VS_)                                                                                       \
+  hipLaunchKernelGGL((agg_heavy_kernel<LPR, VL_, VS_, true>), hgrid, block, 0, st, ga.heavy, ga.rowptr, ga.col, ga.w, \
+                     h, ldh, bsh, bias, y, ldy, bsy, F, present)
+    if (vl && vs) GCL_AGGH(true, true);
+    else if (vl) GCL_AGGH(true, false);
+    else if (vs) GCL_AGGH(false, true);
+    else GCL_AGGH(false, false);
+#undef GCL_AGGH
+    GCL_CHECK_LAUNCH();
+    return GCL_OK;
+  }
 #define GCL_AGGH(VL_, VS_)                                                                                       \
   hipLaunchKernelGGL((agg_heavy_kernel<LPR, VL_, VS_>), hgrid, block, 0, st, ga.heavy, ga.rowptr, ga.col, ga.w, h, \
-                     ldh, bsh, bias, y, ldy, bsy, F)
+                     ldh, bsh, bias, y, ldy, bsy, F, (const int32_t*)nullptr)
   if (vl && vs) GCL_AGGH(true, true);
   else if (vl) GCL_AGGH(true, false);
   else if (vs) GCL_AGGH(false, true);
@@ -494,17 +533,17 @@
 
 template <int LPR>
 int launch_agg(const AggArgs& ga, const float* h, int64_t ldh, int64_t bsh, const float* bias, float* y, int64_t ldy,
-               int64_t bsy, int32_t n, int32_t B, int32_t F, hipStream_t st) {
+               int64_t bsy, int32_t n, int32_t B, int32_t F, hipStream_t st, const int32_t* present = nullptr) {
   constexpr int RPW = 64 / LPR;
   constexpr int EL = LPR < gcl::kEll ? LPR : gcl::kEll;
   const bool vl = (ldh % 4 == 0) && (bsh % 4 == 0) && gcl::aligned16(h) && ldh >= ((F + 3) / 4) * 4;
   const bool vs = (ldy % 4 == 0) && (bsy % 4 == 0) && gcl::aligned16(y) && (F % 4 == 0);
   if constexpr (LPR >= 16) {
     if (vl && vs && (!bias || gcl::aligned16(bias))) {
-      const int hr = launch_agg_halo<LPR>(ga, h, ldh, bsh, bias, y, ldy, bsy, n, B, F, st);
+      const int hr = launch_agg_halo<LPR>(ga, h, ldh, bsh, bias, y, ldy, bsy, n, B, F, st, present);
       if (hr >= 0) {
         if (hr != GCL_OK || ga.n_heavy == 0) return hr;
-        return launch_agg_heavy<LPR>(ga, h, ldh, bsh, bias, y, ldy, bsy, B, F, true, true, st);
+        return launch_agg_heavy<LPR>(ga, h, ldh, bsh, bias, y, ldy, bsy, B, F, true, true, st, present);
       }
     }
   }
@@ -514,8 +553,8 @@
   int ewidth = ew_env > 0 ? ew_env : ga.ell_width;
   if (ewidth > EL) ewidth = EL;
   ewidth = ewidth >= 8 ? 8 : ewidth >= 4 ? 4 : ewidth >= 2 ? 2 : 1;
-  const int iter = (iter_env == 1 || iter_env == 2 || iter_env == 4 || iter_env == 8) ? iter_env
-                                                                                       : (ewidth >= 4 ? 1 : 2);
+  const int iter = (!present && (iter_env == 1 || iter_env == 2 || iter_env == 4 || iter_env == 8)) ? iter_env
+                                                                                                     : (ewidth >= 4 ? 1 : 2);
   int32_t nRB = (int32_t)gcl::cdiv(n, RPW * 4 * iter);
   if (ga.order16 && RPW * 4 * iter <= 16) nRB = ga.n_order16 * (16 / (RPW * 4 * iter));
   const int xcd_map = B >= gcl::kNumXCD ? 1 : 0;
@@ -525,9 +564,16 @@
   const int32_t* order16 = (RPW * 4 * iter <= 16) ? ga.order16 : nullptr;
 #define GCL_AGG4(VL_, VS_, EW_, IT_)                                                                             \
   hipLaunchKernelGGL((agg_kernel<LPR, VL_, VS_, EW_, IT_>), grid, block, 0, st, ga.rowptr, ga.col, ga.w, ga.ecol, \
-                     ga.ew, h, ldh, bsh, bias, y, ldy, bsy, n, B, F, nRB, xcd_map, nt, order16)
+                     ga.ew, h, ldh, bsh, bias, y, ldy, bsy, n, B, F, nRB, xcd_map, nt, order16, (const int32_t*)nullptr)
+#define GCL_AGGP(VL_, VS_, EW_, IT_)                                                                                   \
+  hipLaunchKernelGGL((agg_kernel<LPR, VL_, VS_, EW_, IT_, true>), grid, block, 0, st, ga.rowptr, ga.col, ga.w, ga.ecol, \
+                     ga.ew, h, ldh, bsh, bias, y, ldy, bsy, n, B, F, nRB, xcd_map, nt, order16, present)
 #define GCL_AGG3(VL_, VS_, EW_)              \
   do {                                       \
+    if (present) {                           \
+      if (EW_ >= 4) GCL_AGGP(VL_, VS_, EW_, 1); \
+      else GCL_AGGP(VL_, VS_, EW_, 2);       \
+    } else                                   \
     if (iter == 8) GCL_AGG4(VL_, VS_, EW_, 8); \
     else if (iter == 4) GCL_AGG4(VL_, VS_, EW_, 4); \
     else if (iter == 2) GCL_AGG4(VL_, VS_, EW_, 2); \
@@ -547,16 +593,17 @@
 #undef GCL_AGG2
 #undef GCL_AGG3
 #undef GCL_AGG4
+#undef GCL_AGGP
   GCL_CHECK_LAUNCH();
-  if (ga.n_heavy > 0) return launch_agg_heavy<LPR>(ga, h, ldh, bsh, bias, y, ldy, bsy, B, F, vl, vs, st);
+  if (ga.n_heavy > 0) return launch_agg_heavy<LPR>(ga, h, ldh, bsh, bias, y, ldy, bsy, B, F, vl, vs, st, present);
   return GCL_OK;
 }
 
 }
 
-extern "C" int gcl_aggregate(const gcl_graph_t* g, int32_t transpose, const float* h, int64_t ldh, int64_t bsh,
-                             const float* bias, float* y, int64_t ldy, int64_t bsy, int32_t B, int32_t F,
-                             gcl_stream_t stream) {
+static int aggregate_impl(const gcl_graph_t* g, int32_t transpose, const float* h, int64_t ldh, int64_t bsh,
+                          const int32_t* present, const float* bias, float* y, int64_t ldy, int64_t bsy, int32_t B,
+                          int32_t F, gcl_stream_t stream) {
   GCL_CHECK_ARG(g && h && y, "aggregate: null argument");
   GCL_CHECK_ARG(B > 0 && F > 0 && F <= 256, "aggregate: unsupported B=%d F=%d (F must be in 1..256)", B, F);
   GCL_CHECK_ARG(ldh >= F && ldy >= F, "aggregate: leading dimension smaller than F");
@@ -577,9 +624,22 @@
   GCL_CHECK_ARG(B <= 65535 || ga.n_heavy == 0, "aggregate: batch too large for the heavy-row launch");
   hipStream_t st = (hipStream_t)stream;
   const int lanes = (F + 3) / 4;
-  if (lanes <= 4) return launch_agg<4>(ga, h, ldh, bsh, bias, y, ldy, bsy, g->n, B, F, st);
-  if (lanes <= 8) return launch_agg<8>(ga, h, ldh, bsh, bias, y, ldy, bsy, g->n, B, F, st);
-  if (lanes <= 16) return launch_agg<16>(ga, h, ldh, bsh, bias, y, ldy, bsy, g->n, B, F, st);
-  if (lanes <= 32) return launch_agg<32>(ga, h, ldh, bsh, bias, y, ldy, bsy, g->n, B, F, st);
-  return launch_agg<64>(ga, h, ldh, bsh, bias, y, ldy, bsy, g->n, B, F, st);
-}
+  if (lanes <= 4) return launch_agg<4>(ga, h, ldh, bsh, bias, y, ldy, bsy, g->n, B, F, st, present);
+  if (lanes <= 8) return launch_agg<8>(ga, h, ldh, bsh, bias, y, ldy, bsy, g->n, B, F, st, present);
+  if (lanes <= 16) return launch_agg<16>(ga, h, ldh, bsh, bias, y, ldy, bsy, g->n, B, F, st, present);
+  if (lanes <= 32) return launch_agg<32>(ga, h, ldh, bsh, bias, y, ldy, bsy, g->n, B, F, st, present);
+  return launch_agg<64>(ga, h, ldh, bsh, bias, y, ldy, bsy, g->n, B, F, st, present);
+}
+
+extern "C" int gcl_aggregate(const gcl_graph_t* g, int32_t transpose, const float* h, int64_t ldh, int64_t bsh,
+                             const float* bias, float* y, int64_t ldy, int64_t bsy, int32_t B, int32_t F,
+                             gcl_stream_t stream) {
+  return aggregate_impl(g, transpose, h, ldh, bsh, nullptr, bias, y, ldy, bsy, B, F, stream);
+}
+
+extern "C" int gcl_aggregate_present(const gcl_graph_t* g, int32_t transpose, const float* h, int64_t ldh, int64_t bsh,
+                                     const int32_t* present, const float* bias, float* y, int64_t ldy, int64_t bsy,
+                                     int32_t B, int32_t F, gcl_stream_t stream) {
+  GCL_CHECK_ARG(present, "aggregate_present: null presence table");
+  return aggregate_impl(g, transpose, h, ldh, bsh, present, bias, y, ldy, bsy, B, F, stream);
+}
diff --git a/graphcast-lite_amd/csrc/gcn_layer.hip b/graphcast-lite_amd/csrc/gcn_layer.hip
--- a/graphcast-lite_amd/csrc/gcn_layer.hip
+++ b/graphcast-lite_amd/csrc/gcn_layer.hip
@@ -563,13 +563,15 @@
     if (s < nks) acc = __builtin_amdgcn_mfma_f32_32x32x16_bf16(ah[s], wf.f[s][0], acc, 0, 0, 0);
 }
 
-template <int ACT, int MAXPW, int STAUX = 0, bool DIRECT = false, bool INTER = false, bool TAB = false>
+template <int ACT, int MAXPW, int STAUX = 0, bool DIRECT = false, bool INTER = false, bool TAB = false, bool PRED = false>
 __global__ __launch_bounds__(256, 3) void gcn_halo_fwd_kernel(
     const int32_t* __restrict__ list, const int32_t* __restrict__ cnt, const int2* __restrict__ rec,
     const int32_t* __restrict__ rowptr, const int32_t* __restrict__ opos, const float* __restrict__ w, int32_t smax,
     const float* __restrict__ X, int64_t ldx, int64_t bsx, const float* __restrict__ slope_p, const float* __restrict__ W,
     const float* __restrict__ bias, float* __restrict__ Y, int64_t ldy, int64_t bsy, int32_t n, int32_t B, int32_t K,
-    int32_t N, int32_t Nst, int32_t ntiles, const int32_t* __restrict__ tab = nullptr) {
+    int32_t N, int32_t Nst, int32_t ntiles, const int32_t* __restrict__ tab = nullptr,
+    const int32_t* __restrict__ present = nullptr) {
+  static_assert(!PRED || DIRECT, "the row predicate is folded into the direct stores");
   using gcl::halo::glds16;
   using gcl::halo::row_bcast;
   extern __shared__ __align__(16) float smem[];
@@ -581,6 +583,7 @@
   float* At = smem;
   float* imgf = At + 2 * AtF;
   float4* img = reinterpret_cast<float4*>(imgf);
+  int* ptab = reinterpret_cast<int*>(imgf + (size_t)(smax + 1) * 64);
   const int lane = threadIdx.x & 63;
   const int wave = __builtin_amdgcn_readfirstlane(threadIdx.x >> 6);
   const int sub = lane >> 4, l = lane & 15, c0 = l * 4;
@@ -617,8 +620,13 @@
   int jj[MAXPW], nhalo = 0, tile = -1;
   int own[TAB ? NIT : 1];
   int2 rc[NIT];
+  int pv = 0;
   auto new_tile = [&](int t) {
     tile = t;
+    if (PRED) {
+      const int row = t * T + wave * 16 + (lane & 15);
+      pv = present[row < n ? row : n - 1];
+    }
     nhalo = cnt[t] / RPW;
     const int32_t* __restrict__ tl = list + (int64_t)t * hstride;
 #pragma unroll
@@ -674,6 +682,7 @@
     }
   };
   new_tile(m / nsamp);
+  if (PRED && lane < 16) ptab[(tile & 1) * 64 + wave * 16 + lane] = pv;
 #pragma unroll
   for (int it = 0; it < NIT; ++it) asm volatile("" : "+v"(rc[it].x), "+v"(rc[it].y));
   if (TAB) {
@@ -755,9 +764,10 @@
     __builtin_amdgcn_s_barrier();
     GCL_STAMP(2);
     const bool more = m + 1 < mend;
+    bool fresh = false;
     if (more) {
       const int tn = (m + 1) / nsamp;
-      if (tn != tile) new_tile(tn);
+      if (tn != tile) { new_tile(tn); fresh = true; }
       if (!INTER) stage(m + 1);
       else if (TAB) Xn = reinterpret_cast<const char*>(X), sbn = (unsigned)(xcd + gcl::kNumXCD * (m + 1 - tile * nsamp)) * (unsigned)bsx * 4u;
       else Xn = reinterpret_cast<const char*>(X + (int64_t)(xcd + gcl::kNumXCD * (m + 1 - tile * nsamp)) * bsx);
@@ -785,9 +795,16 @@
       const __amdgpu_buffer_rsrc_t ry = make_rsrc(Yb, nr > 0 ? ((int64_t)(nr - 1) * ldy + Nst) * 4 : 0);
       const unsigned cofs = col < Nst ? (unsigned)col * 4u : kOOB;
       const unsigned ldyb = (unsigned)ldy * 4u;
+      if (PRED && fresh && lane < 16) ptab[(tile & 1) * 64 + wave * 16 + lane] = pv;
+      const int4* pt4 = reinterpret_cast<const int4*>(ptab + ((trow >> 6) & 1) * 64 + pair * 32 + 4 * (lane >> 5));
 #pragma unroll
       for (int r = 0; r < 16; ++r) {
-        const unsigned off = (unsigned)d_row(r, lane) * ldyb + cofs;
+        unsigned off = (unsigned)d_row(r, lane) * ldyb + cofs;
+        if (PRED) {
+          const int4 e = pt4[2 * (r >> 2)];
+          const int er = (r & 3) == 0 ? e.x : (r & 3) == 1 ? e.y : (r & 3) == 2 ? e.z : e.w;
+          off = er >= 0 ? off : kOOB;
+        }
         __builtin_amdgcn_raw_buffer_store_b32(__builtin_bit_cast(unsigned, acc[r] + bcol), ry, off, 0, STAUX);
       }
       GCL_STAMP(6);
@@ -830,7 +847,7 @@
 static int halo_layer_launch(const gcl_graph_t* g, const float* x, int64_t ldx, int64_t bsx, const int32_t* tab,
                              int64_t x_rows, int32_t act, const float* slope, const float* W, const float* bias, float* y,
                              int64_t ldy, int64_t bsy, int32_t B, int32_t Fin, int32_t Fout, int32_t Fout_store,
-                             int32_t rows_out, hipStream_t st, bool* launched) {
+                             int32_t rows_out, hipStream_t st, bool* launched, const int32_t* present = nullptr) {
   *launched = false;
   const int32_t n = g->n;
   const int halo_on = gcl::env_int("GCL_GCN_HALO", 1);
@@ -838,7 +855,7 @@
   const gcl_halo& hl = g->halo[0][0];
   const int hp4 = hl.T == 64 ? (int)gcl::cdiv((hl.smax - 64) / 4, 4) : 99;
   const int KPh = Fin + 2;
-  const size_t ldsh = (size_t)2 * (32 * KPh > 2048 ? 32 * KPh : 2048) * 4 + (size_t)(hl.smax + 1) * 256;
+  const size_t ldsh = (size_t)2 * (32 * KPh > 2048 ? 32 * KPh : 2048) * 4 + (size_t)(hl.smax + 1) * 256 + (present ? 512 : 0);
   const bool offs_ok = tab ? (x_rows * ldx * 4 < ((int64_t)1 << 32) && (int64_t)B * bsx * 4 < ((int64_t)1 << 32) && x_rows < (1 << 24))
                            : ((int64_t)n * ldx * 4 < ((int64_t)1 << 31));
   if (!(halo_on && x3_on && g->kind == GCL_GRAPH_GCN && g->n_heavy == 0 && hl.T == 64 && hp4 <= 8 && Fin % 16 == 0 && Fin > 32 && rows_out == n &&
@@ -846,6 +863,7 @@
         (int64_t)n * ldy * 4 < ((int64_t)1 << 31)))
     return GCL_OK;
   if (tab && hp4 > 4) return GCL_OK;
+  if (present && (tab || hp4 > 4 || !gcl::env_int("GCL_GCN_HALO_FORM", 1))) return GCL_OK;
   static const int bpc_env = gcl::env_int("GCL_GCN_HALO_BPC", 0);
   const int per_cu = (int)(gcl::kLdsBytes / ldsh);
   const int Jx = 32 * (bpc_env > 0 ? bpc_env : per_cu);
@@ -854,12 +872,16 @@
     GCL_ENSURE_DYN_LDS(kern, ldsh);
     hipLaunchKernelGGL(kern, grid, dim3(256), ldsh, st, hl.list, hl.cnt, reinterpret_cast<const int2*>(hl.rec), g->rowptr,
                        hl.opos, g->w, hl.smax, x, ldx, bsx, slope, W, bias, y, ldy, bsy, n, B, Fin, Fout, Fout_store,
-                       hl.ntiles, tab);
+                       hl.ntiles, tab, present);
     return GCL_OK;
   };
   int rc;
   const int form_env = gcl::env_int("GCL_GCN_HALO_FORM", 1);
-  if (tab)
+  if (present)
+    rc = act == GCL_ACT_PRELU  ? go(&gcn_halo_fwd_kernel<gcl::kActPrelu, 4, 2, true, true, false, true>)
+         : act == GCL_ACT_SILU ? go(&gcn_halo_fwd_kernel<gcl::kActSilu, 4, 2, true, true, false, true>)
+                               : go(&gcn_halo_fwd_kernel<gcl::kActNone, 4, 2, true, true, false, true>);
+  else if (tab)
     rc = act == GCL_ACT_PRELU  ? go(&gcn_halo_fwd_kernel<gcl::kActPrelu, 4, 2, true, true, true>)
          : act == GCL_ACT_SILU ? go(&gcn_halo_fwd_kernel<gcl::kActSilu, 4, 2, true, true, true>)
                                : go(&gcn_halo_fwd_kernel<gcl::kActNone, 4, 2, true, true, true>);
@@ -889,10 +911,10 @@
                                 g ? g->n : 0, stream);
 }
 
-extern "C" int gcl_gcn_layer_fwd_rows(const gcl_graph_t* g, const float* x, int64_t ldx, int64_t bsx, int32_t act,
-                                      const float* slope, const float* W, const float* bias, float* y, int64_t ldy,
-                                      int64_t bsy, int32_t B, int32_t Fin, int32_t Fout, int32_t Fout_store,
-                                      int32_t rows_out, gcl_stream_t stream) {
+static int layer_fwd_impl(const gcl_graph_t* g, const float* x, int64_t ldx, int64_t bsx, int32_t act,
+                          const float* slope, const float* W, const float* bias, float* y, int64_t ldy, int64_t bsy,
+                          int32_t B, int32_t Fin, int32_t Fout, int32_t Fout_store, int32_t rows_out,
+                          const int32_t* present, gcl_stream_t stream) {
   GCL_CHECK_ARG(g && x && W && y, "gcn_layer_fwd: null argument");
   GCL_CHECK_ARG(g->kind == GCL_GRAPH_GCN || g->kind == GCL_GRAPH_MEAN, "gcn_layer_fwd: graph carries no edge weights");
   GCL_CHECK_ARG(B > 0 && Fin >= 4 && Fin <= 64 && Fin % 4 == 0 && Fout >= 1 && Fout <= 64,
@@ -908,6 +930,12 @@
   const int32_t n = g->n;
   GCL_CHECK_ARG(rows_out >= 1 && rows_out <= n, "gcn_layer_fwd: rows_out=%d outside [1, n=%d]", rows_out, n);
   hipStream_t st = (hipStream_t)stream;
+  if (present) {
+    bool launched = false;
+    const int rc = halo_layer_launch(g, x, ldx, bsx, nullptr, 0, act, slope, W, bias, y, ldy, bsy, B, Fin, Fout, Fout_store,
+                                     rows_out, st, &launched, present);
+    if (rc || launched) return rc;
+  }
   {
     bool launched = false;
     const int rc = halo_layer_launch(g, x, ldx, bsx, nullptr, 0, act, slope, W, bias, y, ldy, bsy, B, Fin, Fout, Fout_store,
@@ -985,6 +1013,22 @@
   return GCL_OK;
 }
 
+extern "C" int gcl_gcn_layer_fwd_rows(const gcl_graph_t* g, const float* x, int64_t ldx, int64_t bsx, int32_t act,
+                                      const float* slope, const float* W, const float* bias, float* y, int64_t ldy,
+                                      int64_t bsy, int32_t B, int32_t Fin, int32_t Fout, int32_t Fout_store,
+                                      int32_t rows_out, gcl_stream_t stream) {
+  return layer_fwd_impl(g, x, ldx, bsx, act, slope, W, bias, y, ldy, bsy, B, Fin, Fout, Fout_store, rows_out, nullptr, stream);
+}
+
+extern "C" int gcl_gcn_layer_fwd_present(const gcl_graph_t* g, const float* x, int64_t ldx, int64_t bsx, int32_t act,
+                                         const float* slope, const float* W, const float* bias, float* y, int64_t ldy,
+                                         int64_t bsy, const int32_t* present, int32_t B, int32_t Fin, int32_t Fout,
+                                         int32_t Fout_store, gcl_stream_t stream) {
+  GCL_CHECK_ARG(present, "gcn_layer_fwd_present: null presence table");
+  return layer_fwd_impl(g, x, ldx, bsx, act, slope, W, bias, y, ldy, bsy, B, Fin, Fout, Fout_store, g ? g->n : 0, present,
+                        stream);
+}
+
 extern "C" int gcl_gcn_layer_fwd_tab(const gcl_graph_t* g, const float* x, int64_t ldx, int64_t bsx, int64_t x_rows,
                                      const int32_t* tab, int32_t act, const float* slope, const float* W,
                                      const float* bias, float* y, int64_t ldy, int64_t bsy, int32_t B, int32_t Fin,
diff --git a/graphcast-lite_amd/csrc/norm.hip b/graphcast-lite_amd/csrc/norm.hip
--- a/graphcast-lite_amd/csrc/norm.hip
+++ b/graphcast-lite_amd/csrc/norm.hip
@@ -45,13 +45,14 @@
   }
 }
 
-template <int LPR, bool V, bool MAP = false>
+template <int LPR, bool V, bool MAP = false, bool LIST = false>
 __global__ __launch_bounds__(256) void ln_fwd_kernel(const float* __restrict__ X, int64_t ldx,
                                                      const float* __restrict__ gamma, const float* __restrict__ beta,
                                                      float eps, float* __restrict__ Y, int64_t ldy,
                                                      float* __restrict__ stats, int64_t rows, int32_t F, int32_t vx,
                                                      int32_t vy, const int32_t* __restrict__ pos = nullptr,
-                                                     int64_t bsy = 0, int32_t n_per = 1) {
+                                                     int64_t bsy = 0, int32_t n_per = 1,
+                                                     const int32_t* __restrict__ rlist = nullptr, int32_t n_list = 1) {
   if (V) vx = vy = 1;
   constexpr int RPB = (64 / LPR) * 4;
   const int lane = threadIdx.x & 63, wave = threadIdx.x >> 6;
@@ -62,7 +63,28 @@
     load4(gamma + c0, c0, F, false, g0, g1, g2, g3);
     load4(beta + c0, c0, F, false, b0, b1, b2, b3);
   }
-  for (int64_t row = (int64_t)blockIdx.x * RPB + wave * (64 / LPR) + sub; row < rows; row += (int64_t)gridDim.x * RPB) {
+  const int64_t item_first = (int64_t)blockIdx.x * RPB + wave * (64 / LPR) + sub, item_step = (int64_t)gridDim.x * RPB;
+  int64_t lb = 0, lsb = 0;
+  int li = 0, lsi = 0;
+  if (LIST) {
+    lb = item_first / n_list;
+    li = (int)(item_first - lb * n_list);
+    lsb = item_step / n_list;
+    lsi = (int)(item_step - lsb * n_list);
+  }
+  for (int64_t item = item_first; item < rows; item += item_step) {
+    int64_t row = item;
+    int pl = 0;
+    int64_t lbq = 0;
+    if (LIST) {
+      const int r = rlist[li];
+      lbq = lb;
+      row = lb * n_per + r;
+      pl = pos[r];
+      li += lsi;
+      lb += lsb;
+      if (li >= n_list) { li -= n_list; ++lb; }
+    }
     float x0 = 0, x1 = 0, x2 = 0, x3 = 0;
     if (c0 < F) load4_row<V>(X + row * ldx + c0, c0, F, vx, x0, x1, x2, x3);
     const float mean = group_sum<LPR>(x0 + x1 + x2 + x3) * invF;
@@ -77,8 +99,8 @@
     const float var = group_sum<LPR>(sq) * invF;
     const float rstd = 1.0f / sqrtf(var + eps);
     if (MAP) {
-      const int64_t bq = row / n_per;
-      const int pj = pos[(int)(row - bq * n_per)];
+      const int64_t bq = LIST ? lbq : row / n_per;
+      const int pj = LIST ? pl : pos[(int)(row - bq * n_per)];
       if (c0 < F && pj >= 0)
         store4(Y + bq * bsy + (int64_t)pj * ldy + c0, c0, F, vy, d0 * rstd * g0 + b0, d1 * rstd * g1 + b1,
                d2 * rstd * g2 + b2, d3 * rstd * g3 + b3);
@@ -92,7 +114,7 @@
   }
 }
 
-template <int LPR, bool V, bool CS, bool MAP>
+template <int LPR, bool V, bool CS, bool MAP, bool SKIP = false>
 __global__ __launch_bounds__(256) void ln_bwd_kernel(const float* __restrict__ dY, int64_t lddy,
                                                      const float* __restrict__ X, int64_t ldx,
                                                      const float* __restrict__ gamma, const float* __restrict__ stats,
@@ -123,7 +145,18 @@
   }
   for (int64_t row = row_first; row < rows; row += row_step) {
     float x0 = 0, x1 = 0, x2 = 0, x3 = 0, y0 = 0, y1 = 0, y2 = 0, y3 = 0;
-    if (c0 < F) {
+    if (SKIP) {
+      const int pj = pos[mi];
+      const int64_t mb_row = mb;
+      mi += msi;
+      mb += msb;
+      if (mi >= n_per) { mi -= n_per; ++mb; }
+      if (pj < 0) continue;
+      if (c0 < F) {
+        load4_row<V>(X + row * ldx + c0, c0, F, vx, x0, x1, x2, x3);
+        load4_row<V>(dY + mb_row * bsdy + (int64_t)pj * lddy + c0, c0, F, vdy, y0, y1, y2, y3);
+      }
+    } else if (c0 < F) {
       load4_row<V>(X + row * ldx + c0, c0, F, vx, x0, x1, x2, x3);
       if (MAP) {
         const int pj = pos[mi];
@@ -132,7 +165,7 @@
         load4_row<V>(dY + row * lddy + c0, c0, F, vdy, y0, y1, y2, y3);
       }
     }
-    if (MAP) {
+    if (MAP && !SKIP) {
       mi += msi;
       mb += msb;
       if (mi >= n_per) { mi -= n_per; ++mb; }
@@ -279,6 +312,34 @@
   return GCL_OK;
 }
 
+extern "C" int gcl_layernorm_fwd_map_skip(const float* x, int64_t ldx, const float* gamma, const float* beta, float eps,
+                                          float* y, int64_t ldy, int64_t bsy, const int32_t* pos, int32_t n_per,
+                                          const int32_t* rlist, int32_t n_list, float* stats, int64_t rows, int32_t F,
+                                          gcl_stream_t stream) {
+  GCL_CHECK_ARG(x && gamma && beta && y && pos && stats && rlist, "layernorm_fwd_map_skip: null argument");
+  GCL_CHECK_ARG(F >= 1 && F <= 256 && ldx >= F && ldy >= F, "layernorm_fwd_map_skip: bad shape F=%d", F);
+  GCL_CHECK_ARG(n_per > 0 && rows % n_per == 0, "layernorm_fwd_map_skip: rows must be B * n_per");
+  GCL_CHECK_ARG(n_list >= 0 && n_list <= n_per, "layernorm_fwd_map_skip: bad list length %d", n_list);
+  const int64_t items = rows / n_per * n_list;
+  if (items == 0) return GCL_OK;
+  const int lpr = lpr_for(F);
+  const int rpb = (64 / lpr) * 4;
+  int64_t nb = gcl::cdiv(items, rpb);
+  if (nb > 8192) nb = 8192;
+  const int vx = vec_ok(x, ldx, F), vy = vec_store_ok(y, ldy, F) && (bsy % 4 == 0);
+#define CALL(L)                                                                                                       \
+  if (vx && vy)                                                                                                       \
+    hipLaunchKernelGGL((ln_fwd_kernel<L, true, true, true>), dim3((unsigned)nb), dim3(256), 0, (hipStream_t)stream, x, \
+                       ldx, gamma, beta, eps, y, ldy, stats, items, F, vx, vy, pos, bsy, n_per, rlist, n_list);       \
+  else                                                                                                                \
+    hipLaunchKernelGGL((ln_fwd_kernel<L, false, true, true>), dim3((unsigned)nb), dim3(256), 0, (hipStream_t)stream,  \
+                       x, ldx, gamma, beta, eps, y, ldy, stats, items, F, vx, vy, pos, bsy, n_per, rlist, n_list)
+  GCL_DISPATCH_LPR(lpr, CALL)
+#undef CALL
+  GCL_CHECK_LAUNCH();
+  return GCL_OK;
+}
+
 extern "C" size_t gcl_layernorm_bwd_ws_bytes(int64_t rows, int32_t F) {
   (void)rows;
   const size_t FP = (size_t)((F + 3) / 4) * 4;
@@ -293,10 +354,10 @@
                                rows, F, ws, ws_bytes, stream);
 }
 
-extern "C" int gcl_layernorm_bwd_map(const float* dy, int64_t lddy, int64_t bsdy, const int32_t* pos, int32_t n_per,
-                                     const float* x, int64_t ldx, const float* gamma, const float* stats, float* dx,
-                                     int64_t lddx, float* dgamma, float* dbeta, float* colsum_dx, int32_t accumulate,
-                                     int64_t rows, int32_t F, void* ws, size_t ws_bytes, gcl_stream_t stream) {
+static int layernorm_bwd_impl(const float* dy, int64_t lddy, int64_t bsdy, const int32_t* pos, int32_t n_per,
+                              const float* x, int64_t ldx, const float* gamma, const float* stats, float* dx,
+                              int64_t lddx, float* dgamma, float* dbeta, float* colsum_dx, int32_t accumulate,
+                              int64_t rows, int32_t F, void* ws, size_t ws_bytes, gcl_stream_t stream, bool skip) {
   GCL_CHECK_ARG(dy && x && gamma && stats && dx && dgamma && dbeta, "layernorm_bwd: null argument");
   GCL_CHECK_ARG(!pos || (n_per > 0 && rows % n_per == 0), "layernorm_bwd: mapped dy needs rows = B * n_per");
   GCL_CHECK_ARG(F >= 1 && F <= 256 && ldx >= F && lddy >= F && lddx >= F, "layernorm_bwd: bad shape F=%d", F);
@@ -314,10 +375,13 @@
 #define CALL4(L, V_, CS_, MAP_)                                                                                       \
   hipLaunchKernelGGL((ln_bwd_kernel<L, V_, CS_, MAP_>), dim3((unsigned)nb), dim3(256), 0, st, dy, lddy, x, ldx, gamma, \
                      stats, dx, lddx, part, rows, F, FP, vdy, vx, vdx, pos, bsdy, n_per)
-#define CALL3(L, V_, CS_)            \
-  do {                               \
-    if (pos) CALL4(L, V_, CS_, true); \
-    else CALL4(L, V_, CS_, false);   \
+#define CALL3(L, V_, CS_)                                                                                              \
+  do {                                                                                                                 \
+    if (skip)                                                                                                          \
+      hipLaunchKernelGGL((ln_bwd_kernel<L, V_, CS_, true, true>), dim3((unsigned)nb), dim3(256), 0, st, dy, lddy, x, ldx, \
+                         gamma, stats, dx, lddx, part, rows, F, FP, vdy, vx, vdx, pos, bsdy, n_per);                   \
+    else if (pos) CALL4(L, V_, CS_, true);                                                                             \
+    else CALL4(L, V_, CS_, false);                                                                                     \
   } while (0)
 #define CALL(L)                                     \
   if (vdy && vx && vdx) {                           \
@@ -334,6 +398,24 @@
   GCL_CHECK_LAUNCH();
   if (!colsum_dx) return gcl::launch_reduce_parts2(part, (int)nb, 2 * FP, FP, FP, dgamma, dbeta, F, acc_p, st);
   return gcl::launch_reduce_parts3(part, (int)nb, 3 * FP, FP, dgamma, acc_p, dbeta, acc_p, colsum_dx, acc_cs, F, st);
+}
+
+extern "C" int gcl_layernorm_bwd_map(const float* dy, int64_t lddy, int64_t bsdy, const int32_t* pos, int32_t n_per,
+                                     const float* x, int64_t ldx, const float* gamma, const float* stats, float* dx,
+                                     int64_t lddx, float* dgamma, float* dbeta, float* colsum_dx, int32_t accumulate,
+                                     int64_t rows, int32_t F, void* ws, size_t ws_bytes, gcl_stream_t stream) {
+  return layernorm_bwd_impl(dy, lddy, bsdy, pos, n_per, x, ldx, gamma, stats, dx, lddx, dgamma, dbeta, colsum_dx, accumulate,
+                            rows, F, ws, ws_bytes, stream, false);
+}
+
+extern "C" int gcl_layernorm_bwd_map_skip(const float* dy, int64_t lddy, int64_t bsdy, const int32_t* pos, int32_t n_per,
+                                          const float* x, int64_t ldx, const float* gamma, const float* stats, float* dx,
+                                          int64_t lddx, float* dgamma, float* dbeta, float* colsum_dx,
+                                          int32_t accumulate, int64_t rows, int32_t F, void* ws, size_t ws_bytes,
+                                          gcl_stream_t stream) {
+  GCL_CHECK_ARG(pos, "layernorm_bwd_map_skip: the row map is required");
+  return layernorm_bwd_impl(dy, lddy, bsdy, pos, n_per, x, ldx, gamma, stats, dx, lddx, dgamma, dbeta, colsum_dx, accumulate,
+                            rows, F, ws, ws_bytes, stream, true);
 }
 
 extern "C" int gcl_layernorm_bwd(const float* dy, int64_t lddy, const float* x, int64_t ldx, const float* gamma,
diff --git a/graphcast-lite_amd/functional.py b/graphcast-lite_amd/functional.py
--- a/graphcast-lite_amd/functional.py
+++ b/graphcast-lite_amd/functional.py
@@ -99,6 +99,10 @@
 
 _LN_COLSUM = os.environ.get("GCL_NO_LN_COLSUM", "0") in ("0", "")
 _ROWS_OUT = os.environ.get("GCL_NO_ROWS_OUT", "0") in ("0", "")
+
+
+def _row_skip() -> bool:
+    return os.environ.get("GCL_NO_ROW_SKIP", "0") in ("0", "")
 
 
 def _lat_first_layer_bwd(lat, enc3, dz3, W, dW, acc_dw: bool, want_dx: bool, Pc=None, enc_shape=None):
@@ -177,6 +181,13 @@
         ps = []
         cur = x3
         pad_last = None
+        land0 = getattr(owner, "_grad_src", None)
+        F_last = params[2 * (L - 1)].shape[0]
+        skip = None
+        if (has_ln and land0 is not None and land0.dec_buf is not None and getattr(land0, "dec_rows", None) is not None
+                and not (out_rows and out_rows < n) and not squeeze and _LN_COLSUM and F_last % 4 == 0
+                and land0.dec_buf.shape[2] == F_last and land0.dec_rows.numel() < n and _row_skip()):
+            skip = (land0.dec_map, land0.dec_rows)
         for k in range(L):
             W, b = params[2 * k].detach(), params[2 * k + 1].detach()
             Fout = W.shape[0]
@@ -191,7 +202,8 @@
                 continue
             if hip.gcn_layer_fusable(graph, cur, W.shape[1], Fout):
                 last_rows = int(out_rows) if (k == L - 1 and out_rows and out_rows < n and not has_ln and _ROWS_OUT) else None
-                p = hip.gcn_layer_fwd(graph, cur, act_k, slope_k, W, b, rows_out=last_rows)
+                p = hip.gcn_layer_fwd(graph, cur, act_k, slope_k, W, b, rows_out=last_rows,
+                                      present=skip[0] if (skip is not None and k == L - 1) else None)
                 if k == L - 1 and ldh != Fout and not has_ln:
                     pad_last = (ldh, Fout, None)
                 elif ldh != Fout:
@@ -226,13 +238,19 @@
         if has_ln:
             land = ctx.land
             if land is not None and land.dec_buf is not None and cur.is_contiguous() and land.dec_buf.shape[2] == cur.shape[2]:
-                stats = hip.layernorm_fwd_map(cur.view(B * n, -1), params[-2].detach(), params[-1].detach(), eps,
-                                              land.dec_buf, land.dec_map)
+                if skip is not None:
+                    stats = hip.layernorm_fwd_map_skip(cur.view(B * n, -1), params[-2].detach(), params[-1].detach(), eps,
+                                                       land.dec_buf, skip[0], skip[1])
+                else:
+                    stats = hip.layernorm_fwd_map(cur.view(B * n, -1), params[-2].detach(), params[-1].detach(), eps,
+                                                  land.dec_buf, land.dec_map)
                 land.dec_filled = True
                 out = cur.new_zeros(()).expand(B, n, cur.shape[2])
             else:
+                assert skip is None, "rows were skipped upstream of a dense LayerNorm"
                 o2, stats = hip.layernorm_fwd(cur.view(B * n, -1), params[-2].detach(), params[-1].detach(), eps)
                 out = o2.view(B, n, -1)
+        ctx.skip = skip
         ctx.owner, ctx.graph, ctx.L, ctx.has_ln = owner, graph, L, has_ln
         ctx.x3, ctx.ps, ctx.stats, ctx.params, ctx.squeeze = x3, ps, stats, params, squeeze
         ctx.n_rows, ctx.out_rows = n, (int(out_rows) if out_rows and out_rows < n else 0)
@@ -271,9 +289,13 @@
             dgam = G.dst[gi] if G.dst[gi] is not None else torch.zeros_like(params[gi])
             dbet = G.dst[bi] if G.dst[bi] is not None else torch.zeros_like(params[bi])
             cs = G.dst[bi_last] if (pad is None and _LN_COLSUM) else None
+            if ctx.skip is not None and dy_map is None:
+                raise RuntimeError("the processor's output received a gradient from outside the decoder-input gather, but its "
+                                   "dropped rows were not kept (set GCL_NO_ROW_SKIP=1 to keep them)")
             dp = hip.layernorm_bwd(None if dy_map is not None else dy3.view(B * n, -1), ps[-1].view(B * n, -1),
                                    params[gi].detach(), ctx.stats, dgam, dbet, G.acc[gi] and G.acc[bi], colsum_dx=cs,
-                                   acc_colsum=bool(cs is not None and G.acc[bi_last]), dy_map=dy_map).view(B, n, -1)
+                                   acc_colsum=bool(cs is not None and G.acc[bi_last]), dy_map=dy_map,
+                                   skip=ctx.skip is not None).view(B, n, -1)
             cs_done = cs is not None
         else:
             dp = dy3
@@ -293,7 +315,10 @@
             W = params[2 * k].detach()
             wi = 2 * k
             inp = (ctx.x3 if k == 0 else ps[k - 1]).view(-1, (ctx.x3 if k == 0 else ps[k - 1]).shape[-1])
-            dh2 = hip.aggregate(graph, dp, None, transpose=True).view(B * n, -1)
+            if k == L - 1 and ctx.skip is not None:
+                dh2 = hip.aggregate_present(graph, dp, ctx.skip[0], transpose=True).view(B * n, -1)
+            else:
+                dh2 = hip.aggregate(graph, dp, None, transpose=True).view(B * n, -1)
             if k == L - 1 and Fp != Fo:
                 dh2 = dh2[:, :Fo]
             dW = G.dst[wi] if G.dst[wi] is not None else torch.zeros_like(params[wi])
@@ -589,6 +614,7 @@
         self.handed_over = False
         self.proc_ready, self.proc_src, self.proc_map = False, None, None
         self.dec_buf, self.dec_map, self.dec_filled = None, None, False
+        self.dec_rows = None
 
 
 class MeshLatFn(torch.autograd.Function):
diff --git a/graphcast-lite_amd/hip.py b/graphcast-lite_amd/hip.py
--- a/graphcast-lite_amd/hip.py
+++ b/graphcast-lite_amd/hip.py
@@ -37,6 +37,7 @@
     "gcl_reduce_jobs": (C.c_int, [_vp, _i32, _vp]),
     "gcl_linear_bwd_all_ws_bytes": (_sz, [_i64, _i32, _i32]),
     "gcl_aggregate": (C.c_int, [_vp, _i32, _vp, _i64, _i64, _vp, _vp, _i64, _i64, _i32, _i32, _vp]),
+    "gcl_aggregate_present": (C.c_int, [_vp, _i32, _vp, _i64, _i64, _vp, _vp, _vp, _i64, _i64, _i32, _i32, _vp]),
     "gcl_gat_fwd": (C.c_int, [_vp, _vp, _i64, _i64, _vp, _vp, _vp, _vp, _vp, _vp, _vp, _i64, _i64, _i32, _i32, _i32, _vp]),
     "gcl_gat_bwd": (C.c_int, [_vp, _vp, _i64, _i64, _vp, _i64, _i64, _vp, _vp, _vp, _vp, _vp, _vp, _i64, _i64,
                               _vp, _vp, _vp, _i32, _i32, _i32, _i32, _vp, _sz, _vp]),
@@ -53,6 +54,10 @@
     "gcl_layernorm_bwd_cs": (C.c_int, [_vp, _i64, _vp, _i64, _vp, _vp, _vp, _i64, _vp, _vp, _vp, _i32, _i64, _i32, _vp, _sz, _vp]),
     "gcl_layernorm_bwd_map": (C.c_int, [_vp, _i64, _i64, _vp, _i32, _vp, _i64, _vp, _vp, _vp, _i64, _vp, _vp, _vp, _i32, _i64,
                                         _i32, _vp, _sz, _vp]),
+    "gcl_layernorm_fwd_map_skip": (C.c_int, [_vp, _i64, _vp, _vp, _f32, _vp, _i64, _i64, _vp, _i32, _vp, _i32, _vp, _i64, _i32,
+                                             _vp]),
+    "gcl_layernorm_bwd_map_skip": (C.c_int, [_vp, _i64, _i64, _vp, _i32, _vp, _i64, _vp, _vp, _vp, _i64, _vp, _vp, _vp, _i32,
+                                             _i64, _i32, _vp, _sz, _vp]),
     "gcl_layernorm_bwd_ws_bytes": (_sz, [_i64, _i32]),
     "gcl_graphnorm_fwd": (C.c_int, [_vp, _i64, _i64, _vp, _vp, _f32, _vp, _i64, _i64, _vp, _i32, _i32, _i32, _vp, _sz, _vp]),
     "gcl_graphnorm_bwd": (C.c_int, [_vp, _i64, _i64, _vp, _i64, _i64, _vp, _vp, _f32, _vp, _i64, _i64, _vp, _vp,
@@ -80,6 +85,8 @@
                                    C.c_size_t, _vp]),
     "gcl_gcn_layer_fwd": (C.c_int, [_vp, _vp, _i64, _i64, _i32, _vp, _vp, _vp, _vp, _i64, _i64, _i32, _i32, _i32, _i32, _vp]),
     "gcl_gcn_layer_fwd_rows": (C.c_int, [_vp, _vp, _i64, _i64, _i32, _vp, _vp, _vp, _vp, _i64, _i64, _i32, _i32, _i32, _i32, _i32, _vp]),
+    "gcl_gcn_layer_fwd_present": (C.c_int, [_vp, _vp, _i64, _i64, _i32, _vp, _vp, _vp, _vp, _i64, _i64, _vp, _i32, _i32, _i32, _i32,
+                                            _vp]),
     "gcl_layernorm_fwd_map": (C.c_int, [_vp, _i64, _vp, _vp, _f32, _vp, _i64, _i64, _vp, _i32, _vp, _i64, _i32, _vp]),
     "gcl_gcn_layer_fwd_tab": (C.c_int, [_vp, _vp, _i64, _i64, _i64, _vp, _i32, _vp, _vp, _vp, _vp, _i64, _i64, _i32, _i32, _i32, _i32, _vp]),
     "gcl_gcn_layer_fwd_tab_ok": (C.c_int, [_vp, _i64, _i64, _i64, _i32, _i32, _i32]),
@@ -469,6 +476,19 @@
     return out
 
 
+def aggregate_present(graph: Graph, h3, present, bias=None, transpose=False, out=None):
+    B, n, F = h3.shape
+    assert n == graph.n, f"graph has {graph.n} nodes, features have {n} rows"
+    assert h3.stride(2) == 1 and present.dtype == torch.int32 and present.numel() == n and present.is_contiguous()
+    if out is None:
+        out = torch.empty(B, n, F, dtype=torch.float32, device=h3.device)
+    tok = _probe_begin("aggregate_present", graph=graph, transpose=bool(transpose), B=B, F=F)
+    _check(lib().gcl_aggregate_present(graph.handle, 1 if transpose else 0, _p(h3), h3.stride(1), h3.stride(0),
+                                       _pi(present), _p(bias), _p(out), out.stride(1), out.stride(0), B, F, _stream()))
+    _probe_end(tok)
+    return out
+
+
 def layernorm_fwd(x, gamma, beta, eps=1e-5):
     rows, F = x.shape
     y = torch.empty(rows, F, dtype=torch.float32, device=x.device)
@@ -487,8 +507,19 @@
     return stats
 
 
+def layernorm_fwd_map_skip(x, gamma, beta, eps, out3, pos, rlist):
+    rows, F = x.shape
+    n_per = pos.numel()
+    assert out3.stride(2) == 1 and rows % n_per == 0 and out3.shape[0] == rows // n_per and rlist.stride(0) == 1
+    stats = torch.empty(rows, 2, dtype=torch.float32, device=x.device)
+    _check(lib().gcl_layernorm_fwd_map_skip(_p(x), _ld(x), _p(gamma), _p(beta), float(eps), _p(out3), out3.stride(1),
+                                            out3.stride(0), _pi(pos), n_per, _pi(rlist), rlist.numel(), _p(stats), rows, F,
+                                            _stream()))
+    return stats
+
+
 def layernorm_bwd(dy, x, gamma, stats, dgamma, dbeta, accumulate: bool, colsum_dx=None, acc_colsum: bool = False,
-                  dy_map=None):
+                  dy_map=None, skip: bool = False):
     rows, F = x.shape
     dx = torch.empty(rows, F, dtype=torch.float32, device=x.device)
     nb = lib().gcl_layernorm_bwd_ws_bytes(rows, F)
@@ -497,10 +528,12 @@
     if dy_map is not None:
         src3, pos = dy_map
         assert src3.stride(2) == 1 and src3.shape[2] >= F and rows % pos.numel() == 0 and src3.shape[0] == rows // pos.numel()
-        _check(lib().gcl_layernorm_bwd_map(_p(src3), src3.stride(1), src3.stride(0), _pi(pos), pos.numel(), _p(x), _ld(x),
+        fn = lib().gcl_layernorm_bwd_map_skip if skip else lib().gcl_layernorm_bwd_map
+        _check(fn(_p(src3), src3.stride(1), src3.stride(0), _pi(pos), pos.numel(), _p(x), _ld(x),
                                            _p(gamma), _p(stats), _p(dx), F, _p(dgamma), _p(dbeta), _p(colsum_dx), acc, rows, F,
                                            ws.data_ptr(), ws.numel(), _stream()))
         return dx
+    assert not skip, "skip needs the mapped gradient"
     _check(lib().gcl_layernorm_bwd_cs(_p(dy), _ld(dy), _p(x), _ld(x), _p(gamma), _p(stats), _p(dx), F, _p(dgamma),
                                       _p(dbeta), _p(colsum_dx), acc, rows, F, ws.data_ptr(), ws.numel(), _stream()))
     return dx
@@ -857,7 +890,7 @@
             and x3.stride(2) == 1 and x3.stride(1) % 4 == 0 and x3.stride(0) % 4 == 0 and x3.data_ptr() % 16 == 0)
 
 
-def gcn_layer_fwd(graph: Graph, x3, act, slope, W, bias, out=None, rows_out=None):
+def gcn_layer_fwd(graph: Graph, x3, act, slope, W, bias, out=None, rows_out=None, present=None):
     B, n, Fin = x3.shape
     assert n == graph.n
     Fout = W.shape[0]
@@ -865,6 +898,14 @@
     if out is None:
         out = torch.empty(B, n, Fst, dtype=torch.float32, device=x3.device)
     assert out.shape[2] >= Fst or out.stride(1) >= Fst
+    if present is not None:
+        assert not rows_out and present.numel() == n
+        tok = _probe_begin("gcn_layer_fwd_present", graph=graph, B=B, Fin=Fin, Fout=Fout)
+        _check(lib().gcl_gcn_layer_fwd_present(graph.handle, _p(x3), x3.stride(1), x3.stride(0), int(act), _p(slope),
+                                               _p(W.contiguous()), _p(bias), _p(out), out.stride(1), out.stride(0),
+                                               _pi(present), B, Fin, Fout, Fst, _stream()))
+        _probe_end(tok)
+        return out[..., :Fout]
     tok = _probe_begin("gcn_layer_fwd", graph=graph, B=B, Fin=Fin, Fout=Fout)
     _check(lib().gcl_gcn_layer_fwd_rows(graph.handle, _p(x3), x3.stride(1), x3.stride(0), int(act), _p(slope),
                                         _p(W.contiguous()), _p(bias), _p(out), out.stride(1), out.stride(0), B, Fin, Fout,
diff --git a/graphcast-lite_amd/models.py b/graphcast-lite_amd/models.py
--- a/graphcast-lite_amd/models.py
+++ b/graphcast-lite_amd/models.py
@@ -726,6 +726,7 @@
                     and not squeeze):
                 land.dec_buf = torch.empty(B, G + c.U, enc_c.shape[-1], dtype=torch.float32, device=enc_c.device)
                 land.dec_map = maps_dec[3]
+                land.dec_rows = maps_dec[1][G:]
             if lat_src is not None:
                 processed = self.processor.forward(X=enc_c, edge_index=pg, attention_threshold=attention_threshold,
                                                    _lat_src=lat_src, **({"_grad_src": land} if land is not None else {}))
diff --git a/include/gcl.h b/include/gcl.h
--- a/include/gcl.h
+++ b/include/gcl.h
@@ -99,6 +99,9 @@
 int gcl_aggregate(const gcl_graph_t* g, int32_t transpose, const float* h, int64_t ldh, int64_t bsh,
                   const float* bias, float* y, int64_t ldy, int64_t bsy, int32_t B, int32_t F,
                   gcl_stream_t stream);
+int gcl_aggregate_present(const gcl_graph_t* g, int32_t transpose, const float* h, int64_t ldh, int64_t bsh,
+                          const int32_t* present , const float* bias, float* y, int64_t ldy, int64_t bsy,
+                          int32_t B, int32_t F, gcl_stream_t stream);
 
 int gcl_gat_fwd(const gcl_graph_t* g, const float* h, int64_t ldh, int64_t bsh,
                 const float* att_src , const float* att_dst , const float* bias ,
@@ -147,6 +150,14 @@
                           const float* x, int64_t ldx, const float* gamma, const float* stats, float* dx,
                           int64_t lddx, float* dgamma, float* dbeta, float* colsum_dx, int32_t accumulate,
                           int64_t rows, int32_t F, void* ws, size_t ws_bytes, gcl_stream_t stream);
+int gcl_layernorm_fwd_map_skip(const float* x, int64_t ldx, const float* gamma, const float* beta, float eps, float* y,
+                               int64_t ldy, int64_t bsy, const int32_t* pos , int32_t n_per,
+                               const int32_t* rlist , int32_t n_list, float* stats, int64_t rows, int32_t F,
+                               gcl_stream_t stream);
+int gcl_layernorm_bwd_map_skip(const float* dy, int64_t lddy, int64_t bsdy, const int32_t* pos, int32_t n_per,
+                               const float* x, int64_t ldx, const float* gamma, const float* stats, float* dx,
+                               int64_t lddx, float* dgamma, float* dbeta, float* colsum_dx, int32_t accumulate,
+                               int64_t rows, int32_t F, void* ws, size_t ws_bytes, gcl_stream_t stream);
 size_t gcl_layernorm_bwd_ws_bytes(int64_t rows, int32_t F);
 int gcl_graphnorm_fwd(const float* x, int64_t ldx, int64_t bsx, const float* gamma, const float* beta,
                       float eps, float* y, int64_t ldy, int64_t bsy, float* stats, int32_t B,
@@ -199,6 +210,10 @@
                            const float* slope, const float* W , const float* bias, float* y,
                            int64_t ldy, int64_t bsy, int32_t B, int32_t Fin, int32_t Fout, int32_t Fout_store,
                            int32_t rows_out, gcl_stream_t stream);
+int gcl_gcn_layer_fwd_present(const gcl_graph_t* g, const float* x, int64_t ldx, int64_t bsx, int32_t act,
+                              const float* slope, const float* W, const float* bias, float* y, int64_t ldy, int64_t bsy,
+                              const int32_t* present , int32_t B, int32_t Fin, int32_t Fout, int32_t Fout_store,
+                              gcl_stream_t stream);
 int gcl_gcn_layer_fwd_tab(const gcl_graph_t* g, const float* x, int64_t ldx, int64_t bsx, int64_t x_rows,
                           const int32_t* tab , int32_t act, const float* slope, const float* W ,
                           const float* bias, float* y, int64_t ldy, int64_t bsy, int32_t B, int32_t Fin, int32_t Fout,
```

Result: faster. 24990 (median of 6 runs) (+1.3%).
